# speechbrain/speechbrain

Measured on NVIDIA H100. Metric: audio-sec/sec (RTFx) Conformer-L ASR, batch=32x10s@16kHz, higher is better.
Workload: dtype fp16 operands, fp32 accumulate/residual/softmax

## Files before the change

### speechbrain_b200/csrc/common.cuh

```cuda
#pragma once
#include <cuda.h>
#include <cuda_fp16.h>
#include <cuda_runtime.h>
#include <stdint.h>

#define SBK_OK 0
#define SBK_ERR_CUDA -1
#define SBK_ERR_ARG -2
#define SBK_ERR_UNSUPPORTED -3
#define SBK_ERR_NOMEM -4

namespace sbk {

void set_error(const char* fmt, ...);

#define SBK_CUDA_CHECK(expr)                                                              \
    do {                                                                                  \
        cudaError_t _e = (expr);                                                          \
        if (_e != cudaSuccess) {                                                          \
            sbk::set_error("%s:%d: %s -> %s", __FILE__, __LINE__, #expr, cudaGetErrorString(_e)); \
            return SBK_ERR_CUDA;                                                          \
        }                                                                                 \
    } while (0)

void count_launch();
#define SBK_LAUNCH_CHECK()                   \
    do {                                     \
        sbk::count_launch();                 \
        SBK_CUDA_CHECK(cudaGetLastError());  \
    } while (0)

#define SBK_REQUIRE(cond, ...)            \
    do {                                  \
        if (!(cond)) {                    \
            sbk::set_error(__VA_ARGS__);  \
            return SBK_ERR_ARG;           \
        }                                 \
    } while (0)

__host__ __device__ inline int ceil_div(int a, int b) { return (a + b - 1) / b; }

constexpr int SBK_NUM_SMS = 132;

__device__ __forceinline__ float warp_sum(float v) {
#pragma unroll
    for (int o = 16; o > 0; o >>= 1) v += __shfl_xor_sync(0xffffffffu, v, o);
    return v;
}
__device__ __forceinline__ float warp_max(float v) {
#pragma unroll
    for (int o = 16; o > 0; o >>= 1) v = fmaxf(v, __shfl_xor_sync(0xffffffffu, v, o));
    return v;
}

__device__ __forceinline__ uint32_t smem_u32(const void* p) {
    return static_cast<uint32_t>(__cvta_generic_to_shared(p));
}

__device__ __forceinline__ void mbar_init(uint64_t* bar, uint32_t count) {
    asm volatile("mbarrier.init.shared::cta.b64 [%0], %1;" ::"r"(smem_u32(bar)), "r"(count));
}
__device__ __forceinline__ void mbar_fence_init() {
    asm volatile("fence.mbarrier_init.release.cluster;" ::: "memory");
}
__device__ __forceinline__ void mbar_arrive_expect_tx(uint64_t* bar, uint32_t bytes) {
    asm volatile("mbarrier.arrive.expect_tx.shared::cta.b64 _, [%0], %1;" ::"r"(smem_u32(bar)), "r"(bytes)
                 : "memory");
}
__device__ __forceinline__ void mbar_arrive(uint64_t* bar) {
    asm volatile("mbarrier.arrive.shared::cta.b64 _, [%0];" ::"r"(smem_u32(bar)) : "memory");
}
__device__ __forceinline__ bool mbar_try_wait(uint64_t* bar, uint32_t parity) {
    uint32_t ok;
    asm volatile(
        "{\n\t.reg .pred p;\n\t"
        "mbarrier.try_wait.parity.shared::cta.b64 p, [%1], %2;\n\t"
        "selp.u32 %0, 1, 0, p;\n\t}"
        : "=r"(ok)
        : "r"(smem_u32(bar)), "r"(parity)
        : "memory");
    return ok != 0;
}
__device__ __forceinline__ void mbar_wait(uint64_t* bar, uint32_t parity) {
    while (!mbar_try_wait(bar, parity)) {
    }
}

__device__ __forceinline__ void tma_prefetch_desc(const CUtensorMap* m) {
    asm volatile("prefetch.tensormap [%0];" ::"l"(reinterpret_cast<uint64_t>(m)) : "memory");
}
__device__ __forceinline__ void tma_load_2d(void* smem_dst, const CUtensorMap* m, uint64_t* bar, int c0, int c1) {
    asm volatile(
        "cp.async.bulk.tensor.2d.shared::cluster.global.mbarrier::complete_tx::bytes [%0], [%1, {%3, %4}], [%2];"
        ::"r"(smem_u32(smem_dst)), "l"(reinterpret_cast<uint64_t>(m)), "r"(smem_u32(bar)), "r"(c0), "r"(c1)
        : "memory");
}
__device__ __forceinline__ void tma_load_4d(void* smem_dst, const CUtensorMap* m, uint64_t* bar, int c0, int c1, int c2, int c3) {
    asm volatile(
        "cp.async.bulk.tensor.4d.shared::cluster.global.mbarrier::complete_tx::bytes [%0], [%1, {%3, %4, %5, %6}], [%2];"
        ::"r"(smem_u32(smem_dst)), "l"(reinterpret_cast<uint64_t>(m)), "r"(smem_u32(bar)), "r"(c0), "r"(c1), "r"(c2), "r"(c3)
        : "memory");
}
__device__ __forceinline__ void bulk_load_1d(void* smem_dst, const void* gsrc, uint32_t bytes, uint64_t* bar) {
    asm volatile(
        "cp.async.bulk.shared::cluster.global.mbarrier::complete_tx::bytes [%0], [%1], %2, [%3];"
        ::"r"(smem_u32(smem_dst)), "l"(reinterpret_cast<uint64_t>(gsrc)), "r"(bytes), "r"(smem_u32(bar))
        : "memory");
}

__device__ __forceinline__ void wgmma_fence() { asm volatile("wgmma.fence.sync.aligned;" ::: "memory"); }
__device__ __forceinline__ void wgmma_commit() { asm volatile("wgmma.commit_group.sync.aligned;" ::: "memory"); }
template <int N>
__device__ __forceinline__ void wgmma_wait() { asm volatile("wgmma.wait_group.sync.aligned %0;" ::"n"(N) : "memory"); }

__device__ __forceinline__ uint64_t make_kmajor_sw128_desc(uint32_t smem_addr) {
    uint64_t d = 0;
    d |= static_cast<uint64_t>((smem_addr & 0x3FFFFu) >> 4);
    d |= static_cast<uint64_t>(1) << 16;
    d |= static_cast<uint64_t>(1024 >> 4) << 32;
    d |= static_cast<uint64_t>(1) << 62;
    return d;
}

template <int N>
__device__ __forceinline__ void wgmma_f16(float (&d)[N / 2], uint64_t desc_a, uint64_t desc_b, uint32_t accumulate);
template <>
__device__ __forceinline__ void wgmma_f16<32>(float (&d)[16], uint64_t desc_a, uint64_t desc_b, uint32_t accumulate) {
    asm volatile(
        "{\n\t.reg .pred p;\n\tsetp.ne.b32 p, %18, 0;\n\t"
        "wgmma.mma_async.sync.aligned.m64n32k16.f32.f16.f16 "
        "{%0, %1, %2, %3, %4, %5, %6, %7, %8, %9, %10, %11, %12, %13, %14, %15}, "
        "%16, %17, p, 1, 1, 0, 0;\n\t}"
        : "+f"(d[0]), "+f"(d[1]), "+f"(d[2]), "+f"(d[3]), "+f"(d[4]), "+f"(d[5]), "+f"(d[6]), "+f"(d[7]),
          "+f"(d[8]), "+f"(d[9]), "+f"(d[10]), "+f"(d[11]), "+f"(d[12]), "+f"(d[13]), "+f"(d[14]), "+f"(d[15])
        : "l"(desc_a), "l"(desc_b), "r"(accumulate)
        : "memory");
}
template <>
__device__ __forceinline__ void wgmma_f16<64>(float (&d)[32], uint64_t desc_a, uint64_t desc_b, uint32_t accumulate) {
    asm volatile(
        "{\n\t.reg .pred p;\n\tsetp.ne.b32 p, %34, 0;\n\t"
        "wgmma.mma_async.sync.aligned.m64n64k16.f32.f16.f16 "
        "{%0, %1, %2, %3, %4, %5, %6, %7, %8, %9, %10, %11, %12, %13, %14, %15, "
        "%16, %17, %18, %19, %20, %21, %22, %23, %24, %25, %26, %27, %28, %29, %30, %31}, "
        "%32, %33, p, 1, 1, 0, 0;\n\t}"
        : "+f"(d[0]), "+f"(d[1]), "+f"(d[2]), "+f"(d[3]), "+f"(d[4]), "+f"(d[5]), "+f"(d[6]), "+f"(d[7]),
          "+f"(d[8]), "+f"(d[9]), "+f"(d[10]), "+f"(d[11]), "+f"(d[12]), "+f"(d[13]), "+f"(d[14]), "+f"(d[15]),
          "+f"(d[16]), "+f"(d[17]), "+f"(d[18]), "+f"(d[19]), "+f"(d[20]), "+f"(d[21]), "+f"(d[22]), "+f"(d[23]),
          "+f"(d[24]), "+f"(d[25]), "+f"(d[26]), "+f"(d[27]), "+f"(d[28]), "+f"(d[29]), "+f"(d[30]), "+f"(d[31])
        : "l"(desc_a), "l"(desc_b), "r"(accumulate)
        : "memory");
}
template <>
__device__ __forceinline__ void wgmma_f16<128>(float (&d)[64], uint64_t desc_a, uint64_t desc_b, uint32_t accumulate) {
    asm volatile(
        "{\n\t.reg .pred p;\n\tsetp.ne.b32 p, %66, 0;\n\t"
        "wgmma.mma_async.sync.aligned.m64n128k16.f32.f16.f16 "
        "{%0, %1, %2, %3, %4, %5, %6, %7, %8, %9, %10, %11, %12, %13, %14, %15, "
        "%16, %17, %18, %19, %20, %21, %22, %23, %24, %25, %26, %27, %28, %29, %30, %31, "
        "%32, %33, %34, %35, %36, %37, %38, %39, %40, %41, %42, %43, %44, %45, %46, %47, "
        "%48, %49, %50, %51, %52, %53, %54, %55, %56, %57, %58, %59, %60, %61, %62, %63}, "
        "%64, %65, p, 1, 1, 0, 0;\n\t}"
        : "+f"(d[0]), "+f"(d[1]), "+f"(d[2]), "+f"(d[3]), "+f"(d[4]), "+f"(d[5]), "+f"(d[6]), "+f"(d[7]),
          "+f"(d[8]), "+f"(d[9]), "+f"(d[10]), "+f"(d[11]), "+f"(d[12]), "+f"(d[13]), "+f"(d[14]), "+f"(d[15]),
          "+f"(d[16]), "+f"(d[17]), "+f"(d[18]), "+f"(d[19]), "+f"(d[20]), "+f"(d[21]), "+f"(d[22]), "+f"(d[23]),
          "+f"(d[24]), "+f"(d[25]), "+f"(d[26]), "+f"(d[27]), "+f"(d[28]), "+f"(d[29]), "+f"(d[30]), "+f"(d[31]),
          "+f"(d[32]), "+f"(d[33]), "+f"(d[34]), "+f"(d[35]), "+f"(d[36]), "+f"(d[37]), "+f"(d[38]), "+f"(d[39]),
          "+f"(d[40]), "+f"(d[41]), "+f"(d[42]), "+f"(d[43]), "+f"(d[44]), "+f"(d[45]), "+f"(d[46]), "+f"(d[47]),
          "+f"(d[48]), "+f"(d[49]), "+f"(d[50]), "+f"(d[51]), "+f"(d[52]), "+f"(d[53]), "+f"(d[54]), "+f"(d[55]),
          "+f"(d[56]), "+f"(d[57]), "+f"(d[58]), "+f"(d[59]), "+f"(d[60]), "+f"(d[61]), "+f"(d[62]), "+f"(d[63])
        : "l"(desc_a), "l"(desc_b), "r"(accumulate)
        : "memory");
}

template <>
__device__ __forceinline__ void wgmma_f16<256>(float (&d)[128], uint64_t desc_a, uint64_t desc_b, uint32_t accumulate) {
    asm volatile(
        "{\n\t.reg .pred p;\n\tsetp.ne.b32 p, %130, 0;\n\t"
        "wgmma.mma_async.sync.aligned.m64n256k16.f32.f16.f16 "
        "{"
        "%0, %1, %2, %3, %4, %5, %6, %7, %8, %9, %10, %11, %12, %13, %14, %15, "
        "%16, %17, %18, %19, %20, %21, %22, %23, %24, %25, %26, %27, %28, %29, %30, %31, "
        "%32, %33, %34, %35, %36, %37, %38, %39, %40, %41, %42, %43, %44, %45, %46, %47, "
        "%48, %49, %50, %51, %52, %53, %54, %55, %56, %57, %58, %59, %60, %61, %62, %63, "
        "%64, %65, %66, %67, %68, %69, %70, %71, %72, %73, %74, %75, %76, %77, %78, %79, "
        "%80, %81, %82, %83, %84, %85, %86, %87, %88, %89, %90, %91, %92, %93, %94, %95, "
        "%96, %97, %98, %99, %100, %101, %102, %103, %104, %105, %106, %107, %108, %109, %110, %111, "
        "%112, %113, %114, %115, %116, %117, %118, %119, %120, %121, %122, %123, %124, %125, %126, %127}, "
        "%128, %129, p, 1, 1, 0, 0;\n\t}"
        :
          "+f"(d[0]), "+f"(d[1]), "+f"(d[2]), "+f"(d[3]), "+f"(d[4]), "+f"(d[5]), "+f"(d[6]), "+f"(d[7]),
          "+f"(d[8]), "+f"(d[9]), "+f"(d[10]), "+f"(d[11]), "+f"(d[12]), "+f"(d[13]), "+f"(d[14]), "+f"(d[15]),
          "+f"(d[16]), "+f"(d[17]), "+f"(d[18]), "+f"(d[19]), "+f"(d[20]), "+f"(d[21]), "+f"(d[22]), "+f"(d[23]),
          "+f"(d[24]), "+f"(d[25]), "+f"(d[26]), "+f"(d[27]), "+f"(d[28]), "+f"(d[29]), "+f"(d[30]), "+f"(d[31]),
          "+f"(d[32]), "+f"(d[33]), "+f"(d[34]), "+f"(d[35]), "+f"(d[36]), "+f"(d[37]), "+f"(d[38]), "+f"(d[39]),
          "+f"(d[40]), "+f"(d[41]), "+f"(d[42]), "+f"(d[43]), "+f"(d[44]), "+f"(d[45]), "+f"(d[46]), "+f"(d[47]),
          "+f"(d[48]), "+f"(d[49]), "+f"(d[50]), "+f"(d[51]), "+f"(d[52]), "+f"(d[53]), "+f"(d[54]), "+f"(d[55]),
          "+f"(d[56]), "+f"(d[57]), "+f"(d[58]), "+f"(d[59]), "+f"(d[60]), "+f"(d[61]), "+f"(d[62]), "+f"(d[63]),
          "+f"(d[64]), "+f"(d[65]), "+f"(d[66]), "+f"(d[67]), "+f"(d[68]), "+f"(d[69]), "+f"(d[70]), "+f"(d[71]),
          "+f"(d[72]), "+f"(d[73]), "+f"(d[74]), "+f"(d[75]), "+f"(d[76]), "+f"(d[77]), "+f"(d[78]), "+f"(d[79]),
          "+f"(d[80]), "+f"(d[81]), "+f"(d[82]), "+f"(d[83]), "+f"(d[84]), "+f"(d[85]), "+f"(d[86]), "+f"(d[87]),
          "+f"(d[88]), "+f"(d[89]), "+f"(d[90]), "+f"(d[91]), "+f"(d[92]), "+f"(d[93]), "+f"(d[94]), "+f"(d[95]),
          "+f"(d[96]), "+f"(d[97]), "+f"(d[98]), "+f"(d[99]), "+f"(d[100]), "+f"(d[101]), "+f"(d[102]), "+f"(d[103]),
          "+f"(d[104]), "+f"(d[105]), "+f"(d[106]), "+f"(d[107]), "+f"(d[108]), "+f"(d[109]), "+f"(d[110]), "+f"(d[111]),
          "+f"(d[112]), "+f"(d[113]), "+f"(d[114]), "+f"(d[115]), "+f"(d[116]), "+f"(d[117]), "+f"(d[118]), "+f"(d[119]),
          "+f"(d[120]), "+f"(d[121]), "+f"(d[122]), "+f"(d[123]), "+f"(d[124]), "+f"(d[125]), "+f"(d[126]), "+f"(d[127])
        : "l"(desc_a), "l"(desc_b), "r"(accumulate)
        : "memory");
}

__device__ __forceinline__ __half2 floats2half2_sat(float lo, float hi) {
    uint32_t r;
    asm("cvt.rn.satfinite.f16x2.f32 %0, %1, %2;" : "=r"(r) : "f"(hi), "f"(lo));
    return *reinterpret_cast<__half2*>(&r);
}
__device__ __forceinline__ __half float2half_sat(float x) {
    const __half2 h = floats2half2_sat(x, 0.0f);
    return __low2half(h);
}

__device__ __forceinline__ float rcp_approx(float x) {
    float y;
    asm("rcp.approx.ftz.f32 %0, %1;" : "=f"(y) : "f"(x));
    return y;
}
__device__ __forceinline__ float exp_ftz(float x) {
    float y;
    asm("ex2.approx.ftz.f32 %0, %1;" : "=f"(y) : "f"(x * 1.4426950408889634f));
    return y;
}
__device__ __forceinline__ float sigmoid_f(float x) { return rcp_approx(1.0f + exp_ftz(-x)); }
__device__ __forceinline__ float tanh_approx(float x) {
    float y;
    asm("tanh.approx.f32 %0, %1;" : "=f"(y) : "f"(x));
    return y;
}
__device__ __forceinline__ float sigmoid_fast(float x) { return fmaf(0.5f, tanh_approx(0.5f * x), 0.5f); }
__device__ __forceinline__ float silu_fast(float x) {
    const float h = 0.5f * x;
    return fmaf(h, tanh_approx(h), h);
}
__device__ __forceinline__ void sts128(uint32_t addr, uint4 v) {
    asm volatile("st.shared.v4.b32 [%0], {%1, %2, %3, %4};" ::"r"(addr), "r"(v.x), "r"(v.y), "r"(v.z), "r"(v.w) : "memory");
}
__device__ __forceinline__ uint4 lds128(uint32_t addr) {
    uint4 v;
    asm volatile("ld.shared.v4.b32 {%0, %1, %2, %3}, [%4];" : "=r"(v.x), "=r"(v.y), "=r"(v.z), "=r"(v.w) : "r"(addr) : "memory");
    return v;
}
__device__ __forceinline__ uint4 f4_as_u4(float4 f) {
    return make_uint4(__float_as_uint(f.x), __float_as_uint(f.y), __float_as_uint(f.z), __float_as_uint(f.w));
}
__device__ __forceinline__ float4 u4_as_f4(uint4 u) {
    return make_float4(__uint_as_float(u.x), __uint_as_float(u.y), __uint_as_float(u.z), __uint_as_float(u.w));
}
__device__ __forceinline__ float silu_f(float x) { return x * sigmoid_f(x); }
__device__ __forceinline__ float gelu_erf_f(float x) { return 0.5f * x * (1.0f + erff(x * 0.70710678118654752f)); }

__device__ __forceinline__ int float_to_ordered(float f) {
    int i = __float_as_int(f);
    return i >= 0 ? i : i ^ 0x7FFFFFFF;
}
__device__ __forceinline__ float ordered_to_float(int i) { return __int_as_float(i >= 0 ? i : i ^ 0x7FFFFFFF); }

int make_tmap_2d_f16(CUtensorMap* out, const void* base, uint64_t rows, uint64_t cols, uint64_t row_stride_elems,
                     uint32_t box_rows, uint32_t box_cols);

}
```

### speechbrain_b200/csrc/decoder.cu

```cuda
#include <stdlib.h>

#include <algorithm>

#include "common.cuh"
#include "sbk_internal.h"

namespace sbk {

__device__ __forceinline__ void mma16816_d(float (&d)[4], const uint32_t (&a)[4], uint32_t b0, uint32_t b1) {
    asm volatile(
        "mma.sync.aligned.m16n8k16.row.col.f32.f16.f16.f32 {%0,%1,%2,%3}, {%4,%5,%6,%7}, {%8,%9}, {%0,%1,%2,%3};"
        : "+f"(d[0]), "+f"(d[1]), "+f"(d[2]), "+f"(d[3])
        : "r"(a[0]), "r"(a[1]), "r"(a[2]), "r"(a[3]), "r"(b0), "r"(b1));
}

__device__ __forceinline__ void pdl_trigger() { asm volatile("griddepcontrol.launch_dependents;" ::: "memory"); }
__device__ __forceinline__ void pdl_wait() { asm volatile("griddepcontrol.wait;" ::: "memory"); }

static bool g_use_pdl = true;
void set_pdl(bool on) { g_use_pdl = on; }

template <typename... KArgs, typename... Args>
static cudaError_t launch_k(void (*kern)(KArgs...), dim3 grid, dim3 block, size_t smem, cudaStream_t st, Args... args) {
    cudaLaunchConfig_t cfg = {};
    cfg.gridDim = grid;
    cfg.blockDim = block;
    cfg.dynamicSmemBytes = smem;
    cfg.stream = st;
    cudaLaunchAttribute attr[1];
    attr[0].id = cudaLaunchAttributeProgrammaticStreamSerialization;
    attr[0].val.programmaticStreamSerializationAllowed = 1;
    cfg.attrs = attr;
    cfg.numAttrs = g_use_pdl ? 1 : 0;
    return cudaLaunchKernelEx(&cfg, kern, args...);
}

constexpr int SK_WARPS = 8;

template <int UNR, int NT, int VPL, int MT = 2>
__global__ void __launch_bounds__(SK_WARPS * 32, ((VPL <= 4 && MT == 2) ? 2 : 1)) skinny_gemm_kernel(const SkinnyArgs a) {
    constexpr bool LN = VPL > 0;
    constexpr int SK_ROWS = 16 * MT;
    static_assert(!LN || MT == 2, "the LayerNorm-fused variant owns 32 rows per CTA");
    __shared__ float red[SK_WARPS][SK_ROWS][8 * NT + 1];
    extern __shared__ __align__(16) __half a_sm[];
    const int warp = threadIdx.x >> 5, lane = threadIdx.x & 31, g = lane >> 2, c = lane & 3;
    const int n0 = blockIdx.x * 8 * NT;
    const int row0 = blockIdx.y * SK_ROWS;
    const int rows = min(SK_ROWS, a.n_rows - row0);
    const int k_per_warp = ((a.K / 16 + SK_WARPS - 1) / SK_WARPS) * 16;
    const int k_begin = warp * k_per_warp, k_end = min(a.K, k_begin + k_per_warp);
    pdl_trigger();

    float acc[MT][NT][4];
#pragma unroll
    for (int i = 0; i < MT; ++i)
#pragma unroll
        for (int j = 0; j < NT; ++j) acc[i][j][0] = acc[i][j][1] = acc[i][j][2] = acc[i][j][3] = 0.0f;
    const __half* wrow[NT];
#pragma unroll
    for (int j = 0; j < NT; ++j)
        wrow[j] = a.W + static_cast<size_t>(min(n0 + 8 * j + g, a.N - 1)) * a.ldw + 2 * c;
    uint32_t bf[UNR][NT][2];
#pragma unroll
    for (int u = 0; u < UNR; ++u) {
        const int k = k_begin + 16 * u;
        const bool ok = k < k_end;
#pragma unroll
        for (int j = 0; j < NT; ++j) {
            bf[u][j][0] = ok ? __ldg(reinterpret_cast<const uint32_t*>(wrow[j] + k)) : 0u;
            bf[u][j][1] = ok ? __ldg(reinterpret_cast<const uint32_t*>(wrow[j] + k + 8)) : 0u;
        }
    }
    pdl_wait();

    const int astr = LN ? a.K + 8 : a.lda;
    const __half* abase = LN ? a_sm : a.A;
    if constexpr (LN) {
        float4 v[4][VPL];
#pragma unroll
        for (int r = 0; r < 4; ++r) {
            const float* xr = a.X + static_cast<size_t>(min(row0 + warp + 8 * r, a.n_rows - 1)) * a.K;
#pragma unroll
            for (int i = 0; i < VPL; ++i) v[r][i] = *reinterpret_cast<const float4*>(xr + 4 * (lane + 32 * i));
        }
        float4 gm[VPL], bt[VPL];
#pragma unroll
        for (int i = 0; i < VPL; ++i) {
            gm[i] = __ldg(reinterpret_cast<const float4*>(a.ln_g + 4 * (lane + 32 * i)));
            bt[i] = __ldg(reinterpret_cast<const float4*>(a.ln_b + 4 * (lane + 32 * i)));
        }
        float s[4], q[4];
#pragma unroll
        for (int r = 0; r < 4; ++r) {
            s[r] = 0.0f;
#pragma unroll
            for (int i = 0; i < VPL; ++i) s[r] += (v[r][i].x + v[r][i].y) + (v[r][i].z + v[r][i].w);
        }
#pragma unroll
        for (int o = 16; o > 0; o >>= 1)
#pragma unroll
            for (int r = 0; r < 4; ++r) s[r] += __shfl_xor_sync(0xffffffffu, s[r], o);
        const float inv_k = 1.0f / static_cast<float>(a.K);
#pragma unroll
        for (int r = 0; r < 4; ++r) {
            s[r] *= inv_k;
            q[r] = 0.0f;
#pragma unroll
            for (int i = 0; i < VPL; ++i) {
                v[r][i].x -= s[r]; v[r][i].y -= s[r]; v[r][i].z -= s[r]; v[r][i].w -= s[r];
                q[r] += (v[r][i].x * v[r][i].x + v[r][i].y * v[r][i].y) + (v[r][i].z * v[r][i].z + v[r][i].w * v[r][i].w);
            }
        }
#pragma unroll
        for (int o = 16; o > 0; o >>= 1)
#pragma unroll
            for (int r = 0; r < 4; ++r) q[r] += __shfl_xor_sync(0xffffffffu, q[r], o);
#pragma unroll
        for (int r = 0; r < 4; ++r) {
            const float rstd = rsqrtf(q[r] * inv_k + a.ln_eps);
            __half* dst = a_sm + (warp + 8 * r) * astr;
#pragma unroll
            for (int i = 0; i < VPL; ++i) {
                __half2 h0 = floats2half2_sat(v[r][i].x * rstd * gm[i].x + bt[i].x, v[r][i].y * rstd * gm[i].y + bt[i].y);
                __half2 h1 = floats2half2_sat(v[r][i].z * rstd * gm[i].z + bt[i].z, v[r][i].w * rstd * gm[i].w + bt[i].w);
                uint2 u;
                u.x = *reinterpret_cast<uint32_t*>(&h0);
                u.y = *reinterpret_cast<uint32_t*>(&h1);
                *reinterpret_cast<uint2*>(dst + 4 * (lane + 32 * i)) = u;
            }
        }
        __syncthreads();
    }
    const __half* arow[2 * MT];
#pragma unroll
    for (int i = 0; i < 2 * MT; ++i) {
        const int rr = LN ? (i * 8 + g) : min(row0 + i * 8 + g, a.n_rows - 1);
        arow[i] = abase + static_cast<size_t>(rr) * astr + 2 * c;
    }
    for (int k0 = k_begin; k0 < k_end; k0 += 16 * UNR) {
        uint32_t af[UNR][MT][4];
#pragma unroll
        for (int u = 0; u < UNR; ++u) {
            const int k = k0 + 16 * u;
            const bool ok = k < k_end;
            if (k0 != k_begin) {
#pragma unroll
                for (int j = 0; j < NT; ++j) {
                    bf[u][j][0] = ok ? __ldg(reinterpret_cast<const uint32_t*>(wrow[j] + k)) : 0u;
                    bf[u][j][1] = ok ? __ldg(reinterpret_cast<const uint32_t*>(wrow[j] + k + 8)) : 0u;
                }
            }
#pragma unroll
            for (int mt = 0; mt < MT; ++mt) {
                af[u][mt][0] = ok ? *reinterpret_cast<const uint32_t*>(arow[2 * mt] + k) : 0u;
                af[u][mt][1] = ok ? *reinterpret_cast<const uint32_t*>(arow[2 * mt + 1] + k) : 0u;
                af[u][mt][2] = ok ? *reinterpret_cast<const uint32_t*>(arow[2 * mt] + k + 8) : 0u;
                af[u][mt][3] = ok ? *reinterpret_cast<const uint32_t*>(arow[2 * mt + 1] + k + 8) : 0u;
            }
        }
#pragma unroll
        for (int u = 0; u < UNR; ++u)
#pragma unroll
            for (int j = 0; j < NT; ++j)
#pragma unroll
                for (int mt = 0; mt < MT; ++mt) mma16816_d(acc[mt][j], af[u][mt], bf[u][j][0], bf[u][j][1]);
    }
#pragma unroll
    for (int mt = 0; mt < MT; ++mt)
#pragma unroll
        for (int j = 0; j < NT; ++j) {
            red[warp][mt * 16 + g][8 * j + 2 * c] = acc[mt][j][0];
            red[warp][mt * 16 + g][8 * j + 2 * c + 1] = acc[mt][j][1];
            red[warp][mt * 16 + g + 8][8 * j + 2 * c] = acc[mt][j][2];
            red[warp][mt * 16 + g + 8][8 * j + 2 * c + 1] = acc[mt][j][3];
        }
    __syncthreads();
    const int step = a.step_ptr ? *a.step_ptr : 0;
#pragma unroll
    for (int it = 0; it < NT * MT / 2; ++it) {
        const int idx = threadIdx.x + it * SK_WARPS * 32;
        const int r = idx / (8 * NT), j = idx - r * (8 * NT);
        const int col = n0 + j;
        const int row = row0 + r;
        if (r < rows && col < a.N) {
            float v = 0.0f;
#pragma unroll
            for (int w = 0; w < SK_WARPS; ++w) v += red[w][r][j];
            if (a.bias) v += __ldg(a.bias + col);
            switch (a.epi) {
                case SK_F16: reinterpret_cast<__half*>(a.out)[static_cast<size_t>(row) * a.ldo + col] = float2half_sat(v); break;
                case SK_F16_RELU:
                    reinterpret_cast<__half*>(a.out)[static_cast<size_t>(row) * a.ldo + col] = float2half_sat(fmaxf(v, 0.0f));
                    break;
                case SK_F16_GELU:
                    reinterpret_cast<__half*>(a.out)[static_cast<size_t>(row) * a.ldo + col] = float2half_sat(gelu_erf_f(v));
                    break;
                case SK_F32: reinterpret_cast<float*>(a.out)[static_cast<size_t>(row) * a.ldo + col] = v; break;
                case SK_RESID: reinterpret_cast<float*>(a.out)[static_cast<size_t>(row) * a.ldo + col] += v; break;
                case SK_QKV_CACHE: {
                    if (col < a.d) {
                        reinterpret_cast<__half*>(a.out)[static_cast<size_t>(row) * a.ldo + col] = float2half_sat(v * a.q_scale);
                    } else if (col < 2 * a.d) {
                        a.kcache[(static_cast<size_t>(row) * a.S_max + step) * a.d + (col - a.d)] = float2half_sat(v);
                    } else {
                        a.vcache[(static_cast<size_t>(row) * a.S_max + step) * a.d + (col - 2 * a.d)] = float2half_sat(v);
                    }
                    break;
                }
            }
        }
    }
}

int skinny_gemm(const SkinnyArgs& a, cudaStream_t stream) {
    SBK_REQUIRE(a.K % 16 == 0 && a.lda % 2 == 0 && a.ldw % 2 == 0, "skinny_gemm: K %% 16 required (K=%d)", a.K);
    if (a.n_rows == 0) return SBK_OK;
    cudaError_t e;
    const int ry = ceil_div(a.n_rows, 32);
    if (a.X == nullptr && a.n_rows >= 96 && getenv("SBK_SKINNY_MT8") != nullptr) {
        const dim3 grid(ceil_div(a.N, 8), ceil_div(a.n_rows, 128));
        if (a.K <= 1024) e = launch_k(skinny_gemm_kernel<2, 1, 0, 8>, grid, dim3(SK_WARPS * 32), 0, stream, a);
        else e = launch_k(skinny_gemm_kernel<4, 1, 0, 8>, grid, dim3(SK_WARPS * 32), 0, stream, a);
        SBK_CUDA_CHECK(e);
        SBK_LAUNCH_CHECK();
        return SBK_OK;
    }
    if (a.X != nullptr) {
        const size_t smem = static_cast<size_t>(32) * (a.K + 8) * 2;
        dim3 grid(ceil_div(a.N, 16), ry);
        static bool attr_done = false;
        if (!attr_done) {
            cudaFuncSetAttribute(skinny_gemm_kernel<4, 2, 4>, cudaFuncAttributeMaxDynamicSharedMemorySize, 80 * 1024);
            cudaFuncSetAttribute(skinny_gemm_kernel<2, 2, 2>, cudaFuncAttributeMaxDynamicSharedMemorySize, 80 * 1024);
            cudaFuncSetAttribute(skinny_gemm_kernel<4, 2, 6>, cudaFuncAttributeMaxDynamicSharedMemorySize, 80 * 1024);
            cudaFuncSetAttribute(skinny_gemm_kernel<8, 2, 8>, cudaFuncAttributeMaxDynamicSharedMemorySize, 80 * 1024);
            attr_done = true;
        }
        if (a.K == 512) e = launch_k(skinny_gemm_kernel<4, 2, 4>, grid, dim3(SK_WARPS * 32), smem, stream, a);
        else if (a.K == 256) e = launch_k(skinny_gemm_kernel<2, 2, 2>, grid, dim3(SK_WARPS * 32), smem, stream, a);
        else if (a.K == 768) e = launch_k(skinny_gemm_kernel<4, 2, 6>, grid, dim3(SK_WARPS * 32), smem, stream, a);
        else if (a.K == 1024) e = launch_k(skinny_gemm_kernel<8, 2, 8>, grid, dim3(SK_WARPS * 32), smem, stream, a);
        else {
            set_error("skinny_gemm(LN): d_model=%d not built (256/512/768/1024)", a.K);
            return SBK_ERR_UNSUPPORTED;
        }
    } else if (a.K <= 1024 && a.N >= 1024) {
        e = launch_k(skinny_gemm_kernel<4, 2, 0>, dim3(ceil_div(a.N, 16), ry), dim3(SK_WARPS * 32), 0, stream, a);
    } else if (a.K <= 1024) {
        e = launch_k(skinny_gemm_kernel<4, 1, 0>, dim3(ceil_div(a.N, 8), ry), dim3(SK_WARPS * 32), 0, stream, a);
    } else {
        e = launch_k(skinny_gemm_kernel<8, 1, 0>, dim3(ceil_div(a.N, 8), ry), dim3(SK_WARPS * 32), 0, stream, a);
    }
    SBK_CUDA_CHECK(e);
    SBK_LAUNCH_CHECK();
    return SBK_OK;
}

constexpr int DA_WARPS = 4;
constexpr int DA_CHUNK = 32;
constexpr int DA_KPG = DA_CHUNK / 4;

__global__ void __launch_bounds__(DA_WARPS * 32, 4) dec_attention_kernel(const DecAttnArgs a) {
    __shared__ float part_o[DA_WARPS][64];
    __shared__ float part_m[DA_WARPS], part_l[DA_WARPS];
    const int warp = threadIdx.x >> 5, lane = threadIdx.x & 31;
    const int r = blockIdx.y, h = blockIdx.x;
    const int blk = r / a.rows_per_block;
    pdl_trigger();
    pdl_wait();
    int n_keys;
    if (a.n_keys_ptr) n_keys = *a.n_keys_ptr + 1;
    else n_keys = a.enc_len ? min(a.enc_len[blk], a.n_keys_fixed) : a.n_keys_fixed;
    const int per = (n_keys + DA_WARPS - 1) / DA_WARPS;
    const int kb = warp * per, ke = min(n_keys, kb + per);
    const int gq = lane >> 3, dl = (lane & 7) * 8;
    const int hs = a.head_stride > 0 ? a.head_stride : 64;
    const __half* kbase = a.kbase + static_cast<size_t>(blk) * a.row_stride + static_cast<size_t>(h) * hs + dl;
    const __half* vbase = a.vbase + static_cast<size_t>(blk) * a.row_stride + static_cast<size_t>(h) * hs + dl;
    const int* lin = nullptr;
    if (a.lineage) lin = a.lineage + static_cast<size_t>((n_keys - 1) & 1) * gridDim.y * a.lin_stride + static_cast<size_t>(r) * a.lin_stride;
    const int* tokc = a.tok_cache;
    float qf[8];
    {
        const uint4 qv = *reinterpret_cast<const uint4*>(a.q + static_cast<size_t>(r) * a.ldq + h * 64 + dl);
        const __half2* q2 = reinterpret_cast<const __half2*>(&qv);
#pragma unroll
        for (int u = 0; u < 4; ++u) {
            const float2 f = __half22float2(q2[u]);
            qf[2 * u] = f.x; qf[2 * u + 1] = f.y;
        }
    }
    float m_run = -INFINITY, l_run = 0.0f;
    float o[8];
#pragma unroll
    for (int e = 0; e < 8; ++e) o[e] = 0.0f;
    for (int c0 = kb; c0 < ke; c0 += DA_CHUNK) {
        uint4 kv[DA_KPG], vv[DA_KPG];
        bool live[DA_KPG];
#pragma unroll
        for (int i = 0; i < DA_KPG; ++i) {
            const int j = c0 + gq + 4 * i;
            live[i] = j < ke;
            if (live[i]) {
                ptrdiff_t off = static_cast<ptrdiff_t>(j) * a.key_stride;
                int src_row = r;
                if (lin) { src_row = lin[j]; off += (static_cast<ptrdiff_t>(src_row) - r) * static_cast<ptrdiff_t>(a.row_stride); }
                kv[i] = *reinterpret_cast<const uint4*>(kbase + off);
                vv[i] = *reinterpret_cast<const uint4*>(vbase + off);
                if (tokc) live[i] = tokc[static_cast<size_t>(src_row) * a.lin_stride + j] != a.pad_tok;
            } else {
                kv[i] = make_uint4(0u, 0u, 0u, 0u);
                vv[i] = make_uint4(0u, 0u, 0u, 0u);
            }
        }
        float sc[DA_KPG];
        float cm = -INFINITY;
#pragma unroll
        for (int i = 0; i < DA_KPG; ++i) {
            const __half2* k2 = reinterpret_cast<const __half2*>(&kv[i]);
            float dot = 0.0f;
#pragma unroll
            for (int u = 0; u < 4; ++u) {
                const float2 kf = __half22float2(k2[u]);
                dot = fmaf(kf.x, qf[2 * u], dot);
                dot = fmaf(kf.y, qf[2 * u + 1], dot);
            }
            dot += __shfl_xor_sync(0xffffffffu, dot, 1);
            dot += __shfl_xor_sync(0xffffffffu, dot, 2);
            dot += __shfl_xor_sync(0xffffffffu, dot, 4);
            sc[i] = live[i] ? dot : -INFINITY;
            cm = fmaxf(cm, sc[i]);
        }
        cm = fmaxf(cm, __shfl_xor_sync(0xffffffffu, cm, 8));
        cm = fmaxf(cm, __shfl_xor_sync(0xffffffffu, cm, 16));
        const float m_new = fmaxf(m_run, cm);
        const float alpha = (m_run == -INFINITY) ? 0.0f : __expf(m_run - m_new);
        float psum = 0.0f;
#pragma unroll
        for (int e = 0; e < 8; ++e) o[e] *= alpha;
#pragma unroll
        for (int i = 0; i < DA_KPG; ++i) {
            const float p = (sc[i] == -INFINITY) ? 0.0f : __expf(sc[i] - m_new);
            psum += p;
            const __half2* v2 = reinterpret_cast<const __half2*>(&vv[i]);
#pragma unroll
            for (int u = 0; u < 4; ++u) {
                const float2 vf = __half22float2(v2[u]);
                o[2 * u] = fmaf(p, vf.x, o[2 * u]);
                o[2 * u + 1] = fmaf(p, vf.y, o[2 * u + 1]);
            }
        }
        psum += __shfl_xor_sync(0xffffffffu, psum, 8);
        psum += __shfl_xor_sync(0xffffffffu, psum, 16);
        l_run = l_run * alpha + psum;
        m_run = m_new;
    }
#pragma unroll
    for (int e = 0; e < 8; ++e) {
        o[e] += __shfl_xor_sync(0xffffffffu, o[e], 8);
        o[e] += __shfl_xor_sync(0xffffffffu, o[e], 16);
    }
    if (lane < 8) {
#pragma unroll
        for (int e = 0; e < 8; ++e) part_o[warp][dl + e] = o[e];
    }
    if (lane == 0) { part_m[warp] = m_run; part_l[warp] = l_run; }
    __syncthreads();
    if (threadIdx.x < 64) {
        float M = part_m[0];
#pragma unroll
        for (int w = 1; w < DA_WARPS; ++w) M = fmaxf(M, part_m[w]);
        float num = 0.0f, den = 0.0f;
#pragma unroll
        for (int w = 0; w < DA_WARPS; ++w) {
            const float sc = part_m[w] == -INFINITY ? 0.0f : __expf(part_m[w] - M);
            num += part_o[w][threadIdx.x] * sc;
            den += part_l[w] * sc;
        }
        a.out[static_cast<size_t>(r) * a.ldo + h * 64 + threadIdx.x] = float2half_sat(num / den);
    }
}

__global__ void __launch_bounds__(DA_WARPS * 32)
dec_cross_attention_tma_kernel(const __grid_constant__ CUtensorMap tmap_kv, const DecAttnArgs a, int box_T) {
    extern __shared__ __align__(128) uint8_t xa_smem[];
    __shared__ uint64_t bar;
    __shared__ float part_o[DA_WARPS][64];
    __shared__ float part_m[DA_WARPS], part_l[DA_WARPS];
    const __half* Ks = reinterpret_cast<const __half*>(xa_smem);
    const __half* Vs = Ks + static_cast<size_t>(box_T) * 64;
    const int warp = threadIdx.x >> 5, lane = threadIdx.x & 31;
    const int r = blockIdx.y, h = blockIdx.x;
    const int blk = r / a.rows_per_block;
    if (threadIdx.x == 0) {
        mbar_init(&bar, 1);
        mbar_fence_init();
    }
    __syncthreads();
    if (threadIdx.x == 0) {
        mbar_arrive_expect_tx(&bar, static_cast<uint32_t>(box_T) * 256u);
        tma_load_4d(const_cast<__half*>(Ks), &tmap_kv, &bar, 0, h, 0, blk);
        tma_load_4d(const_cast<__half*>(Vs), &tmap_kv, &bar, 0, a.H + h, 0, blk);
    }
    const int n_keys = a.enc_len ? min(a.enc_len[blk], a.n_keys_fixed) : a.n_keys_fixed;
    const int per = (n_keys + DA_WARPS - 1) / DA_WARPS;
    const int kb = warp * per, ke = min(n_keys, kb + per);
    const int gq = lane >> 3, dl = (lane & 7) * 8;
    float qf[8];
    {
        const uint4 qv = *reinterpret_cast<const uint4*>(a.q + static_cast<size_t>(r) * a.ldq + h * 64 + dl);
        const __half2* q2 = reinterpret_cast<const __half2*>(&qv);
#pragma unroll
        for (int u = 0; u < 4; ++u) {
            const float2 f = __half22float2(q2[u]);
            qf[2 * u] = f.x; qf[2 * u + 1] = f.y;
        }
    }
    float m_run = -INFINITY, l_run = 0.0f;
    float o[8];
#pragma unroll
    for (int e = 0; e < 8; ++e) o[e] = 0.0f;
    mbar_wait(&bar, 0);
    for (int c0 = kb; c0 < ke; c0 += DA_CHUNK) {
        float sc[DA_KPG];
        float cm = -INFINITY;
#pragma unroll
        for (int i = 0; i < DA_KPG; ++i) {
            const int j = c0 + gq + 4 * i;
            float dot = 0.0f;
            if (j < ke) {
                const uint4 kv = *reinterpret_cast<const uint4*>(Ks + static_cast<size_t>(j) * 64 + dl);
                const __half2* k2 = reinterpret_cast<const __half2*>(&kv);
#pragma unroll
                for (int u = 0; u < 4; ++u) {
                    const float2 kf = __half22float2(k2[u]);
                    dot = fmaf(kf.x, qf[2 * u], dot);
                    dot = fmaf(kf.y, qf[2 * u + 1], dot);
                }
            }
            dot += __shfl_xor_sync(0xffffffffu, dot, 1);
            dot += __shfl_xor_sync(0xffffffffu, dot, 2);
            dot += __shfl_xor_sync(0xffffffffu, dot, 4);
            sc[i] = j < ke ? dot : -INFINITY;
            cm = fmaxf(cm, sc[i]);
        }
        cm = fmaxf(cm, __shfl_xor_sync(0xffffffffu, cm, 8));
        cm = fmaxf(cm, __shfl_xor_sync(0xffffffffu, cm, 16));
        const float m_new = fmaxf(m_run, cm);
        const float alpha = (m_run == -INFINITY) ? 0.0f : __expf(m_run - m_new);
        float psum = 0.0f;
#pragma unroll
        for (int e = 0; e < 8; ++e) o[e] *= alpha;
#pragma unroll
        for (int i = 0; i < DA_KPG; ++i) {
            const int j = c0 + gq + 4 * i;
            const float p = (sc[i] == -INFINITY) ? 0.0f : __expf(sc[i] - m_new);
            psum += p;
            if (j < ke) {
                const uint4 vv = *reinterpret_cast<const uint4*>(Vs + static_cast<size_t>(j) * 64 + dl);
                const __half2* v2 = reinterpret_cast<const __half2*>(&vv);
#pragma unroll
                for (int u = 0; u < 4; ++u) {
                    const float2 vf = __half22float2(v2[u]);
                    o[2 * u] = fmaf(p, vf.x, o[2 * u]);
                    o[2 * u + 1] = fmaf(p, vf.y, o[2 * u + 1]);
                }
            }
        }
        psum += __shfl_xor_sync(0xffffffffu, psum, 8);
        psum += __shfl_xor_sync(0xffffffffu, psum, 16);
        l_run = l_run * alpha + psum;
        m_run = m_new;
    }
#pragma unroll
    for (int e = 0; e < 8; ++e) {
        o[e] += __shfl_xor_sync(0xffffffffu, o[e], 8);
        o[e] += __shfl_xor_sync(0xffffffffu, o[e], 16);
    }
    if (lane < 8) {
#pragma unroll
        for (int e = 0; e < 8; ++e) part_o[warp][dl + e] = o[e];
    }
    if (lane == 0) { part_m[warp] = m_run; part_l[warp] = l_run; }
    __syncthreads();
    if (threadIdx.x < 64) {
        float M = part_m[0];
#pragma unroll
        for (int w = 1; w < DA_WARPS; ++w) M = fmaxf(M, part_m[w]);
        float num = 0.0f, den = 0.0f;
#pragma unroll
        for (int w = 0; w < DA_WARPS; ++w) {
            const float sc = part_m[w] == -INFINITY ? 0.0f : __expf(part_m[w] - M);
            num += part_o[w][threadIdx.x] * sc;
            den += part_l[w] * sc;
        }
        a.out[static_cast<size_t>(r) * a.ldo + h * 64 + threadIdx.x] = float2half_sat(num / den);
    }
}

constexpr int XP_WARPS = 8;
__global__ void __launch_bounds__(XP_WARPS * 32, 1)
dec_cross_attention_persist_kernel(const __grid_constant__ CUtensorMap tmap_kv, const DecAttnArgs a, int box_T, int n_items) {
    extern __shared__ __align__(128) uint8_t xp_smem[];
    __shared__ uint64_t full[2];
    __shared__ float part_o[XP_WARPS][64];
    __shared__ float part_m[XP_WARPS], part_l[XP_WARPS];
    const size_t stage_halfs = static_cast<size_t>(box_T) * 128;
    __half* stage0 = reinterpret_cast<__half*>(xp_smem);
    const int warp = threadIdx.x >> 5, lane = threadIdx.x & 31;
    const int gq = lane >> 3, dl = (lane & 7) * 8;
    const int H = a.H;
    if (threadIdx.x == 0) {
        mbar_init(&full[0], 1);
        mbar_init(&full[1], 1);
        mbar_fence_init();
    }
    __syncthreads();
    auto issue = [&](int item, int s) {
        const int r = item / H, h = item - r * H, blk = r / a.rows_per_block;
        __half* dst = stage0 + s * stage_halfs;
        mbar_arrive_expect_tx(&full[s], static_cast<uint32_t>(box_T) * 256u);
        tma_load_4d(dst, &tmap_kv, &full[s], 0, h, 0, blk);
        tma_load_4d(dst + static_cast<size_t>(box_T) * 64, &tmap_kv, &full[s], 0, H + h, 0, blk);
    };
    const int first = blockIdx.x, stride = gridDim.x;
    if (threadIdx.x == 0) {
        if (first < n_items) issue(first, 0);
        if (first + stride < n_items) issue(first + stride, 1);
    }
    auto load_q = [&](int item) {
        const int r = item / H, h = item - r * H;
        return *reinterpret_cast<const uint4*>(a.q + static_cast<size_t>(r) * a.ldq + h * 64 + dl);
    };
    uint4 qv = make_uint4(0u, 0u, 0u, 0u);
    if (first < n_items) qv = load_q(first);
    int it = 0;
    for (int item = first; item < n_items; item += stride, ++it) {
        const int s = it & 1;
        const int r = item / H, h = item - r * H, blk = r / a.rows_per_block;
        float qf[8];
        {
            const __half2* q2 = reinterpret_cast<const __half2*>(&qv);
#pragma unroll
            for (int u = 0; u < 4; ++u) {
                const float2 f = __half22float2(q2[u]);
                qf[2 * u] = f.x; qf[2 * u + 1] = f.y;
            }
        }
        if (item + stride < n_items) qv = load_q(item + stride);
        const int n_keys = a.enc_len ? min(a.enc_len[blk], a.n_keys_fixed) : a.n_keys_fixed;
        const __half* Ks = stage0 + s * stage_halfs;
        const __half* Vs = Ks + static_cast<size_t>(box_T) * 64;
        mbar_wait(&full[s], (it >> 1) & 1);
        const int c0 = warp * DA_CHUNK;
        float sc[DA_KPG];
        float cm = -INFINITY;
#pragma unroll
        for (int i = 0; i < DA_KPG; ++i) {
            const int j = c0 + gq + 4 * i;
            float dot = 0.0f;
            if (j < n_keys) {
                const uint4 kv = *reinterpret_cast<const uint4*>(Ks + static_cast<size_t>(j) * 64 + dl);
                const __half2* k2 = reinterpret_cast<const __half2*>(&kv);
#pragma unroll
                for (int u = 0; u < 4; ++u) {
                    const float2 kf = __half22float2(k2[u]);
                    dot = fmaf(kf.x, qf[2 * u], dot);
                    dot = fmaf(kf.y, qf[2 * u + 1], dot);
                }
            }
            dot += __shfl_xor_sync(0xffffffffu, dot, 1);
            dot += __shfl_xor_sync(0xffffffffu, dot, 2);
            dot += __shfl_xor_sync(0xffffffffu, dot, 4);
            sc[i] = j < n_keys ? dot : -INFINITY;
            cm = fmaxf(cm, sc[i]);
        }
        cm = fmaxf(cm, __shfl_xor_sync(0xffffffffu, cm, 8));
        cm = fmaxf(cm, __shfl_xor_sync(0xffffffffu, cm, 16));
        float o[8];
#pragma unroll
        for (int e = 0; e < 8; ++e) o[e] = 0.0f;
        float psum = 0.0f;
#pragma unroll
        for (int i = 0; i < DA_KPG; ++i) {
            const int j = c0 + gq + 4 * i;
            const float p = (sc[i] == -INFINITY) ? 0.0f : __expf(sc[i] - cm);
            psum += p;
            if (j < n_keys) {
                const uint4 vv = *reinterpret_cast<const uint4*>(Vs + static_cast<size_t>(j) * 64 + dl);
                const __half2* v2 = reinterpret_cast<const __half2*>(&vv);
#pragma unroll
                for (int u = 0; u < 4; ++u) {
                    const float2 vf = __half22float2(v2[u]);
                    o[2 * u] = fmaf(p, vf.x, o[2 * u]);
                    o[2 * u + 1] = fmaf(p, vf.y, o[2 * u + 1]);
                }
            }
        }
        psum += __shfl_xor_sync(0xffffffffu, psum, 8);
        psum += __shfl_xor_sync(0xffffffffu, psum, 16);
#pragma unroll
        for (int e = 0; e < 8; ++e) {
            o[e] += __shfl_xor_sync(0xffffffffu, o[e], 8);
            o[e] += __shfl_xor_sync(0xffffffffu, o[e], 16);
        }
        if (lane < 8) {
#pragma unroll
            for (int e = 0; e < 8; ++e) part_o[warp][dl + e] = o[e];
        }
        if (lane == 0) { part_m[warp] = cm; part_l[warp] = psum; }
        __syncthreads();
        if (threadIdx.x == 0 && item + 2 * stride < n_items) issue(item + 2 * stride, s);
        if (threadIdx.x < 64) {
            float M = part_m[0];
#pragma unroll
            for (int w = 1; w < XP_WARPS; ++w) M = fmaxf(M, part_m[w]);
            float num = 0.0f, den = 0.0f;
// ... 936 lines not shown
```

### speechbrain_b200/csrc/encoder_ops.cu

```cuda
#include <algorithm>

#include "common.cuh"
#include "sbk_internal.h"

namespace sbk {

constexpr int LN_MAX_PER_LANE = 32;

template <bool OUT_HALF>
__global__ void __launch_bounds__(256)
layernorm_rows_kernel(const float* __restrict__ x, void* __restrict__ out, const float* __restrict__ gamma,
                      const float* __restrict__ beta, int M, int D, float eps, int act_silu) {
    const int row = blockIdx.x * (blockDim.x >> 5) + (threadIdx.x >> 5);
    if (row >= M) return;
    const int lane = threadIdx.x & 31;
    const float* xr = x + static_cast<size_t>(row) * D;
    float v[LN_MAX_PER_LANE];
    float s = 0.0f;
    const int nv = D >> 2;
#pragma unroll
    for (int i = 0; i < LN_MAX_PER_LANE / 4; ++i) {
        const int vi = lane + i * 32;
        if (vi < nv) {
            const float4 t = *reinterpret_cast<const float4*>(xr + vi * 4);
            v[4 * i] = t.x; v[4 * i + 1] = t.y; v[4 * i + 2] = t.z; v[4 * i + 3] = t.w;
            s += (t.x + t.y) + (t.z + t.w);
        } else {
            v[4 * i] = v[4 * i + 1] = v[4 * i + 2] = v[4 * i + 3] = 0.0f;
        }
    }
    const float mean = warp_sum(s) / D;
    float q = 0.0f;
#pragma unroll
    for (int i = 0; i < LN_MAX_PER_LANE / 4; ++i) {
        const int vi = lane + i * 32;
        if (vi < nv) {
#pragma unroll
            for (int j = 0; j < 4; ++j) {
                const float d = v[4 * i + j] - mean;
                q += d * d;
            }
        }
    }
    const float rstd = rsqrtf(warp_sum(q) / D + eps);
#pragma unroll
    for (int i = 0; i < LN_MAX_PER_LANE / 4; ++i) {
        const int vi = lane + i * 32;
        if (vi < nv) {
            const float4 g = __ldg(reinterpret_cast<const float4*>(gamma + vi * 4));
            const float4 b = __ldg(reinterpret_cast<const float4*>(beta + vi * 4));
            float y0 = (v[4 * i] - mean) * rstd * g.x + b.x;
            float y1 = (v[4 * i + 1] - mean) * rstd * g.y + b.y;
            float y2 = (v[4 * i + 2] - mean) * rstd * g.z + b.z;
            float y3 = (v[4 * i + 3] - mean) * rstd * g.w + b.w;
            if (act_silu) { y0 = silu_f(y0); y1 = silu_f(y1); y2 = silu_f(y2); y3 = silu_f(y3); }
            if constexpr (OUT_HALF) {
                __half2 h0 = floats2half2_sat(y0, y1), h1 = floats2half2_sat(y2, y3);
                uint2 u;
                u.x = *reinterpret_cast<uint32_t*>(&h0);
                u.y = *reinterpret_cast<uint32_t*>(&h1);
                *reinterpret_cast<uint2*>(reinterpret_cast<__half*>(out) + static_cast<size_t>(row) * D + vi * 4) = u;
            } else {
                *reinterpret_cast<float4*>(reinterpret_cast<float*>(out) + static_cast<size_t>(row) * D + vi * 4) =
                    make_float4(y0, y1, y2, y3);
            }
        }
    }
}

int layernorm_rows(const float* x, void* out, bool out_half, const float* gamma, const float* beta, int M, int D,
                   float eps, bool act_silu, cudaStream_t stream) {
    SBK_REQUIRE(D % 4 == 0 && D <= 32 * LN_MAX_PER_LANE, "layernorm_rows: D=%d unsupported", D);
    if (M == 0) return SBK_OK;
    const int rows_per_cta = 8;
    if (out_half)
        layernorm_rows_kernel<true><<<ceil_div(M, rows_per_cta), rows_per_cta * 32, 0, stream>>>(x, out, gamma, beta, M, D,
                                                                                              eps, act_silu);
    else
        layernorm_rows_kernel<false><<<ceil_div(M, rows_per_cta), rows_per_cta * 32, 0, stream>>>(x, out, gamma, beta, M,
                                                                                               D, eps, act_silu);
    SBK_LAUNCH_CHECK();
    return SBK_OK;
}


template <bool OUT_HALF>
__global__ void __launch_bounds__(256)
layernorm2_rows_kernel(const float* __restrict__ x, float* __restrict__ y_out, void* __restrict__ z_out,
                       const float* __restrict__ ga, const float* __restrict__ ba, float eps_a,
                       const float* __restrict__ gb, const float* __restrict__ bb, float eps_b, int M, int D) {
    const int row = blockIdx.x * (blockDim.x >> 5) + (threadIdx.x >> 5);
    if (row >= M) return;
    const int lane = threadIdx.x & 31;
    const float* xr = x + static_cast<size_t>(row) * D;
    float v[LN_MAX_PER_LANE];
    const int nv = D >> 2;
    float s = 0.0f;
#pragma unroll
    for (int i = 0; i < LN_MAX_PER_LANE / 4; ++i) {
        const int vi = lane + i * 32;
        float4 t = make_float4(0.f, 0.f, 0.f, 0.f);
        if (vi < nv) t = *reinterpret_cast<const float4*>(xr + vi * 4);
        v[4 * i] = t.x; v[4 * i + 1] = t.y; v[4 * i + 2] = t.z; v[4 * i + 3] = t.w;
        s += (t.x + t.y) + (t.z + t.w);
    }
    float mean = warp_sum(s) / D;
    float q = 0.0f;
#pragma unroll
    for (int i = 0; i < LN_MAX_PER_LANE / 4; ++i)
        if (lane + i * 32 < nv) {
#pragma unroll
            for (int j = 0; j < 4; ++j) { const float d = v[4 * i + j] - mean; q += d * d; }
        }
    float rstd = rsqrtf(warp_sum(q) / D + eps_a);
    s = 0.0f;
#pragma unroll
    for (int i = 0; i < LN_MAX_PER_LANE / 4; ++i) {
        const int vi = lane + i * 32;
        if (vi < nv) {
            const float4 g = __ldg(reinterpret_cast<const float4*>(ga + vi * 4));
            const float4 b = __ldg(reinterpret_cast<const float4*>(ba + vi * 4));
            v[4 * i] = (v[4 * i] - mean) * rstd * g.x + b.x;
            v[4 * i + 1] = (v[4 * i + 1] - mean) * rstd * g.y + b.y;
            v[4 * i + 2] = (v[4 * i + 2] - mean) * rstd * g.z + b.z;
            v[4 * i + 3] = (v[4 * i + 3] - mean) * rstd * g.w + b.w;
            if (y_out != nullptr)
                *reinterpret_cast<float4*>(y_out + static_cast<size_t>(row) * D + vi * 4) =
                    make_float4(v[4 * i], v[4 * i + 1], v[4 * i + 2], v[4 * i + 3]);
            s += (v[4 * i] + v[4 * i + 1]) + (v[4 * i + 2] + v[4 * i + 3]);
        }
    }
    mean = warp_sum(s) / D;
    q = 0.0f;
#pragma unroll
    for (int i = 0; i < LN_MAX_PER_LANE / 4; ++i)
        if (lane + i * 32 < nv) {
#pragma unroll
            for (int j = 0; j < 4; ++j) { const float d = v[4 * i + j] - mean; q += d * d; }
        }
    rstd = rsqrtf(warp_sum(q) / D + eps_b);
#pragma unroll
    for (int i = 0; i < LN_MAX_PER_LANE / 4; ++i) {
        const int vi = lane + i * 32;
        if (vi < nv) {
            const float4 g = __ldg(reinterpret_cast<const float4*>(gb + vi * 4));
            const float4 b = __ldg(reinterpret_cast<const float4*>(bb + vi * 4));
            const float z0 = (v[4 * i] - mean) * rstd * g.x + b.x, z1 = (v[4 * i + 1] - mean) * rstd * g.y + b.y;
            const float z2 = (v[4 * i + 2] - mean) * rstd * g.z + b.z, z3 = (v[4 * i + 3] - mean) * rstd * g.w + b.w;
            if constexpr (OUT_HALF) {
                __half2 h0 = floats2half2_sat(z0, z1), h1 = floats2half2_sat(z2, z3);
                uint2 u;
                u.x = *reinterpret_cast<uint32_t*>(&h0);
                u.y = *reinterpret_cast<uint32_t*>(&h1);
                *reinterpret_cast<uint2*>(reinterpret_cast<__half*>(z_out) + static_cast<size_t>(row) * D + vi * 4) = u;
            } else {
                *reinterpret_cast<float4*>(reinterpret_cast<float*>(z_out) + static_cast<size_t>(row) * D + vi * 4) =
                    make_float4(z0, z1, z2, z3);
            }
        }
    }
}

int layernorm2_rows(const float* x, float* y_out, void* z_out, bool z_half, const float* ga, const float* ba, float eps_a,
                    const float* gb, const float* bb, float eps_b, int M, int D, cudaStream_t stream) {
    SBK_REQUIRE(D % 4 == 0 && D <= 32 * LN_MAX_PER_LANE, "layernorm2_rows: D=%d unsupported", D);
    if (M == 0) return SBK_OK;
    const int rows_per_cta = 8;
    if (z_half)
        layernorm2_rows_kernel<true><<<ceil_div(M, rows_per_cta), rows_per_cta * 32, 0, stream>>>(x, y_out, z_out, ga, ba, eps_a,
                                                                                                 gb, bb, eps_b, M, D);
    else
        layernorm2_rows_kernel<false><<<ceil_div(M, rows_per_cta), rows_per_cta * 32, 0, stream>>>(x, y_out, z_out, ga, ba, eps_a,
                                                                                                  gb, bb, eps_b, M, D);
    SBK_LAUNCH_CHECK();
    return SBK_OK;
}

__global__ void cast_f32_f16_kernel(const float* __restrict__ in, __half* __restrict__ out, size_t n) {
    for (size_t i = blockIdx.x * static_cast<size_t>(blockDim.x) + threadIdx.x; i < n;
         i += static_cast<size_t>(gridDim.x) * blockDim.x)
        out[i] = float2half_sat(in[i]);
}
int cast_f32_f16(const float* in, __half* out, size_t n, cudaStream_t stream) {
    if (n == 0) return SBK_OK;
    const int blocks = static_cast<int>(std::min<size_t>((n + 255) / 256, SBK_NUM_SMS * 16));
    cast_f32_f16_kernel<<<blocks, 256, 0, stream>>>(in, out, n);
    SBK_LAUNCH_CHECK();
    return SBK_OK;
}

constexpr int DW_TT = 16;

template <int KT, int MAXC, bool CHUNKED = false>
__global__ void __launch_bounds__(256, 2)
dwconv_ln_swish_kernel(const float* __restrict__ glu, int T, int D, int K, const float* __restrict__ wdw ,
                       const float* __restrict__ bdw, const float* __restrict__ gamma, const float* __restrict__ beta,
                       float eps, __half* __restrict__ out, int chunk) {
    extern __shared__ __align__(128) float dw_smem[];
    __shared__ uint64_t bar;
    const int halo = (K - 1) / 2;
    const int rows_in = DW_TT + K - 1;
    float* slab = dw_smem;
    const int b = blockIdx.y, t0 = blockIdx.x * DW_TT;
    const float* src = glu + static_cast<size_t>(b) * T * D;
    const int r_lo = max(0, halo - t0), r_hi = min(rows_in, T + halo - t0);
    if (threadIdx.x == 0) {
        mbar_init(&bar, 1);
        mbar_fence_init();
    }
    __syncthreads();
    if (threadIdx.x == 0) {
        const uint32_t row_bytes = static_cast<uint32_t>(D) * 4;
        mbar_arrive_expect_tx(&bar, row_bytes * static_cast<uint32_t>(r_hi - r_lo));
        for (int r = r_lo; r < r_hi; r += 8) {
            const int nr = min(8, r_hi - r);
            bulk_load_1d(slab + r * D, src + static_cast<size_t>(t0 - halo + r) * D, row_bytes * nr, &bar);
        }
    }
    for (int i = threadIdx.x; i < (r_lo + rows_in - r_hi) * D; i += blockDim.x) {
        int r = i / D;
        const int ch = i - r * D;
        if (r >= r_lo) r += r_hi - r_lo;
        slab[r * D + ch] = 0.0f;
    }
    float wreg[KT > 0 ? MAXC : 1][KT > 0 ? KT : 1];
    float breg[MAXC];
#pragma unroll
    for (int cc = 0; cc < MAXC; ++cc) {
        const int ch = threadIdx.x + cc * 256;
        breg[cc] = 0.0f;
        if (ch < D) {
            breg[cc] = __ldg(bdw + ch);
            if constexpr (KT > 0) {
#pragma unroll
                for (int k = 0; k < KT; ++k) wreg[cc][k] = __ldg(wdw + static_cast<size_t>(k) * D + ch);
            }
        }
    }
    mbar_wait(&bar, 0);
    __syncthreads();
    float acc[MAXC][DW_TT];
#pragma unroll
    for (int cc = 0; cc < MAXC; ++cc) {
        const int ch = threadIdx.x + cc * 256;
        if (ch < D) {
            const float bz = breg[cc];
#pragma unroll
            for (int i = 0; i < DW_TT; ++i) acc[cc][i] = bz;
            const float* w = wdw + ch;
            if constexpr (KT > 0) {
                int lim[CHUNKED ? DW_TT : 1];
                if constexpr (CHUNKED) {
#pragma unroll
                    for (int i = 0; i < DW_TT; ++i) lim[i] = ((t0 + i) / chunk + 1) * chunk - t0 + halo;
                }
#pragma unroll
                for (int r = 0; r < DW_TT + KT - 1; ++r) {
                    const float xv = slab[r * D + ch];
#pragma unroll
                    for (int i = 0; i < DW_TT; ++i)
                        if (r - i >= 0 && r - i < KT) {
                            if constexpr (CHUNKED) acc[cc][i] = fmaf(r < lim[i] ? xv : 0.0f, wreg[cc][r - i], acc[cc][i]);
                            else acc[cc][i] = fmaf(xv, wreg[cc][r - i], acc[cc][i]);
                        }
                }
            } else {
                for (int r = 0; r < rows_in; ++r) {
                    const float xv = slab[r * D + ch];
#pragma unroll
                    for (int i = 0; i < DW_TT; ++i) {
                        const int k = r - i;
                        if (k >= 0 && k < K && (!CHUNKED || r < ((t0 + i) / chunk + 1) * chunk - t0 + halo))
                            acc[cc][i] = fmaf(xv, __ldg(w + static_cast<size_t>(k) * D), acc[cc][i]);
                    }
                }
            }
        }
    }
    __syncthreads();
#pragma unroll
    for (int cc = 0; cc < MAXC; ++cc) {
        const int ch = threadIdx.x + cc * 256;
        if (ch < D) {
#pragma unroll
            for (int i = 0; i < DW_TT; ++i) slab[i * D + ch] = acc[cc][i];
        }
    }
    __syncthreads();
    const int warp = threadIdx.x >> 5, lane = threadIdx.x & 31;
    constexpr int MAXP = MAXC * 4;
    float2 g2[MAXP], b2[MAXP];
#pragma unroll
    for (int p = 0; p < MAXP; ++p) {
        const int j = 2 * lane + 64 * p;
        if (j < D) {
            g2[p] = __ldg(reinterpret_cast<const float2*>(gamma + j));
            b2[p] = __ldg(reinterpret_cast<const float2*>(beta + j));
        }
    }
    for (int i = warp; i < DW_TT; i += (blockDim.x >> 5)) {
        const int t = t0 + i;
        if (t >= T) continue;
        const float* c = slab + i * D;
        float s = 0.0f;
        for (int j = lane; j < D; j += 32) s += c[j];
        const float mean = warp_sum(s) / D;
        float q = 0.0f;
        for (int j = lane; j < D; j += 32) {
            const float d = c[j] - mean;
            q += d * d;
        }
        const float rstd = rsqrtf(warp_sum(q) / D + eps);
        __half* o = out + (static_cast<size_t>(b) * T + t) * D;
#pragma unroll
        for (int p = 0; p < MAXP; ++p) {
            const int j = 2 * lane + 64 * p;
            if (j < D) {
                const float2 cv = *reinterpret_cast<const float2*>(c + j);
                const float y0 = silu_f((cv.x - mean) * rstd * g2[p].x + b2[p].x);
                const float y1 = silu_f((cv.y - mean) * rstd * g2[p].y + b2[p].y);
                *reinterpret_cast<__half2*>(o + j) = floats2half2_sat(y0, y1);
            }
        }
    }
}

int dwconv_ln_swish(const float* glu, int B, int T, int D, int K, const float* wdw, const float* bdw,
                    const float* gamma, const float* beta, float eps, __half* out, cudaStream_t stream, int chunk) {
    SBK_REQUIRE(D % 4 == 0 && D <= 1024 && (K & 1) == 1, "dwconv_ln_swish: D %% 4, D <= 1024 and odd K required (D=%d K=%d)", D, K);
    SBK_REQUIRE((reinterpret_cast<uintptr_t>(glu) & 15) == 0, "dwconv_ln_swish: input must be 16-byte aligned");
    const size_t smem = static_cast<size_t>(DW_TT + K - 1) * D * sizeof(float);
    SBK_REQUIRE(smem <= 200 * 1024, "dwconv_ln_swish: tile too large for shared memory (D=%d K=%d)", D, K);
    auto kern = dwconv_ln_swish_kernel<0, 4>;
    if (chunk > 0) {
        kern = dwconv_ln_swish_kernel<0, 4, true>;
        if (K == 31) kern = D <= 256 ? dwconv_ln_swish_kernel<31, 1, true> : D <= 512 ? dwconv_ln_swish_kernel<31, 2, true>
                                                                                        : dwconv_ln_swish_kernel<31, 4, true>;
    } else if (K == 31) {
        kern = D <= 256 ? dwconv_ln_swish_kernel<31, 1> : D <= 512 ? dwconv_ln_swish_kernel<31, 2> : dwconv_ln_swish_kernel<31, 4>;
    }
    SBK_CUDA_CHECK(cudaFuncSetAttribute(kern, cudaFuncAttributeMaxDynamicSharedMemorySize, (int)smem));
    kern<<<dim3(ceil_div(T, DW_TT), B), 256, smem, stream>>>(glu, T, D, K, wdw, bdw, gamma, beta, eps, out, chunk);
    SBK_LAUNCH_CHECK();
    return SBK_OK;
}

constexpr int ATT_BQ = 64;
constexpr int ATT_BK = 64;

__device__ __forceinline__ void ldmatrix_x2_trans(uint32_t& r0, uint32_t& r1, const void* p) {
    asm volatile("ldmatrix.sync.aligned.m8n8.x2.trans.shared.b16 {%0,%1}, [%2];" : "=r"(r0), "=r"(r1) : "r"(smem_u32(p)));
}
__device__ __forceinline__ void ldmatrix_x4(uint32_t& r0, uint32_t& r1, uint32_t& r2, uint32_t& r3, const void* p) {
    asm volatile("ldmatrix.sync.aligned.m8n8.x4.shared.b16 {%0,%1,%2,%3}, [%4];"
                 : "=r"(r0), "=r"(r1), "=r"(r2), "=r"(r3) : "r"(smem_u32(p)));
}
__device__ __forceinline__ void ldmatrix_x2(uint32_t& r0, uint32_t& r1, const void* p) {
    asm volatile("ldmatrix.sync.aligned.m8n8.x2.shared.b16 {%0,%1}, [%2];" : "=r"(r0), "=r"(r1) : "r"(smem_u32(p)));
}
__device__ __forceinline__ void ldmatrix_x4_trans(uint32_t& r0, uint32_t& r1, uint32_t& r2, uint32_t& r3, const void* p) {
    asm volatile("ldmatrix.sync.aligned.m8n8.x4.trans.shared.b16 {%0,%1,%2,%3}, [%4];"
                 : "=r"(r0), "=r"(r1), "=r"(r2), "=r"(r3) : "r"(smem_u32(p)));
}
__device__ __forceinline__ float ex2_ftz(float x) {
    float y;
    asm("ex2.approx.ftz.f32 %0, %1;" : "=f"(y) : "f"(x));
    return y;
}
__device__ __forceinline__ void mma16816(float (&d)[4], const uint32_t (&a)[4], uint32_t b0, uint32_t b1) {
    asm volatile(
        "mma.sync.aligned.m16n8k16.row.col.f32.f16.f16.f32 {%0,%1,%2,%3}, {%4,%5,%6,%7}, {%8,%9}, {%0,%1,%2,%3};"
        : "+f"(d[0]), "+f"(d[1]), "+f"(d[2]), "+f"(d[3])
        : "r"(a[0]), "r"(a[1]), "r"(a[2]), "r"(a[3]), "r"(b0), "r"(b1));
}
__device__ __forceinline__ uint32_t pack_half2(float a, float b) {
    __half2 h = floats2half2_sat(a, b);
    return *reinterpret_cast<uint32_t*>(&h);
}

template <int DH, int DHP, bool RELPOS>
__global__ void __launch_bounds__(128)
encoder_attention_kernel(const __half* __restrict__ qkv, int ld, int T, const int* __restrict__ lens,
                         const float* __restrict__ pos_u, const float* __restrict__ pos_v,
// ... 319 lines not shown
```

### speechbrain_b200/csrc/engine.cu

```cuda
#include <math.h>
#include <stdio.h>
#include <stdlib.h>
#include <string.h>

#include <algorithm>
#include <map>
#include <string>
#include <vector>

#include "common.cuh"
#include "sbk_internal.h"
#include "../../include/sbk.h"

namespace sbk {

struct EncLayerW {
    const float *ffn1_ln_g, *ffn1_ln_b, *ffn1_b1, *ffn1_b2;
    const __half *ffn1_w1, *ffn1_w2;
    const float *norm1_g, *norm1_b;
    const __half *wqkv, *wo;
    const float* bo;
    const __half* wpos;
    const float *pos_u, *pos_v;
    const float *conv_ln_g, *conv_ln_b;
// ... 387 lines not shown
            std::vector<float> ws(wi, wi + (size_t)3 * dl * dl), bs(bi, bi + 3 * dl);
            for (size_t i = 0; i < (size_t)dl * dl; ++i) ws[i] *= qs;
            for (int i = 0; i < dl; ++i) bs[i] *= qs;
            e.w_in = p.f16_raw(ws.data(), ws.size());
            e.b_in = p.f32_raw(bs.data(), bs.size());
            e.w_out = p.f16(q + "self_att.att.out_proj.weight", (int64_t)dl * dl); e.b_out = p.f32(q + "self_att.att.out_proj.bias", dl);
            e.w1 = p.f16(q + "pos_ffn.ffn.0.weight", (int64_t)Fl * dl); e.b1 = p.f32(q + "pos_ffn.ffn.0.bias", Fl);
            e.w2 = p.f16(q + "pos_ffn.ffn.3.weight", (int64_t)dl * Fl); e.b2 = p.f32(q + "pos_ffn.ffn.3.bias", dl);
            e.n1g = p.f32(q + "norm1.norm.weight", dl); e.n1b = p.f32(q + "norm1.norm.bias", dl);
            e.n2g = p.f32(q + "norm2.norm.weight", dl); e.n2b = p.f32(q + "norm2.norm.bias", dl);
        }
        m->lm_norm_g = p.f32("lm.encoder.norm.norm.weight", dl); m->lm_norm_b = p.f32("lm.encoder.norm.norm.bias", dl);
        m->lm_wp0 = p.f16("lm.output_proj.layers.0.w.weight", (int64_t)dl * dl); m->lm_bp0 = p.f32("lm.output_proj.layers.0.w.bias", dl);
        m->lm_lnp_g = p.f32("lm.output_proj.layers.1.norm.weight", dl); m->lm_lnp_b = p.f32("lm.output_proj.layers.1.norm.bias", dl);
        m->lm_wp2 = p.f16("lm.output_proj.layers.2.w.weight", (int64_t)c.vocab * dl); m->lm_bp2 = p.f32("lm.output_proj.layers.2.w.bias", c.vocab);
        if (!p.ok) { rc = SBK_ERR_ARG; goto fail; }
    }
    if (w.count("ctc_lin.w.weight")) {
        m->w_ctc = p.f16("ctc_lin.w.weight", (int64_t)c.vocab * d);
        m->b_ctc = p.f32("ctc_lin.w.bias", c.vocab);
    }
    if (!p.ok) { rc = SBK_ERR_ARG; goto fail; }
    if (cudaMallocHost(&m->host_flag, 64) != cudaSuccess) { set_error("cudaMallocHost failed"); rc = SBK_ERR_NOMEM; goto fail; }
    m->weight_refs = new int(1);
    if (cudaDeviceSynchronize() != cudaSuccess) { set_error("asr_create: device error after upload"); rc = SBK_ERR_CUDA; goto fail; }
    *out = m;
    return SBK_OK;
fail:
    if (m->fbank) fbank_destroy(m->fbank);
    cudaFree(m->warena.base);
    delete m;
    return rc;
}

int asr_clone(AsrModel* src, AsrModel** out) {
    SBK_REQUIRE(src && out, "asr_clone: null argument");
    AsrModel* m = new AsrModel(*src);
    m->ws = Arena();
    m->wsB = m->wsL = m->ws_rows = m->ws_steps = 0;
    m->b = AsrModel::Buf();
    m->ctc = AsrModel::CtcBuf();
    m->cov = AsrModel::CovBuf();
    m->step_graph = nullptr;
    m->pipe_graph = nullptr;
    m->group_graph = nullptr;
    m->hgroup_graph = nullptr;
    m->beam_graph = nullptr;
    m->gwav = m->grel = nullptr; m->gwav_cap = 0;
    m->copy_stream = nullptr; m->ev_fork = nullptr;
    for (auto& e : m->ev_ready) e = nullptr;
    m->graph_rows = m->graph_T = m->graph_B = -1;
    m->cap_stream = nullptr;
    m->host_flag = nullptr;
    if (cudaMallocHost(&m->host_flag, 64) != cudaSuccess) {
        delete m;
        set_error("asr_clone: cudaMallocHost failed");
        return SBK_ERR_NOMEM;
    }
    ++*m->weight_refs;
    *out = m;
    return SBK_OK;
}

void asr_destroy(AsrModel* m) {
    if (!m) return;
    if (m->step_graph) cudaGraphExecDestroy(m->step_graph);
    if (m->pipe_graph) cudaGraphExecDestroy(m->pipe_graph);
    if (m->group_graph) cudaGraphExecDestroy(m->group_graph);
    if (m->hgroup_graph) cudaGraphExecDestroy(m->hgroup_graph);
    if (m->beam_graph) cudaGraphExecDestroy(m->beam_graph);
    cudaFree(m->gwav);
    if (m->copy_stream) cudaStreamDestroy(m->copy_stream);
    if (m->ev_fork) cudaEventDestroy(m->ev_fork);
    for (auto e : m->ev_ready) if (e) cudaEventDestroy(e);
    if (m->weight_refs && --*m->weight_refs == 0) {
        if (m->fbank) fbank_destroy(m->fbank);
        cudaFree(m->warena.base);
        delete m->weight_refs;
    }
    cudaFree(m->ws.base);
    cudaFree(m->ctc.base);
    cudaFree(m->cov.base);
    if (m->host_flag) cudaFreeHost(m->host_flag);
    if (m->cap_stream) cudaStreamDestroy(m->cap_stream);
    if (m->side_stream) cudaStreamDestroy(m->side_stream);
    if (m->dec_stream) cudaStreamDestroy(m->dec_stream);
    if (m->ev_dfork) cudaEventDestroy(m->ev_dfork);
    if (m->ev_djoin) cudaEventDestroy(m->ev_djoin);
    if (m->ev_bfork) cudaEventDestroy(m->ev_bfork);
    if (m->ev_bjoin) cudaEventDestroy(m->ev_bjoin);
    delete m;
}

static void drop_graphs(AsrModel* m) {
    if (m->step_graph) { cudaGraphExecDestroy(m->step_graph); m->step_graph = nullptr; m->graph_rows = -1; }
    if (m->pipe_graph) { cudaGraphExecDestroy(m->pipe_graph); m->pipe_graph = nullptr; }
    if (m->group_graph) { cudaGraphExecDestroy(m->group_graph); m->group_graph = nullptr; }
    if (m->hgroup_graph) { cudaGraphExecDestroy(m->hgroup_graph); m->hgroup_graph = nullptr; }
    if (m->beam_graph) { cudaGraphExecDestroy(m->beam_graph); m->beam_graph = nullptr; }
}

static void frames(const sbk_asr_config& c, int L, int* T0, int* T1, int* T2) {
    *T0 = 1 + L / c.hop;
    *T1 = (*T0 - 1) / 2 + 1;
    *T2 = (*T1 - 1) / 2 + 1;
}

static int ensure_workspace(AsrModel* m, int B, int L, int rows, int steps) {
    if (m->ws.base && B <= m->wsB && L <= m->wsL && rows <= m->ws_rows && steps <= m->ws_steps) return SBK_OK;
    B = std::max(B, m->wsB); L = std::max(L, m->wsL); rows = std::max(rows, m->ws_rows); steps = std::max(steps, m->ws_steps);
    const sbk_asr_config& c = m->cfg;
    int T0, T1, T2;
    frames(c, L, &T0, &T1, &T2);
    const int F1 = (c.n_mels - 1) / 2 + 1;
    const size_t M = (size_t)B * T2, d = c.d_model, F = c.d_ffn, Ld = c.num_decoder_layers, S = steps + 1;
    const size_t Md = (size_t)std::max(B, rows) * T2;
    size_t need = 0;
    auto sz = [&](size_t bytes) { need += (bytes + 255) & ~size_t(255); };
    sz((size_t)B * L * 4); sz((size_t)B * T0 * c.n_mels * 4); sz(M * d * 4); sz(M * d * 4); sz(Md * d * 4);
    sz((size_t)B * T1 * F1 * c.cnn_c1 * 4); sz(M * c.input_size * 4); sz((size_t)rows * d * 4);
    sz((size_t)rows * c.vocab * 4); sz((size_t)rows * S * 4);
    sz(B * 4); sz((size_t)std::max(B, rows) * 4); sz((size_t)rows * (S + 1) * 4); sz(rows * 4 + 64); sz(rows * 4); sz(64); sz((size_t)rows * S * 4); sz(B * 4);
    sz((size_t)B * T1 * F1 * c.cnn_c1 * 2); sz(M * c.input_size * 2); sz(M * d * 2); sz(M * F * 2); sz(M * 3 * d * 2);
    sz(M * d * 2); sz((size_t)T2 * d * 2); sz(Md * d * 2); sz(Md * Ld * 2 * d * 2);
    sz((size_t)Ld * rows * S * d * 2); sz((size_t)Ld * rows * S * d * 2);
    sz((size_t)rows * d * 2); sz((size_t)rows * d * 2); sz((size_t)rows * d * 2); sz((size_t)rows * F * 2);
    sz((size_t)2 * rows * S * 4); sz(B * 4 + 64); sz((size_t)2 * rows * 4); sz((size_t)rows * d * 4); sz((size_t)rows * 33 * 4);
    sz((size_t)rows * S * 4); sz((size_t)rows * S * 4); sz((size_t)rows * S * 4); sz((size_t)rows * S * 4);
    const size_t dl = m->has_lm ? c.lm_d_model : 0, Fl = m->has_lm ? c.lm_d_ffn : 0, Ll = m->has_lm ? c.lm_layers : 0;
    if (m->has_lm) {
        sz(rows * dl * 4); sz(rows * dl * 4); sz((size_t)rows * c.vocab * 4); sz((size_t)rows * c.vocab * 4);
        sz(rows * dl * 2); sz(rows * dl * 2); sz(rows * dl * 2); sz(rows * Fl * 2); sz(rows * dl * 2);
        sz(Ll * rows * S * dl * 2); sz(Ll * rows * S * dl * 2); sz((size_t)rows * S * 4);
    }
    need += 1 << 20;
    if (need > m->ws.cap) {
        if (m->ws.base) { cudaDeviceSynchronize(); cudaFree(m->ws.base); m->ws.base = nullptr; }
        if (cudaMalloc(&m->ws.base, need) != cudaSuccess) {
            m->ws.cap = 0;
            set_error("workspace cudaMalloc(%zu) failed", need);
            return SBK_ERR_NOMEM;
        }
        m->ws.cap = need;
    }
    drop_graphs(m);
    m->ws.used = 0;
    AsrModel::Buf& b = m->b;
#define TAKE(field, type, bytes) b.field = reinterpret_cast<type*>(m->ws.take(bytes))
    TAKE(wav, float, (size_t)B * L * 4); TAKE(feats, float, (size_t)B * T0 * c.n_mels * 4); TAKE(x, float, M * d * 4);
    TAKE(glu, float, M * d * 4); TAKE(enc_out, float, Md * d * 4); TAKE(act1_f, float, (size_t)B * T1 * F1 * c.cnn_c1 * 4);
    TAKE(cnn_f, float, M * c.input_size * 4); TAKE(dx, float, (size_t)rows * d * 4); TAKE(logits, float, (size_t)rows * c.vocab * 4);
    TAKE(score, float, (size_t)rows * S * 4);
    TAKE(utt_max, int, B * 4); TAKE(enc_len, int, (size_t)std::max(B, rows) * 4); TAKE(tokens, int, (size_t)rows * (S + 1) * 4); TAKE(step, int, rows * 4 + 64);
    TAKE(has_ended, int, rows * 4); TAKE(ended_count, int, 64); TAKE(pred, int, (size_t)rows * S * 4); TAKE(rel_len, float, B * 4);
    TAKE(act1, __half, (size_t)B * T1 * F1 * c.cnn_c1 * 2); TAKE(a_in, __half, M * c.input_size * 2); TAKE(h16, __half, M * d * 2);
    TAKE(f16, __half, M * F * 2); TAKE(qkv16, __half, M * 3 * d * 2); TAKE(att16, __half, M * d * 2);
    TAKE(P16, __half, (size_t)T2 * d * 2); TAKE(enc16, __half, Md * d * 2); TAKE(ckv16, __half, Md * Ld * 2 * d * 2);
    TAKE(kcache, __half, (size_t)Ld * rows * S * d * 2); TAKE(vcache, __half, (size_t)Ld * rows * S * d * 2);
    TAKE(dh16, __half, (size_t)rows * d * 2); TAKE(dq16, __half, (size_t)rows * d * 2); TAKE(datt16, __half, (size_t)rows * d * 2);
    TAKE(df16, __half, (size_t)rows * F * 2);
    TAKE(lineage, int, (size_t)2 * rows * S * 4); TAKE(finished, int, B * 4 + 64); TAKE(seq_scores, float, (size_t)2 * rows * 4);
    TAKE(lnout, float, (size_t)rows * d * 4); TAKE(beam_scr, float, (size_t)rows * 33 * 4);
    TAKE(hist_tok, int, (size_t)rows * S * 4); TAKE(hist_pred, int, (size_t)rows * S * 4);
    TAKE(hist_score, float, (size_t)rows * S * 4); TAKE(hist_lp, float, (size_t)rows * S * 4);
    if (m->has_lm) {
        TAKE(lx, float, rows * dl * 4); TAKE(lh32, float, rows * dl * 4); TAKE(lm_logits, float, (size_t)rows * c.vocab * 4);
        TAKE(lm_extra, float, (size_t)rows * c.vocab * 4);
        TAKE(lx16, __half, rows * dl * 2); TAKE(lq16, __half, rows * dl * 2); TAKE(latt16, __half, rows * dl * 2);
        TAKE(lf16, __half, rows * Fl * 2); TAKE(lh16, __half, rows * dl * 2);
        TAKE(lkc, __half, Ll * rows * S * dl * 2); TAKE(lvc, __half, Ll * rows * S * dl * 2); TAKE(tok_cache, int, (size_t)rows * S * 4);
        if (!b.tok_cache) { set_error("workspace carve failed (LM)"); return SBK_ERR_NOMEM; }
    }
    if (!b.df16 || !b.seq_scores || !b.lnout || !b.hist_lp) { set_error("workspace carve failed"); return SBK_ERR_NOMEM; }
#undef TAKE
    m->wsB = B; m->wsL = L; m->ws_rows = rows; m->ws_steps = steps;
    return SBK_OK;
}

#define RC(expr) do { int _rc = (expr); if (_rc) return _rc; } while (0)

static int run_encoder(AsrModel* m, const float* feats, int B, int T0, const int* enc_len, float* cnn_out_f,
                       float* enc_out, cudaStream_t st) {
    const sbk_asr_config& c = m->cfg;
    AsrModel::Buf& b = m->b;
    const int T1 = (T0 - 1) / 2 + 1, T = feats ? (T1 - 1) / 2 + 1 : T0;
    const int M = B * T, d = c.d_model, F = c.d_ffn, H = c.nhead, dh = d / H;
    SBK_REQUIRE(m->has_enc, "encode: this handle was created without encoder weights");
    SBK_REQUIRE(feats == nullptr || m->has_cnn, "encode: this handle was created without CNN weights");
    SBK_REQUIRE(T <= m->pos_len, "encode: %d frames exceed max_len=%d", T, m->pos_len);
    if (feats != nullptr)
        RC(cnn_frontend_forward(feats, B, T0, c.n_mels, m->c1_w, m->c1_b, m->c1_g, m->c1_be, c.cnn_c1, m->c2_w, m->c2_b,
                                m->c2_g, m->c2_be, c.cnn_c2, b.act1, nullptr, b.a_in, cnn_out_f, st));
    GemmEpilogue e;
    e.mode = EPI_F32; e.bias = m->b_in; e.out = b.x; e.ldo = d;
    RC(gemm_f16(b.a_in, c.input_size, m->w_in, c.input_size, e, M, d, c.input_size, st));
    const float att_scale = 1.0f / sqrtf((float)d);
    for (int l = 0; l < c.num_encoder_layers; ++l) {
        const EncLayerW& w = m->enc[l];
        if (l == 0) RC(layernorm_rows(b.x, b.h16, true, w.ffn1_ln_g, w.ffn1_ln_b, M, d, 1e-5f, false, st));
        e = GemmEpilogue(); e.mode = EPI_F16; e.act = ACT_SILU; e.bias = w.ffn1_b1; e.out = b.f16; e.ldo = F;
        RC(gemm_f16(b.h16, d, w.ffn1_w1, d, e, M, F, d, st));
        e = GemmEpilogue(); e.mode = EPI_RESID; e.bias = w.ffn1_b2; e.out = b.x; e.resid = b.x; e.ldo = d; e.alpha = 0.5f;
        RC(gemm_f16(b.f16, F, w.ffn1_w2, F, e, M, d, F, st));
        RC(layernorm_rows(b.x, b.h16, true, w.norm1_g, w.norm1_b, M, d, 1e-5f, false, st));
        e = GemmEpilogue(); e.out = b.qkv16; e.ldo = 3 * d;
        if (c.attention_type == SBK_ATT_ROPE) {
            e.mode = EPI_ROPE; e.alpha = att_scale; e.T = T; e.rope_cos = m->rope_cos; e.rope_sin = m->rope_sin; e.head_dim = dh;
        } else {
            e.mode = EPI_F16;
        }
        RC(gemm_f16(b.h16, d, w.wqkv, d, e, M, 3 * d, d, st));
        if (c.attention_type == SBK_ATT_RELPOS) {
            e = GemmEpilogue(); e.mode = EPI_F16; e.out = b.P16; e.ldo = d;
            RC(gemm_f16(m->relpos_pe, d, w.wpos, d, e, T, d, d, st));
        }
        RC(encoder_attention(b.qkv16, 3 * d, B, T, H, dh, enc_len, c.attention_type == SBK_ATT_RELPOS, w.pos_u, w.pos_v,
                             b.P16, d, att_scale, b.att16, d, st, m->dyn_chunk, m->dyn_left));
        e = GemmEpilogue(); e.mode = EPI_RESID; e.bias = w.bo; e.out = b.x; e.resid = b.x; e.ldo = d; e.alpha = 1.0f;
        RC(gemm_f16(b.att16, d, w.wo, d, e, M, d, d, st));
        RC(layernorm_rows(b.x, b.h16, true, w.conv_ln_g, w.conv_ln_b, M, d, 1e-5f, false, st));
        e = GemmEpilogue(); e.mode = EPI_GLU; e.bias = w.bpw1; e.out = b.glu; e.ldo = d;
        RC(gemm_f16(b.h16, d, w.wpw1, d, e, M, 2 * d, d, st));
        RC(dwconv_ln_swish(b.glu, B, T, d, c.kernel_size, w.wdw, w.bdw, w.aconv_ln_g, w.aconv_ln_b, 1e-5f, b.h16, st, m->dyn_chunk));
        e = GemmEpilogue(); e.mode = EPI_RESID; e.bias = w.bpw2; e.out = b.x; e.resid = b.x; e.ldo = d; e.alpha = 1.0f;
        e.row_lens = enc_len; e.T = T;
        RC(gemm_f16(b.h16, d, w.wpw2, d, e, M, d, d, st));
        RC(layernorm_rows(b.x, b.h16, true, w.ffn2_ln_g, w.ffn2_ln_b, M, d, 1e-5f, false, st));
        e = GemmEpilogue(); e.mode = EPI_F16; e.act = ACT_SILU; e.bias = w.ffn2_b1; e.out = b.f16; e.ldo = F;
        RC(gemm_f16(b.h16, d, w.ffn2_w1, d, e, M, F, d, st));
        e = GemmEpilogue(); e.mode = EPI_RESID; e.bias = w.ffn2_b2; e.out = b.x; e.resid = b.x; e.ldo = d; e.alpha = 0.5f;
        RC(gemm_f16(b.f16, F, w.ffn2_w2, F, e, M, d, F, st));
        if (l + 1 < c.num_encoder_layers) {
            const EncLayerW& nx = m->enc[l + 1];
            RC(layernorm2_rows(b.x, b.x, b.h16, true, w.norm2_g, w.norm2_b, 1e-5f, nx.ffn1_ln_g, nx.ffn1_ln_b, 1e-5f, M, d, st));
        } else {
            RC(layernorm2_rows(b.x, nullptr, enc_out, false, w.norm2_g, w.norm2_b, 1e-5f, m->enc_norm_g, m->enc_norm_b, 1e-6f, M,
                               d, st));
        }
    }
    if (c.num_encoder_layers == 0)
        RC(layernorm_rows(b.x, enc_out, false, m->enc_norm_g, m->enc_norm_b, M, d, 1e-6f, false, st));
    return SBK_OK;
}

__global__ void abs_len_kernel(const float* rel, int B, int T, int* out) {
    const int i = blockIdx.x * blockDim.x + threadIdx.x;
    if (i < B) out[i] = min(T, max(0, __float2int_rn(rel[i] * static_cast<float>(T))));
}

static int dec_ln(AsrModel* m, SkinnyArgs& a, const float* g, const float* bta, int rows, cudaStream_t st) {
    AsrModel::Buf& b = m->b;
    const int d = m->cfg.d_model;
    if (m->fuse_dec_ln && (d == 256 || d == 512 || d == 768 || d == 1024)) {
        a.X = b.dx; a.ln_g = g; a.ln_b = bta; a.ln_eps = 1e-6f;
        return SBK_OK;
    }
    a.A = b.dh16; a.lda = d;
    return layernorm_rows(b.dx, b.dh16, true, g, bta, rows, d, 1e-6f, false, st);
}

static bool xatt_headmajor(const AsrModel* m) {
    static const bool legacy = getenv("SBK_XATT_ROWMAJOR") != nullptr || getenv("SBK_GEMM_V1") != nullptr;
    return !legacy && m->cfg.d_model / m->cfg.nhead == 64 && m->cfg.d_model % 256 == 0;
}
static int project_cross_kv(AsrModel* m, int M, int T, cudaStream_t st) {
    const sbk_asr_config& c = m->cfg;
    AsrModel::Buf& b = m->b;
    const int d = c.d_model, Ld = c.num_decoder_layers;
    RC(cast_f32_f16(b.enc_out, b.enc16, (size_t)M * d, st));
    if (xatt_headmajor(m)) {
        GemmEpilogue e;
        e.mode = EPI_F16; e.bias = m->b_ckv; e.out = b.ckv16; e.ldo = Ld * 2 * d;
        e.kv_heads = c.nhead; e.kv_part_stride = (size_t)M * d; e.kv_layer_stride = (size_t)M * 2 * d; e.T = T;
        return gemm_f16(b.enc16, d, m->w_ckv, d, e, M, Ld * 2 * d, d, st);
    }
    for (int l = 0; l < Ld; ++l) {
        GemmEpilogue e;
        e.mode = EPI_F16; e.bias = m->b_ckv + (size_t)l * 2 * d; e.out = b.ckv16 + (size_t)l * M * 2 * d; e.ldo = 2 * d;
        RC(gemm_f16(b.enc16, d, m->w_ckv + (size_t)l * 2 * d * d, d, e, M, 2 * d, d, st));
    }
    return SBK_OK;
}
static void cross_kv_args(const AsrModel* m, DecAttnArgs& t, int l, int n_utt, int T) {
    const int d = m->cfg.d_model;
    const size_t M = (size_t)n_utt * T;
    t.kbase = m->b.ckv16 + (size_t)l * M * 2 * d;
    if (xatt_headmajor(m)) {
        t.vbase = t.kbase + M * d; t.row_stride = (size_t)T * d; t.head_stride = T * 64; t.key_stride = 64;
    } else {
        t.vbase = t.kbase + d; t.row_stride = (size_t)T * 2 * d; t.head_stride = 0; t.key_stride = 2 * d;
    }
}

static int enqueue_decode_layers_tc(AsrModel* m, int rows, int rows_per_utt, int T, int S_max, const int* lineage,
                                    cudaStream_t st, bool with_head) {
    const sbk_asr_config& c = m->cfg;
    AsrModel::Buf& b = m->b;
    const int d = c.d_model, F = c.d_ffn, H = c.nhead, dh = d / H, Ld = c.num_decoder_layers;
    const int n_utt = rows / rows_per_utt;
    for (int l = 0; l < Ld; ++l) {
        const DecLayerW& w = m->dec[l];
        __half* kc = b.kcache + (size_t)l * rows * S_max * d;
        __half* vc = b.vcache + (size_t)l * rows * S_max * d;
        RC(layernorm_rows(b.dx, b.dh16, true, w.n1g, w.n1b, rows, d, 1e-6f, false, st));
        GemmEpilogue e;
        e.mode = EPI_QKV_CACHE; e.bias = w.b_self_in; e.out = b.dq16; e.ldo = d; e.kcache = kc; e.vcache = vc;
        e.step_ptr = b.step; e.S_max = S_max; e.qkv_d = d;
        RC(gemm_f16_small(b.dh16, d, w.w_self_in, d, e, rows, 3 * d, d, st));
        DecAttnArgs t{};
        t.q = b.dq16; t.ldq = d; t.kbase = kc; t.vbase = vc; t.row_stride = (size_t)S_max * d; t.key_stride = d;
        t.rows_per_block = 1; t.n_keys_ptr = b.step; t.enc_len = nullptr; t.H = H; t.dh = dh; t.out = b.datt16; t.ldo = d;
        t.lineage = lineage; t.lin_stride = S_max;
        RC(dec_attention(t, rows, S_max, st));
        e = GemmEpilogue(); e.mode = EPI_RESID; e.bias = w.b_self_out; e.out = b.dx; e.resid = b.dx; e.ldo = d;
        RC(gemm_f16_small(b.datt16, d, w.w_self_out, d, e, rows, d, d, st));
        RC(layernorm_rows(b.dx, b.dh16, true, w.n2g, w.n2b, rows, d, 1e-6f, false, st));
        e = GemmEpilogue(); e.mode = EPI_F16; e.bias = w.b_cross_q; e.out = b.dq16; e.ldo = d;
        RC(gemm_f16_small(b.dh16, d, w.w_cross_q, d, e, rows, d, d, st));
        t = DecAttnArgs{};
        t.q = b.dq16; t.ldq = d; cross_kv_args(m, t, l, n_utt, T); t.rows_per_block = rows_per_utt;
        t.n_keys_ptr = nullptr; t.enc_len = b.enc_len; t.H = H; t.dh = dh; t.out = b.datt16; t.ldo = d;
        RC(dec_attention(t, rows, T, st));
        e = GemmEpilogue(); e.mode = EPI_RESID; e.bias = w.b_cross_out; e.out = b.dx; e.resid = b.dx; e.ldo = d;
        RC(gemm_f16_small(b.datt16, d, w.w_cross_out, d, e, rows, d, d, st));
        RC(layernorm_rows(b.dx, b.dh16, true, w.n3g, w.n3b, rows, d, 1e-6f, false, st));
        e = GemmEpilogue(); e.mode = EPI_F16; e.act = c.decoder_activation == SBK_ACT_GELU ? ACT_GELU : ACT_RELU;
        e.bias = w.b_ffn1; e.out = b.df16; e.ldo = F;
        RC(gemm_f16_small(b.dh16, d, w.w_ffn1, d, e, rows, F, d, st));
        e = GemmEpilogue(); e.mode = EPI_RESID; e.bias = w.b_ffn2; e.out = b.dx; e.resid = b.dx; e.ldo = d;
        RC(gemm_f16_small(b.df16, F, w.w_ffn2, F, e, rows, d, F, st));
    }
    if (!with_head) return SBK_OK;
    SBK_REQUIRE(m->w_lin != nullptr, "decode step: this handle was created without the output head (seq_lin.w.*)");
    RC(layernorm_rows(b.dx, b.dh16, true, m->dec_norm_g, m->dec_norm_b, rows, d, 1e-6f, false, st));
    GemmEpilogue e;
    e.mode = EPI_F32; e.bias = m->b_lin; e.out = b.logits; e.ldo = c.vocab;
    RC(gemm_f16_small(b.dh16, d, m->w_lin, d, e, rows, c.vocab, d, st));
    return SBK_OK;
}

static int enqueue_decode_layers(AsrModel* m, int rows, int rows_per_utt, int T, int S_max, const int* lineage,
                                 cudaStream_t st, bool with_head = true) {
    if (rows >= m->dec_tc_rows && m->cfg.d_model % 32 == 0)
        return enqueue_decode_layers_tc(m, rows, rows_per_utt, T, S_max, lineage, st, with_head);
    const sbk_asr_config& c = m->cfg;
    AsrModel::Buf& b = m->b;
    const int d = c.d_model, F = c.d_ffn, H = c.nhead, dh = d / H, Ld = c.num_decoder_layers;
    const int ffn_epi = c.decoder_activation == SBK_ACT_GELU ? SK_F16_GELU : SK_F16_RELU;
    const int n_utt = rows / rows_per_utt;
    for (int l = 0; l < Ld; ++l) {
        const DecLayerW& w = m->dec[l];
        __half* kc = b.kcache + (size_t)l * rows * S_max * d;
        __half* vc = b.vcache + (size_t)l * rows * S_max * d;
        SkinnyArgs a{};
        RC(dec_ln(m, a, w.n1g, w.n1b, rows, st));
        a.W = w.w_self_in; a.ldw = d; a.bias = w.b_self_in; a.n_rows = rows; a.N = 3 * d; a.K = d;
        a.epi = SK_QKV_CACHE; a.out = b.dq16; a.ldo = d; a.kcache = kc; a.vcache = vc; a.step_ptr = b.step; a.S_max = S_max;
        a.d = d; a.q_scale = 1.0f;
        RC(skinny_gemm(a, st));
        DecAttnArgs t{};
        t.q = b.dq16; t.ldq = d; t.kbase = kc; t.vbase = vc; t.row_stride = (size_t)S_max * d; t.key_stride = d;
        t.rows_per_block = 1; t.n_keys_ptr = b.step; t.enc_len = nullptr; t.H = H; t.dh = dh; t.out = b.datt16; t.ldo = d;
        t.lineage = lineage; t.lin_stride = S_max;
        RC(dec_attention(t, rows, S_max, st));
        a = SkinnyArgs{}; a.A = b.datt16; a.lda = d; a.W = w.w_self_out; a.ldw = d; a.bias = w.b_self_out; a.n_rows = rows;
        a.N = d; a.K = d; a.epi = SK_RESID; a.out = b.dx; a.ldo = d;
        RC(skinny_gemm(a, st));
        a = SkinnyArgs{};
        RC(dec_ln(m, a, w.n2g, w.n2b, rows, st));
        a.W = w.w_cross_q; a.ldw = d; a.bias = w.b_cross_q; a.n_rows = rows;
        a.N = d; a.K = d; a.epi = SK_F16; a.out = b.dq16; a.ldo = d;
        RC(skinny_gemm(a, st));
        t = DecAttnArgs{};
        t.q = b.dq16; t.ldq = d; cross_kv_args(m, t, l, n_utt, T); t.rows_per_block = rows_per_utt;
        t.n_keys_ptr = nullptr; t.enc_len = b.enc_len; t.H = H; t.dh = dh; t.out = b.datt16; t.ldo = d;
        RC(dec_attention(t, rows, T, st));
        a = SkinnyArgs{}; a.A = b.datt16; a.lda = d; a.W = w.w_cross_out; a.ldw = d; a.bias = w.b_cross_out; a.n_rows = rows;
        a.N = d; a.K = d; a.epi = SK_RESID; a.out = b.dx; a.ldo = d;
        RC(skinny_gemm(a, st));
        a = SkinnyArgs{};
        RC(dec_ln(m, a, w.n3g, w.n3b, rows, st));
        a.W = w.w_ffn1; a.ldw = d; a.bias = w.b_ffn1; a.n_rows = rows;
        a.N = F; a.K = d; a.epi = ffn_epi; a.out = b.df16; a.ldo = F;
        RC(skinny_gemm(a, st));
        a = SkinnyArgs{}; a.A = b.df16; a.lda = F; a.W = w.w_ffn2; a.ldw = F; a.bias = w.b_ffn2; a.n_rows = rows;
        a.N = d; a.K = F; a.epi = SK_RESID; a.out = b.dx; a.ldo = d;
        RC(skinny_gemm(a, st));
    }
    if (!with_head) return SBK_OK;
    SBK_REQUIRE(m->w_lin != nullptr, "decode step: this handle was created without the output head (seq_lin.w.*)");
    SkinnyArgs a{};
    RC(dec_ln(m, a, m->dec_norm_g, m->dec_norm_b, rows, st));
    a.W = m->w_lin; a.ldw = d; a.bias = m->b_lin; a.n_rows = rows; a.N = c.vocab; a.K = d;
    a.epi = SK_F32; a.out = b.logits; a.ldo = c.vocab;
    RC(skinny_gemm(a, st));
    return SBK_OK;
}

static int enqueue_decode_step(AsrModel* m, int rows, int rows_per_utt, int T, int S_max, int eos, float* log_probs,
                               int L_lp, cudaStream_t st) {
    AsrModel::Buf& b = m->b;
    RC(enqueue_decode_layers(m, rows, rows_per_utt, T, S_max, nullptr, st));
    RC(greedy_select(b.logits, rows, m->cfg.vocab, b.step, eos, b.tokens, S_max + 1, b.has_ended, b.ended_count, b.pred,
                     b.score, S_max, log_probs, L_lp, m->emb, m->dec_pe, m->cfg.d_model, b.dx, st));
    return SBK_OK;
}

static int enqueue_lm_step_tc(AsrModel* m, int rows, int S_max, float temperature, float weight, cudaStream_t st) {
    const sbk_asr_config& c = m->cfg;
    AsrModel::Buf& b = m->b;
    const int dl = c.lm_d_model, Fl = c.lm_d_ffn, H = c.lm_nhead;
    for (int l = 0; l < c.lm_layers; ++l) {
        const LmLayerW& w = m->lm[l];
        __half* kc = b.lkc + (size_t)l * rows * S_max * dl;
        __half* vc = b.lvc + (size_t)l * rows * S_max * dl;
        GemmEpilogue e;
        e.mode = EPI_QKV_CACHE; e.bias = w.b_in; e.out = b.lq16; e.ldo = dl; e.kcache = kc; e.vcache = vc;
        e.step_ptr = b.step; e.S_max = S_max; e.qkv_d = dl;
        RC(gemm_f16_small(b.lx16, dl, w.w_in, dl, e, rows, 3 * dl, dl, st));
        DecAttnArgs t{};
        t.q = b.lq16; t.ldq = dl; t.kbase = kc; t.vbase = vc; t.row_stride = (size_t)S_max * dl; t.key_stride = dl;
        t.rows_per_block = 1; t.n_keys_ptr = b.step; t.H = H; t.dh = 64; t.out = b.latt16; t.ldo = dl;
        t.lineage = b.lineage; t.lin_stride = S_max; t.tok_cache = b.tok_cache; t.pad_tok = 0;
        RC(dec_attention(t, rows, S_max, st));
        e = GemmEpilogue(); e.mode = EPI_RESID; e.bias = w.b_out; e.out = b.lx; e.resid = b.lx; e.ldo = dl;
        RC(gemm_f16_small(b.latt16, dl, w.w_out, dl, e, rows, dl, dl, st));
        RC(layernorm_dual(b.lx, b.lx16, w.n1g, w.n1b, rows, dl, 1e-6f, true, st));
        e = GemmEpilogue(); e.mode = EPI_F16; e.act = c.lm_activation == SBK_ACT_GELU ? ACT_GELU : ACT_RELU;
        e.bias = w.b1; e.out = b.lf16; e.ldo = Fl;
        RC(gemm_f16_small(b.lx16, dl, w.w1, dl, e, rows, Fl, dl, st));
        e = GemmEpilogue(); e.mode = EPI_RESID; e.bias = w.b2; e.out = b.lx; e.resid = b.lx; e.ldo = dl;
        RC(gemm_f16_small(b.lf16, Fl, w.w2, Fl, e, rows, dl, Fl, st));
        RC(layernorm_dual(b.lx, b.lx16, w.n2g, w.n2b, rows, dl, 1e-6f, true, st));
    }
    RC(layernorm_dual(b.lx, b.lx16, m->lm_norm_g, m->lm_norm_b, rows, dl, 1e-6f, false, st));
    GemmEpilogue e;
    e.mode = EPI_F32; e.bias = m->lm_bp0; e.out = b.lh32; e.ldo = dl;
    RC(gemm_f16_small(b.lx16, dl, m->lm_wp0, dl, e, rows, dl, dl, st));
    RC(layernorm_dual(b.lh32, b.lh16, m->lm_lnp_g, m->lm_lnp_b, rows, dl, 1e-6f, false, st));
    e = GemmEpilogue(); e.mode = EPI_F32; e.bias = m->lm_bp2; e.out = b.lm_logits; e.ldo = c.vocab;
    RC(gemm_f16_small(b.lh16, dl, m->lm_wp2, dl, e, rows, c.vocab, dl, st));
    RC(weighted_log_softmax(b.lm_logits, b.lm_extra, rows, c.vocab, temperature, weight, st));
    return SBK_OK;
}

static int enqueue_lm_step(AsrModel* m, int rows, int S_max, float temperature, float weight, cudaStream_t st) {
    if (rows >= m->dec_tc_rows) return enqueue_lm_step_tc(m, rows, S_max, temperature, weight, st);
    const sbk_asr_config& c = m->cfg;
    AsrModel::Buf& b = m->b;
    const int dl = c.lm_d_model, Fl = c.lm_d_ffn, H = c.lm_nhead;
    for (int l = 0; l < c.lm_layers; ++l) {
        const LmLayerW& w = m->lm[l];
        __half* kc = b.lkc + (size_t)l * rows * S_max * dl;
        __half* vc = b.lvc + (size_t)l * rows * S_max * dl;
        SkinnyArgs a{};
        a.A = b.lx16; a.lda = dl; a.W = w.w_in; a.ldw = dl; a.bias = w.b_in; a.n_rows = rows; a.N = 3 * dl; a.K = dl;
        a.epi = SK_QKV_CACHE; a.out = b.lq16; a.ldo = dl; a.kcache = kc; a.vcache = vc; a.step_ptr = b.step; a.S_max = S_max;
        a.d = dl; a.q_scale = 1.0f;
        RC(skinny_gemm(a, st));
        DecAttnArgs t{};
        t.q = b.lq16; t.ldq = dl; t.kbase = kc; t.vbase = vc; t.row_stride = (size_t)S_max * dl; t.key_stride = dl;
        t.rows_per_block = 1; t.n_keys_ptr = b.step; t.H = H; t.dh = 64; t.out = b.latt16; t.ldo = dl;
        t.lineage = b.lineage; t.lin_stride = S_max; t.tok_cache = b.tok_cache; t.pad_tok = 0;
        RC(dec_attention(t, rows, S_max, st));
        a = SkinnyArgs{}; a.A = b.latt16; a.lda = dl; a.W = w.w_out; a.ldw = dl; a.bias = w.b_out; a.n_rows = rows;
        a.N = dl; a.K = dl; a.epi = SK_RESID; a.out = b.lx; a.ldo = dl;
        RC(skinny_gemm(a, st));
        RC(layernorm_dual(b.lx, b.lx16, w.n1g, w.n1b, rows, dl, 1e-6f, true, st));
        a = SkinnyArgs{}; a.A = b.lx16; a.lda = dl; a.W = w.w1; a.ldw = dl; a.bias = w.b1; a.n_rows = rows;
        a.N = Fl; a.K = dl; a.epi = c.lm_activation == SBK_ACT_GELU ? SK_F16_GELU : SK_F16_RELU; a.out = b.lf16; a.ldo = Fl;
        RC(skinny_gemm(a, st));
        a = SkinnyArgs{}; a.A = b.lf16; a.lda = Fl; a.W = w.w2; a.ldw = Fl; a.bias = w.b2; a.n_rows = rows;
        a.N = dl; a.K = Fl; a.epi = SK_RESID; a.out = b.lx; a.ldo = dl;
        RC(skinny_gemm(a, st));
        RC(layernorm_dual(b.lx, b.lx16, w.n2g, w.n2b, rows, dl, 1e-6f, true, st));
    }
    RC(layernorm_dual(b.lx, b.lx16, m->lm_norm_g, m->lm_norm_b, rows, dl, 1e-6f, false, st));
    SkinnyArgs a{};
    a.A = b.lx16; a.lda = dl; a.W = m->lm_wp0; a.ldw = dl; a.bias = m->lm_bp0; a.n_rows = rows; a.N = dl; a.K = dl;
    a.epi = SK_F32; a.out = b.lh32; a.ldo = dl;
    RC(skinny_gemm(a, st));
    RC(layernorm_dual(b.lh32, b.lh16, m->lm_lnp_g, m->lm_lnp_b, rows, dl, 1e-6f, false, st));
    a = SkinnyArgs{}; a.A = b.lh16; a.lda = dl; a.W = m->lm_wp2; a.ldw = dl; a.bias = m->lm_bp2; a.n_rows = rows;
    a.N = c.vocab; a.K = dl; a.epi = SK_F32; a.out = b.lm_logits; a.ldo = c.vocab;
    RC(skinny_gemm(a, st));
    RC(weighted_log_softmax(b.lm_logits, b.lm_extra, rows, c.vocab, temperature, weight, st));
    return SBK_OK;
}

static int run_beam(AsrModel* m, int B, int T, const sbk_beam_params& p, int* hist_tok_out, int* hist_pred_out,
                    float* hist_score_out, float* hist_lp_out, int* steps_done, cudaStream_t st) {
    const sbk_asr_config& c = m->cfg;
    AsrModel::Buf& b = m->b;
    const int d = c.d_model, Ld = c.num_decoder_layers, M = B * T, beam = p.beam_size, rows = B * beam, S_max = m->ws_steps + 1;
    SBK_REQUIRE(m->has_dec, "beam: this handle was created without decoder weights");
    SBK_REQUIRE(p.max_steps <= m->ws_steps && p.max_steps + 1 <= c.max_len, "beam: max_steps=%d too large", p.max_steps);
    *steps_done = 0;
    if (p.max_steps <= 0) return SBK_OK;
    RC(project_cross_kv(m, M, T, st));
    set_pdl(getenv("SBK_PDL") != nullptr);
    const bool use_lm = p.lm_weight != 0.0f;
    SBK_REQUIRE(!use_lm || m->has_lm, "beam: lm_weight != 0 but this handle has no TransformerLM weights");
    const bool use_ctc = p.ctc_weight != 0.0f;
    int* hist_tok = b.hist_tok; int* hist_pred = b.hist_pred; float* hist_score = b.hist_score; float* hist_lp = b.hist_lp;
    CtcStep cs{};
    if (use_ctc) {
        SBK_REQUIRE(m->w_ctc, "beam: ctc_weight != 0 but this handle has no ctc_lin weights");
        SBK_REQUIRE(p.blank_index >= 0 && p.blank_index < c.vocab && p.blank_index != p.bos && p.blank_index != p.eos &&
                    p.bos != p.eos, "Set blank, eos and bos to different indexes for joint ATT/CTC or CTC decoding");
        const size_t V = c.vocab;
        auto al = [](size_t n) { return (n * 4 + 255) & ~size_t(255); };
        const size_t need = 2 * al((size_t)M * V) + al(M) + 2 * al((size_t)2 * rows * T) + al(2 * rows) + (use_lm ? 0 : al(rows * V)) +
                            al((size_t)2 * rows * (T + 4)) + al(2 * rows);
        AsrModel::CtcBuf& cb = m->ctc;
        if (need > cb.cap) {
            if (cb.base) { SBK_CUDA_CHECK(cudaStreamSynchronize(st)); cudaFree(cb.base); cb.base = nullptr; cb.cap = 0; }
            if (m->beam_graph) { cudaGraphExecDestroy(m->beam_graph); m->beam_graph = nullptr; }
            if (cudaMalloc(&cb.base, need) != cudaSuccess) { set_error("beam: CTC scorer cudaMalloc(%zu) failed", need); return SBK_ERR_NOMEM; }
            cb.cap = need;
        }
        char* q = reinterpret_cast<char*>(cb.base);
        cb.x = reinterpret_cast<float*>(q); q += al((size_t)M * V);
        cb.xlin = reinterpret_cast<float*>(q); q += al((size_t)M * V);
        cb.xb = reinterpret_cast<float*>(q); q += al(M);
        cb.rsum = reinterpret_cast<float*>(q); q += al((size_t)2 * rows * T);
        cb.rb = reinterpret_cast<float*>(q); q += al((size_t)2 * rows * T);
        cb.psi = reinterpret_cast<float*>(q); q += al(2 * rows);
        cb.tab = reinterpret_cast<float*>(q); q += al((size_t)2 * rows * (T + 4));
        cb.tabM = reinterpret_cast<float*>(q); q += al(2 * rows);
        cb.add = use_lm ? b.lm_extra : reinterpret_cast<float*>(q);
        GemmEpilogue e;
        e.mode = EPI_F32; e.bias = m->b_ctc; e.out = cb.x; e.ldo = c.vocab;
        RC(gemm_f16(b.enc16, d, m->w_ctc, d, e, M, c.vocab, d, st));
        RC(ctc_prefix_reset(cb.x, cb.xlin, cb.xb, b.enc_len, B, T, c.vocab, p.blank_index, beam, cb.rsum, cb.rb, cb.psi, cb.tab, cb.tabM, st));
        cs.x = cb.x; cs.xlin = cb.xlin; cs.xb = cb.xb; cs.enc_len = b.enc_len; cs.hist_tok = hist_tok; cs.hist_pred = hist_pred; cs.n_bh = rows;
        cs.rsum_base = cb.rsum; cs.rb_base = cb.rb; cs.psi_base = cb.psi; cs.step_ptr = b.step; cs.tab = cb.tab; cs.tabM = cb.tabM;
        cs.bos = p.bos; cs.T = T; cs.V = c.vocab; cs.beam = beam; cs.blank = p.blank_index; cs.eos = p.eos;
        cs.weight = p.ctc_weight; cs.out = cb.add; cs.accumulate = use_lm ? 1 : 0;
    }
    const bool use_cov = p.coverage_weight != 0.0f;
    CoverageStep cv{};
    if (use_cov) {
        SBK_REQUIRE(d / c.nhead == 64, "beam: the coverage scorer is built for head_dim 64");
        const size_t need = ((size_t)2 * rows * T + rows) * 4 + 256;
        if (need > m->cov.cap) {
            if (m->cov.base) { SBK_CUDA_CHECK(cudaStreamSynchronize(st)); cudaFree(m->cov.base); m->cov.base = nullptr; m->cov.cap = 0; }
            if (m->beam_graph) { cudaGraphExecDestroy(m->beam_graph); m->beam_graph = nullptr; }
            if (cudaMalloc(&m->cov.base, need) != cudaSuccess) { set_error("beam: coverage scorer cudaMalloc(%zu) failed", need); return SBK_ERR_NOMEM; }
            m->cov.cap = need;
        }
        cv.q = b.dq16; cv.ldq = d; cv.kbase = b.ckv16 + (size_t)(Ld - 1) * M * 2 * d;
        if (xatt_headmajor(m)) { cv.utt_stride = (size_t)T * d; cv.key_stride = 64; cv.head_stride = T * 64; }
        else { cv.utt_stride = (size_t)T * 2 * d; cv.key_stride = 2 * d; cv.head_stride = 64; }
        cv.enc_len = b.enc_len; cv.rows_per_utt = beam; cv.T = T; cv.H = c.nhead;
        cv.cov_base = m->cov.base; cv.hist_pred = hist_pred; cv.step_ptr = b.step; cv.n_bh = rows;
        cv.threshold = p.coverage_threshold; cv.weight = p.coverage_weight; cv.out = m->cov.base + (size_t)2 * rows * T;
    }
    BeamLm lm;
    if (use_lm) { lm.emb = m->lm_emb; lm.pe = m->lm_pe; lm.d = c.lm_d_model; lm.x = b.lx; lm.x16 = b.lx16; lm.tok_cache = b.tok_cache; }
    RC(beam_reset(rows, beam, S_max, p.bos, b.step, b.seq_scores, b.lineage, b.finished, b.ended_count, m->emb, m->dec_pe, d,
                  b.dx, use_lm ? &lm : nullptr, st));
    BeamStepArgs a{};
    a.add_scores = use_lm ? b.lm_extra : (use_ctc ? m->ctc.add : nullptr);
    a.lm = lm;
    if (use_ctc) { a.attn_weight = 1.0f - p.ctc_weight; a.blank = p.blank_index; }
    a.add_const = p.length_weight;
    a.add_row = use_cov ? cv.out : nullptr;
    a.logits = b.logits; a.V = c.vocab; a.beam = beam; a.S_max = S_max; a.seq_scores = b.seq_scores; a.lineage = b.lineage;
    a.step_arr = b.step; a.finished = b.finished; a.n_full = b.ended_count;
    a.hist_tok = hist_tok; a.hist_pred = hist_pred; a.hist_score = hist_score; a.hist_lp = hist_lp;
    a.temperature = p.temperature; a.eos_threshold = p.eos_threshold; a.minus_inf = p.minus_inf; a.min_steps = p.min_steps;
    a.eos = p.eos; a.use_eos_threshold = p.using_eos_threshold; a.length_norm = p.length_normalization;
    a.emb = m->emb; a.pe = m->dec_pe; a.d = d; a.x_next = b.dx; a.scratch = b.beam_scr;
    const bool fork = (use_lm || use_ctc) && getenv("SBK_BEAM_SERIAL") == nullptr;
    if (fork && !m->side_stream) {
        SBK_CUDA_CHECK(cudaStreamCreateWithFlags(&m->side_stream, cudaStreamNonBlocking));
        SBK_CUDA_CHECK(cudaEventCreateWithFlags(&m->ev_bfork, cudaEventDisableTiming));
        SBK_CUDA_CHECK(cudaEventCreateWithFlags(&m->ev_bjoin, cudaEventDisableTiming));
    }
    auto enqueue_step = [&](cudaStream_t s_) -> int {
        cudaStream_t s2 = s_;
        if (fork) {
            s2 = m->side_stream;
            SBK_CUDA_CHECK(cudaEventRecord(m->ev_bfork, s_));
            SBK_CUDA_CHECK(cudaStreamWaitEvent(s2, m->ev_bfork, 0));
        }
        if (use_ctc) RC(ctc_prefix_update(cs, s2));
        if (use_lm) RC(enqueue_lm_step(m, rows, S_max, p.lm_temperature, p.lm_weight, s2));
        RC(enqueue_decode_layers(m, rows, beam, T, S_max, b.lineage, s_));
        if (use_cov) RC(coverage_score(cv, s_));
        if (fork) {
            SBK_CUDA_CHECK(cudaEventRecord(m->ev_bjoin, s2));
            SBK_CUDA_CHECK(cudaStreamWaitEvent(s_, m->ev_bjoin, 0));
        }
        if (use_ctc) RC(ctc_prefix_score(cs, s_));
        RC(beam_step(a, B, s_));
        return SBK_OK;
    };
    const bool use_graph = getenv("SBK_NO_GRAPH") == nullptr;
    if (use_graph) {
        AsrModel::BeamKey key;
        memset(&key, 0, sizeof(key));
        key.p = p; key.B = B; key.T = T; key.rows = rows; key.S_max = S_max; key.fuse_ln = m->fuse_dec_ln; key.tc_rows = m->dec_tc_rows; key.fork = fork ? 1 : 0;
        if (m->beam_graph == nullptr || memcmp(&key, &m->beam_key, sizeof(key)) != 0) {
            if (m->beam_graph) { cudaGraphExecDestroy(m->beam_graph); m->beam_graph = nullptr; }
            if (!m->cap_stream) SBK_CUDA_CHECK(cudaStreamCreateWithFlags(&m->cap_stream, cudaStreamNonBlocking));
            cudaGraph_t g;
            SBK_CUDA_CHECK(cudaStreamBeginCapture(m->cap_stream, cudaStreamCaptureModeThreadLocal));
            launch_count_begin_capture();
            int rc = enqueue_step(m->cap_stream);
            m->beam_nodes = launch_count_end_capture();
            cudaError_t ce = cudaStreamEndCapture(m->cap_stream, &g);
            if (rc) return rc;
            SBK_CUDA_CHECK(ce);
            SBK_CUDA_CHECK(cudaGraphInstantiate(&m->beam_graph, g, 0));
            cudaGraphDestroy(g);
            m->beam_key = key;
        }
    }
    const int check_every = m->poll_every > 0 ? m->poll_every : p.max_steps;
    int s = 0;
    while (s < p.max_steps) {
        const int chunk = std::min(check_every, p.max_steps - s);
        for (int i = 0; i < chunk; ++i) {
            if (use_graph) { SBK_CUDA_CHECK(cudaGraphLaunch(m->beam_graph, st)); launch_count_add(m->beam_nodes); }
            else RC(enqueue_step(st));
        }
        s += chunk;
        if (s < p.max_steps && m->poll_every > 0) {
            SBK_CUDA_CHECK(cudaMemcpyAsync(m->host_flag, b.ended_count, 4, cudaMemcpyDeviceToHost, st));
            SBK_CUDA_CHECK(cudaStreamSynchronize(st));
            if (*m->host_flag >= B) break;
        }
    }
    const size_t hb = (size_t)s * rows * 4;
    if (hist_tok_out) SBK_CUDA_CHECK(cudaMemcpyAsync(hist_tok_out, hist_tok, hb, cudaMemcpyDeviceToDevice, st));
    if (hist_pred_out) SBK_CUDA_CHECK(cudaMemcpyAsync(hist_pred_out, hist_pred, hb, cudaMemcpyDeviceToDevice, st));
    if (hist_score_out) SBK_CUDA_CHECK(cudaMemcpyAsync(hist_score_out, hist_score, hb, cudaMemcpyDeviceToDevice, st));
    if (hist_lp_out) SBK_CUDA_CHECK(cudaMemcpyAsync(hist_lp_out, hist_lp, hb, cudaMemcpyDeviceToDevice, st));
    *steps_done = s;
    return SBK_OK;
}

static int run_greedy(AsrModel* m, int B, int T, int max_steps, int bos, int eos, float* log_probs, int* steps_done,
                      cudaStream_t st, bool in_capture = false) {
    const sbk_asr_config& c = m->cfg;
    AsrModel::Buf& b = m->b;
    const int d = c.d_model, M = B * T, rows = B, S_max = m->ws_steps + 1;
    SBK_REQUIRE(m->has_dec, "greedy: this handle was created without decoder weights");
    SBK_REQUIRE(max_steps <= m->ws_steps && max_steps + 1 <= c.max_len, "greedy: max_steps=%d too large", max_steps);
    *steps_done = 0;
    if (max_steps <= 0) return SBK_OK;
    RC(project_cross_kv(m, M, T, st));
    RC(greedy_reset(b.tokens, S_max + 1, rows, bos, b.step, b.has_ended, b.ended_count, m->emb, m->dec_pe, d, b.dx, st));
    set_pdl(getenv("SBK_PDL") != nullptr);
    const bool use_graph = !in_capture && getenv("SBK_NO_GRAPH") == nullptr && log_probs == nullptr;
    if (in_capture) {
        for (int i = 0; i < max_steps; ++i) RC(enqueue_decode_step(m, rows, 1, T, S_max, eos, log_probs, max_steps, st));
        *steps_done = max_steps;
        return SBK_OK;
    }
    if (use_graph && (m->step_graph == nullptr || m->graph_rows != rows || m->graph_T != T || m->graph_B != B ||
                      m->graph_eos != eos || m->graph_S != S_max)) {
        if (m->step_graph) { cudaGraphExecDestroy(m->step_graph); m->step_graph = nullptr; }
        cudaGraph_t g;
        if (!m->cap_stream) SBK_CUDA_CHECK(cudaStreamCreateWithFlags(&m->cap_stream, cudaStreamNonBlocking));
        SBK_CUDA_CHECK(cudaStreamBeginCapture(m->cap_stream, cudaStreamCaptureModeThreadLocal));
        launch_count_begin_capture();
        int rc = enqueue_decode_step(m, rows, 1, T, S_max, eos, nullptr, 0, m->cap_stream);
        m->graph_nodes = launch_count_end_capture();
        cudaError_t ce = cudaStreamEndCapture(m->cap_stream, &g);
        if (rc) return rc;
        SBK_CUDA_CHECK(ce);
        SBK_CUDA_CHECK(cudaGraphInstantiate(&m->step_graph, g, 0));
        cudaGraphDestroy(g);
        m->graph_rows = rows; m->graph_T = T; m->graph_B = B; m->graph_eos = eos; m->graph_S = S_max;
    }
    const int check_every = m->poll_every > 0 ? m->poll_every : max_steps;
    int s = 0;
    while (s < max_steps) {
        const int chunk = std::min(check_every, max_steps - s);
        for (int i = 0; i < chunk; ++i) {
            if (use_graph) { SBK_CUDA_CHECK(cudaGraphLaunch(m->step_graph, st)); launch_count_add(m->graph_nodes); }
            else RC(enqueue_decode_step(m, rows, 1, T, S_max, eos, log_probs, max_steps, st));
        }
        s += chunk;
        if (s < max_steps && m->poll_every > 0) {
            SBK_CUDA_CHECK(cudaMemcpyAsync(m->host_flag, b.ended_count, 4, cudaMemcpyDeviceToHost, st));
            SBK_CUDA_CHECK(cudaStreamSynchronize(st));
            if (*m->host_flag >= rows) break;
        }
    }
    *steps_done = s;
    return SBK_OK;
}

__global__ void lm_teacher_reset_kernel(const int* __restrict__ tokens, int n, int L, int S_max, int pad, int* __restrict__ lineage,
                                        int* __restrict__ tok_cache, float* __restrict__ scores) {
    const int r = blockIdx.x;
    for (int p = threadIdx.x; p < S_max; p += blockDim.x) {
        lineage[static_cast<size_t>(r) * S_max + p] = r;
        lineage[static_cast<size_t>(n) * S_max + static_cast<size_t>(r) * S_max + p] = r;
        tok_cache[static_cast<size_t>(r) * S_max + p] = p < L ? tokens[static_cast<size_t>(r) * L + p] : pad;
    }
    if (threadIdx.x == 0) scores[r] = 0.0f;
}
__global__ void lm_teacher_embed_kernel(const int* __restrict__ tokens, int L, int s, const float* __restrict__ emb,
                                        const float* __restrict__ pe, int d, float sqrt_d, float* __restrict__ x,
                                        __half* __restrict__ x16, int* __restrict__ step_arr) {
    const int r = blockIdx.x;
    const int tok = tokens[static_cast<size_t>(r) * L + s];
    for (int i = threadIdx.x; i < d; i += blockDim.x) {
        const float v = emb[static_cast<size_t>(tok) * d + i] * sqrt_d + pe[static_cast<size_t>(s) * d + i];
        x[static_cast<size_t>(r) * d + i] = v;
        x16[static_cast<size_t>(r) * d + i] = float2half_sat(v);
    }
    if (threadIdx.x == 0) step_arr[r] = s;
}
__global__ void lm_teacher_score_kernel(const float* __restrict__ log_probs, int V, const int* __restrict__ tokens, int L, int s,
                                        const int* __restrict__ lens, int pad, float* __restrict__ scores, int n) {
    const int r = blockIdx.x * blockDim.x + threadIdx.x;
    if (r >= n || s + 1 >= lens[r]) return;
    const float* lp = log_probs + static_cast<size_t>(r) * V;
    const int tgt = tokens[static_cast<size_t>(r) * L + s + 1];
    const float v = (tgt == pad ? -INFINITY : lp[tgt]) - log1pf(-expf(lp[pad]));
    if (v == v) scores[r] += v;
}

__global__ void dec_teacher_embed_kernel(const int* __restrict__ tokens, int S, int s, const float* __restrict__ emb,
                                         const float* __restrict__ pe, int d, float sqrt_d, float* __restrict__ x,
                                         int* __restrict__ step_arr) {
    const int r = blockIdx.x;
    const int tok = tokens[static_cast<size_t>(r) * S + s];
    for (int i = threadIdx.x; i < d; i += blockDim.x)
        x[static_cast<size_t>(r) * d + i] = emb[static_cast<size_t>(tok) * d + i] * sqrt_d + pe[static_cast<size_t>(s) * d + i];
    if (threadIdx.x == 0) step_arr[r] = s;
}

static int run_decode_teacher(AsrModel* m, const int* tokens, int n, int S, int T, float* out, cudaStream_t st) {
    const sbk_asr_config& c = m->cfg;
    AsrModel::Buf& b = m->b;
    const int d = c.d_model, M = n * T, S_max = m->ws_steps + 1;
    SBK_REQUIRE(m->has_dec, "decode: this handle was created without decoder weights");
    SBK_REQUIRE(S <= m->ws_steps && S <= c.max_len, "decode: %d target positions exceed the workspace / max_len", S);
    RC(project_cross_kv(m, M, T, st));
    for (int s = 0; s < S; ++s) {
        dec_teacher_embed_kernel<<<n, 128, 0, st>>>(tokens, S, s, m->emb, m->dec_pe, d, sqrtf((float)d), b.dx, b.step);
        SBK_LAUNCH_CHECK();
        RC(enqueue_decode_layers(m, n, 1, T, S_max, nullptr, st, false));
        RC(layernorm_rows(b.dx, b.lnout, false, m->dec_norm_g, m->dec_norm_b, n, d, 1e-6f, false, st));
        SBK_CUDA_CHECK(cudaMemcpy2DAsync(out + (size_t)s * d, (size_t)S * d * 4, b.lnout, (size_t)d * 4, (size_t)d * 4, n,
                                         cudaMemcpyDeviceToDevice, st));
    }
    return SBK_OK;
}

static int run_lm_rescore(AsrModel* m, const int* tokens, const int* lens, int n, int L, float temperature, int pad,
                          float* scores, cudaStream_t st) {
    const sbk_asr_config& c = m->cfg;
    AsrModel::Buf& b = m->b;
    const int S_max = m->ws_steps + 1, dl = c.lm_d_model;
    lm_teacher_reset_kernel<<<n, 128, 0, st>>>(tokens, n, L, S_max, pad, b.lineage, b.tok_cache, scores);
    SBK_LAUNCH_CHECK();
    for (int s = 0; s + 1 < L; ++s) {
        lm_teacher_embed_kernel<<<n, 128, 0, st>>>(tokens, L, s, m->lm_emb, m->lm_pe, dl, sqrtf((float)dl), b.lx, b.lx16, b.step);
        SBK_LAUNCH_CHECK();
        RC(enqueue_lm_step(m, n, S_max, temperature, 1.0f, st));
        lm_teacher_score_kernel<<<ceil_div(n, 128), 128, 0, st>>>(b.lm_extra, c.vocab, tokens, L, s, lens, pad, scores, n);
        SBK_LAUNCH_CHECK();
    }
    return SBK_OK;
}

}

using namespace sbk;

extern "C" {

const char* sbk_last_error(void) { return sbk::last_error(); }

int sbk_version(void) { return 100; }

long long sbk_launch_count(void) { return sbk::launch_count(); }

void sbk_gemm_profile_enable(int on) {
    GemmProfile* p = gemm_profile();
    for (cudaEvent_t e : p->ev) cudaEventDestroy(e);
    p->ev.clear();
    p->flops.clear();
    p->shape.clear();
    p->enabled = on != 0;
}
int sbk_gemm_profile_read(int* n_launches, double* total_ms, double* total_flops) {
    GemmProfile* p = gemm_profile();
    double ms = 0.0, fl = 0.0;
    for (size_t i = 0; i < p->flops.size(); ++i) {
        float t = 0.0f;
        if (cudaEventElapsedTime(&t, p->ev[2 * i], p->ev[2 * i + 1]) != cudaSuccess) {
            set_error("sbk_gemm_profile_read: events not complete (synchronize first)");
            return SBK_ERR_CUDA;
        }
        ms += t;
        fl += p->flops[i];
        if (getenv("SBK_GEMM_TRACE"))
            fprintf(stderr, "gemm M=%d N=%d K=%d epi=%d : %.1f us  %.0f TFLOP/s\n", p->shape[4 * i], p->shape[4 * i + 1],
                    p->shape[4 * i + 2], p->shape[4 * i + 3], t * 1e3, p->flops[i] / (t * 1e-3) / 1e12);
    }
    if (n_launches) *n_launches = (int)p->flops.size();
    if (total_ms) *total_ms = ms;
    if (total_flops) *total_flops = fl;
    return SBK_OK;
}

int sbk_fbank_create(int n_fft, int hop, int n_mels, const float* window_host, const float* mel_matrix_host, float amin,
                     float top_db, sbk_fbank** out) {
    return fbank_create(reinterpret_cast<Fbank**>(out), n_fft, hop, n_mels, window_host, mel_matrix_host, amin, top_db);
}
void sbk_fbank_destroy(sbk_fbank* fb) { fbank_destroy(reinterpret_cast<Fbank*>(fb)); }
int sbk_fbank_num_frames(const sbk_fbank* fb, int n_samples) { return fbank_num_frames(reinterpret_cast<const Fbank*>(fb), n_samples); }
int sbk_fbank_forward(const sbk_fbank* fb, const float* wav_dev, int B, int L, float* out_dev, int* utt_max_scratch_dev,
                      void* stream) {
    return fbank_forward(reinterpret_cast<const Fbank*>(fb), wav_dev, B, L, out_dev, utt_max_scratch_dev, nullptr, nullptr,
                         0.0f, static_cast<cudaStream_t>(stream));
}
int sbk_input_norm_global(const float* x_dev, float* out_dev, int B, int T, int F, const float* mean_dev,
                          const float* std_dev, float eps, void* stream) {
    return global_norm_forward(x_dev, out_dev, B, T, F, mean_dev, std_dev, eps, static_cast<cudaStream_t>(stream));
}
int sbk_input_norm_sentence(const float* x_dev, float* out_dev, const float* rel_len_dev, int B, int T, int F,
                            int std_norm, int avoid_padding_norm, float eps, void* stream) {
    return sentence_norm_forward(x_dev, out_dev, rel_len_dev, B, T, F, std_norm, avoid_padding_norm, eps,
                                 static_cast<cudaStream_t>(stream));
}

int sbk_gemm_f16_test(const void* A_dev, const void* W_dev, const float* bias_dev, void* out_dev, int out_is_f32, int act,
                      int M, int N, int K, void* stream) {
    GemmEpilogue e;
    e.mode = out_is_f32 ? EPI_F32 : EPI_F16;
    e.act = act;
    e.bias = bias_dev;
    e.out = out_dev;
    e.ldo = N;
    return gemm_f16(A_dev, K, W_dev, K, e, M, N, K, static_cast<cudaStream_t>(stream));
}

int sbk_gemm_f16_resid_test(const void* A_dev, const void* W_dev, const float* bias_dev, float* x_dev, float alpha, int M,
                            int N, int K, void* stream) {
    GemmEpilogue e;
    e.mode = EPI_RESID;
    e.bias = bias_dev;
    e.out = x_dev;
    e.resid = x_dev;
    e.alpha = alpha;
    e.ldo = N;
    return gemm_f16(A_dev, K, W_dev, K, e, M, N, K, static_cast<cudaStream_t>(stream));
}

int sbk_gemm_epilogue_test(const void* A_dev, const void* W_dev, const float* bias_dev, void* out_dev, int ldo, int mode,
                           int act, float alpha, const float* resid_dev, const int* row_lens_dev, int T,
                           const float* rope_cos_dev, const float* rope_sin_dev, int head_dim, int kv_heads,
                           long long kv_part_stride, long long kv_layer_stride, int M, int N, int K, void* stream) {
    GemmEpilogue e;
    e.mode = mode; e.act = act; e.bias = bias_dev; e.out = out_dev; e.ldo = ldo; e.alpha = alpha;
    e.resid = resid_dev; e.row_lens = row_lens_dev; e.T = T;
    e.rope_cos = rope_cos_dev; e.rope_sin = rope_sin_dev; e.head_dim = head_dim;
    e.kv_heads = kv_heads; e.kv_part_stride = (size_t)kv_part_stride; e.kv_layer_stride = (size_t)kv_layer_stride;
    if (mode < EPI_F16 || mode > EPI_ROPE) { set_error("sbk_gemm_epilogue_test: mode %d", mode); return SBK_ERR_ARG; }
    return gemm_f16(A_dev, K, W_dev, K, e, M, N, K, static_cast<cudaStream_t>(stream));
}

int sbk_asr_create(const sbk_asr_config* cfg, const sbk_tensor* weights, int n_weights, sbk_asr** out) {
    return asr_create(cfg, weights, n_weights, reinterpret_cast<AsrModel**>(out));
}
void sbk_asr_destroy(sbk_asr* m) { asr_destroy(reinterpret_cast<AsrModel*>(m)); }
int sbk_asr_clone(sbk_asr* src, sbk_asr** out) {
    return asr_clone(reinterpret_cast<AsrModel*>(src), reinterpret_cast<AsrModel**>(out));
}
int sbk_asr_set_decoder_ln_fusion(sbk_asr* m, int on) {
    AsrModel* mm = reinterpret_cast<AsrModel*>(m);
    if (mm->fuse_dec_ln != (on != 0)) drop_graphs(mm);
    mm->fuse_dec_ln = on != 0;
    return SBK_OK;
}
int sbk_asr_set_decoder_tc_min_rows(sbk_asr* m, int rows) {
    AsrModel* mm = reinterpret_cast<AsrModel*>(m);
    if (mm->dec_tc_rows != rows) drop_graphs(mm);
    mm->dec_tc_rows = rows;
    return SBK_OK;
}
int sbk_asr_set_dynchunk(sbk_asr* m, int chunk_size, int left_context_chunks) {
    AsrModel* mm = reinterpret_cast<AsrModel*>(m);
    SBK_REQUIRE(chunk_size >= 0, "set_dynchunk: chunk_size must be >= 0 (0 = full-context attention)");
    const int left = left_context_chunks < 0 ? -1 : left_context_chunks;
    if (mm->dyn_chunk != chunk_size || mm->dyn_left != left) drop_graphs(mm);
    mm->dyn_chunk = chunk_size;
    mm->dyn_left = left;
    return SBK_OK;
}
int sbk_asr_set_poll_interval(sbk_asr* m, int every_n_steps) {
    reinterpret_cast<AsrModel*>(m)->poll_every = every_n_steps;
    return SBK_OK;
}

int sbk_asr_num_frames(const sbk_asr* mm, int n_samples, int* T_feat, int* T_enc) {
    const AsrModel* m = reinterpret_cast<const AsrModel*>(mm);
    int T0, T1, T2;
    frames(m->cfg, n_samples, &T0, &T1, &T2);
    if (T_feat) *T_feat = T0;
    if (T_enc) *T_enc = T2;
    return SBK_OK;
}

int sbk_asr_cnn_forward(sbk_asr* mm, const float* feats_dev, int B, int T0, float* out_dev, void* stream) {
    AsrModel* m = reinterpret_cast<AsrModel*>(mm);
    const sbk_asr_config& c = m->cfg;
    SBK_REQUIRE(m->has_cnn, "cnn_forward: this handle was created without CNN weights");
    const int L = (T0 - 1) * c.hop;
    RC(ensure_workspace(m, B, L, std::max(B, m->ws_rows), std::max(1, m->ws_steps)));
    return cnn_frontend_forward(feats_dev, B, T0, c.n_mels, m->c1_w, m->c1_b, m->c1_g, m->c1_be, c.cnn_c1, m->c2_w, m->c2_b,
                                m->c2_g, m->c2_be, c.cnn_c2, m->b.act1, nullptr, m->b.a_in, out_dev,
                                static_cast<cudaStream_t>(stream));
}

int sbk_asr_encode_feats(sbk_asr* mm, const float* feats_dev, const float* rel_len_dev, int B, int T0,
                         float* cnn_out_dev, float* enc_out_dev, void* stream) {
    AsrModel* m = reinterpret_cast<AsrModel*>(mm);
    cudaStream_t st = static_cast<cudaStream_t>(stream);
    const sbk_asr_config& c = m->cfg;
    const int L = (T0 - 1) * c.hop;
    RC(ensure_workspace(m, B, L, std::max(B, m->ws_rows), std::max(1, m->ws_steps)));
    const int T1 = (T0 - 1) / 2 + 1, T = (T1 - 1) / 2 + 1;
    const int* enc_len = nullptr;
    if (rel_len_dev) {
        abs_len_kernel<<<ceil_div(B, 128), 128, 0, st>>>(rel_len_dev, B, T, m->b.enc_len);
        SBK_LAUNCH_CHECK();
        enc_len = m->b.enc_len;
    }
    return run_encoder(m, feats_dev, B, T0, enc_len, cnn_out_dev, enc_out_dev ? enc_out_dev : m->b.enc_out, st);
}

int sbk_asr_encode_from_cnn(sbk_asr* mm, const float* src_dev, const float* rel_len_dev, int B, int T,
                            float* enc_out_dev, void* stream) {
    AsrModel* m = reinterpret_cast<AsrModel*>(mm);
    cudaStream_t st = static_cast<cudaStream_t>(stream);
    const sbk_asr_config& c = m->cfg;
    const int L = ((T - 1) * 4) * c.hop;
    RC(ensure_workspace(m, B, L, std::max(B, m->ws_rows), std::max(1, m->ws_steps)));
    RC(cast_f32_f16(src_dev, m->b.a_in, (size_t)B * T * c.input_size, st));
    const int* enc_len = nullptr;
    if (rel_len_dev) {
        abs_len_kernel<<<ceil_div(B, 128), 128, 0, st>>>(rel_len_dev, B, T, m->b.enc_len);
        SBK_LAUNCH_CHECK();
        enc_len = m->b.enc_len;
    }
    return run_encoder(m, nullptr, B, T, enc_len, nullptr, enc_out_dev ? enc_out_dev : m->b.enc_out, st);
}

// ... 408 lines not shown
```

### speechbrain_b200/csrc/gemm_epilogue.cuh

```cuda
#pragma once
#include "common.cuh"
#include "sbk_internal.h"

namespace sbk {

struct EpiPrefetch {
    float4 bias[8];
    float4 res[8];
    bool on = false;
};
__device__ __forceinline__ void epilogue_prefetch(const GemmEpilogue& e, EpiPrefetch& p, int row, int col0, int M, int N) {
    p.on = row < M && col0 + 32 <= N;
    if (!p.on) return;
#pragma unroll
    for (int j = 0; j < 8; ++j)
        p.bias[j] = e.bias != nullptr ? __ldg(reinterpret_cast<const float4*>(e.bias + col0) + j) : make_float4(0.f, 0.f, 0.f, 0.f);
    if (e.mode == EPI_RESID) {
        const float4* r = reinterpret_cast<const float4*>(e.resid + static_cast<size_t>(row) * e.ldo + col0);
#pragma unroll
        for (int j = 0; j < 8; ++j) p.res[j] = __ldcg(r + j);
    }
}

__device__ __forceinline__ void epilogue_chunk(const GemmEpilogue& e, const uint32_t (&acc)[32], int row, int col0,
                                               int M, int N, const EpiPrefetch& pre) {
    if (row >= M || col0 >= N) return;
    const bool full = (col0 + 32 <= N);
    float v[32];
#pragma unroll
    for (int j = 0; j < 32; ++j) v[j] = __uint_as_float(acc[j]);
    if (pre.on) {
#pragma unroll
        for (int j = 0; j < 32; j += 4) {
            const float4 b = pre.bias[j >> 2];
            v[j] += b.x; v[j + 1] += b.y; v[j + 2] += b.z; v[j + 3] += b.w;
        }
    } else if (e.bias != nullptr) {
        if (full) {
#pragma unroll
            for (int j = 0; j < 32; j += 4) {
                const float4 b = __ldg(reinterpret_cast<const float4*>(e.bias + col0 + j));
                v[j] += b.x; v[j + 1] += b.y; v[j + 2] += b.z; v[j + 3] += b.w;
            }
        } else {
#pragma unroll
            for (int j = 0; j < 32; ++j)
                if (col0 + j < N) v[j] += __ldg(e.bias + col0 + j);
        }
    }
    switch (e.mode) {
        case EPI_F16: {
            if (e.act == ACT_SILU) {
#pragma unroll
                for (int j = 0; j < 32; ++j) v[j] = silu_f(v[j]);
            } else if (e.act == ACT_GELU) {
#pragma unroll
                for (int j = 0; j < 32; ++j) v[j] = gelu_erf_f(v[j]);
            } else if (e.act == ACT_RELU) {
#pragma unroll
                for (int j = 0; j < 32; ++j) v[j] = fmaxf(v[j], 0.0f);
            }
            __half* o = reinterpret_cast<__half*>(e.out) + static_cast<size_t>(row) * e.ldo + col0;
            if (full) {
#pragma unroll
                for (int j = 0; j < 32; j += 8) {
                    __half2 h0 = floats2half2_sat(v[j], v[j + 1]), h1 = floats2half2_sat(v[j + 2], v[j + 3]);
                    __half2 h2 = floats2half2_sat(v[j + 4], v[j + 5]), h3 = floats2half2_sat(v[j + 6], v[j + 7]);
                    uint4 u;
                    u.x = *reinterpret_cast<uint32_t*>(&h0); u.y = *reinterpret_cast<uint32_t*>(&h1);
                    u.z = *reinterpret_cast<uint32_t*>(&h2); u.w = *reinterpret_cast<uint32_t*>(&h3);
                    *reinterpret_cast<uint4*>(o + j) = u;
                }
            } else {
#pragma unroll
                for (int j = 0; j < 32; ++j)
                    if (col0 + j < N) o[j] = float2half_sat(v[j]);
            }
            break;
        }
        case EPI_F32: {
            float* o = reinterpret_cast<float*>(e.out) + static_cast<size_t>(row) * e.ldo + col0;
            if (full) {
#pragma unroll
                for (int j = 0; j < 32; j += 4)
                    *reinterpret_cast<float4*>(o + j) = make_float4(v[j], v[j + 1], v[j + 2], v[j + 3]);
            } else {
#pragma unroll
                for (int j = 0; j < 32; ++j)
                    if (col0 + j < N) o[j] = v[j];
            }
            break;
        }
        case EPI_RESID: {
            float alpha = e.alpha;
            if (e.row_lens != nullptr) {
                const int b = row / e.T, t = row - b * e.T;
                if (t >= e.row_lens[b]) alpha = 0.0f;
            }
            const float* r = e.resid + static_cast<size_t>(row) * e.ldo + col0;
            float* o = reinterpret_cast<float*>(e.out) + static_cast<size_t>(row) * e.ldo + col0;
            if (full) {
#pragma unroll
                for (int j = 0; j < 32; j += 4) {
                    const float4 x = pre.on ? pre.res[j >> 2] : *reinterpret_cast<const float4*>(r + j);
                    *reinterpret_cast<float4*>(o + j) = make_float4(fmaf(alpha, v[j], x.x), fmaf(alpha, v[j + 1], x.y),
                                                                    fmaf(alpha, v[j + 2], x.z), fmaf(alpha, v[j + 3], x.w));
                }
            } else {
#pragma unroll
                for (int j = 0; j < 32; ++j)
                    if (col0 + j < N) o[j] = fmaf(alpha, v[j], r[j]);
            }
            break;
        }
        case EPI_QKV_CACHE: {
            const int sect = col0 / e.qkv_d, c = col0 - sect * e.qkv_d;
            __half* o;
            if (sect == 0) o = reinterpret_cast<__half*>(e.out) + static_cast<size_t>(row) * e.ldo + c;
            else o = (sect == 1 ? e.kcache : e.vcache) +
                     (static_cast<size_t>(row) * e.S_max + __ldg(e.step_ptr + row)) * e.qkv_d + c;
#pragma unroll
            for (int j = 0; j < 32; j += 8) {
                __half2 h0 = floats2half2_sat(v[j], v[j + 1]), h1 = floats2half2_sat(v[j + 2], v[j + 3]);
                __half2 h2 = floats2half2_sat(v[j + 4], v[j + 5]), h3 = floats2half2_sat(v[j + 6], v[j + 7]);
                uint4 u;
                u.x = *reinterpret_cast<uint32_t*>(&h0); u.y = *reinterpret_cast<uint32_t*>(&h1);
                u.z = *reinterpret_cast<uint32_t*>(&h2); u.w = *reinterpret_cast<uint32_t*>(&h3);
                *reinterpret_cast<uint4*>(o + j) = u;
            }
            break;
        }
        case EPI_GLU: {
            float* o = reinterpret_cast<float*>(e.out) + static_cast<size_t>(row) * e.ldo + (col0 >> 1);
#pragma unroll
            for (int j = 0; j < 16; j += 4)
                *reinterpret_cast<float4*>(o + j) =
                    make_float4(v[j] * sigmoid_f(v[j + 16]), v[j + 1] * sigmoid_f(v[j + 17]),
                                v[j + 2] * sigmoid_f(v[j + 18]), v[j + 3] * sigmoid_f(v[j + 19]));
            break;
        }
        case EPI_ROPE: {
            const int dh = e.head_dim;
            const int within = col0 % (3 * dh);
            const int sect = within / dh;
            if (sect < 2) {
                const int t = row % e.T;
                const int p0 = (within - sect * dh) >> 1;
                const float* cs = e.rope_cos + static_cast<size_t>(t) * (dh >> 1) + p0;
                const float* sn = e.rope_sin + static_cast<size_t>(t) * (dh >> 1) + p0;
                const float sc = sect == 0 ? e.alpha : 1.0f;
#pragma unroll
                for (int j = 0; j < 32; j += 2) {
                    const float c = __ldg(cs + (j >> 1)), s = __ldg(sn + (j >> 1));
                    const float x0 = v[j], x1 = v[j + 1];
                    v[j] = (x0 * c - x1 * s) * sc;
                    v[j + 1] = (x1 * c + x0 * s) * sc;
                }
            }
            __half* o = reinterpret_cast<__half*>(e.out) + static_cast<size_t>(row) * e.ldo + col0;
#pragma unroll
            for (int j = 0; j < 32; j += 8) {
                __half2 h0 = floats2half2_sat(v[j], v[j + 1]), h1 = floats2half2_sat(v[j + 2], v[j + 3]);
                __half2 h2 = floats2half2_sat(v[j + 4], v[j + 5]), h3 = floats2half2_sat(v[j + 6], v[j + 7]);
                uint4 u;
                u.x = *reinterpret_cast<uint32_t*>(&h0); u.y = *reinterpret_cast<uint32_t*>(&h1);
                u.z = *reinterpret_cast<uint32_t*>(&h2); u.w = *reinterpret_cast<uint32_t*>(&h3);
                *reinterpret_cast<uint4*>(o + j) = u;
            }
            break;
        }
    }
}

}
```

### speechbrain_b200/csrc/gemm_mainloop.cuh

```cuda
#pragma once
#include "common.cuh"

namespace sbk {

constexpr int WG_BM = 128;
constexpr int WG_BK = 64;
constexpr int WG_CONSUMERS = 256;
constexpr int WG_THREADS = WG_CONSUMERS + 32;

template <int BN>
struct WgAcc {
    static constexpr int WN = BN < 128 ? BN : 128;
    static constexpr int NI = BN / WN;
    float r[NI][WN / 2];
};

template <int BN, int STAGES>
struct WgRing {
    static constexpr int A_BYTES = WG_BM * WG_BK * 2;
    static constexpr int B_BYTES = BN * WG_BK * 2;
    static constexpr int STAGE_BYTES = A_BYTES + B_BYTES;
    static constexpr int BAR_OFFSET = STAGES * STAGE_BYTES;
    static constexpr int END = BAR_OFFSET + 2 * STAGES * 8;
    static constexpr int STG_PITCH = BN * 4 + 16;
    static_assert(STAGE_BYTES % 1024 == 0, "128B-swizzled stages must stay 1 KB aligned");
    static_assert(WG_BM * STG_PITCH <= BAR_OFFSET, "the accumulator staging tile reuses the operand ring");
};

__device__ __forceinline__ void wg_consumers_sync() { asm volatile("bar.sync 1, %0;" ::"n"(WG_CONSUMERS) : "memory"); }

template <int BN, int STAGES>
__device__ __forceinline__ void wg_init(uint8_t* smem, const CUtensorMap* ta, const CUtensorMap* tb) {
    using R = WgRing<BN, STAGES>;
    uint64_t* full_bar = reinterpret_cast<uint64_t*>(smem + R::BAR_OFFSET);
    uint64_t* empty_bar = full_bar + STAGES;
    if (threadIdx.x == WG_CONSUMERS) {
        tma_prefetch_desc(ta);
        tma_prefetch_desc(tb);
        for (int s = 0; s < STAGES; ++s) {
            mbar_init(&full_bar[s], 1);
            mbar_init(&empty_bar[s], 2);
        }
        mbar_fence_init();
    }
    __syncthreads();
}

template <int BN, int STAGES>
__device__ __forceinline__ void wg_produce(uint8_t* smem, const CUtensorMap* ta, const CUtensorMap* tb, int m0, int n0,
                                           int kb0, int num_kb) {
    using R = WgRing<BN, STAGES>;
    if (threadIdx.x != WG_CONSUMERS) return;
    uint64_t* full_bar = reinterpret_cast<uint64_t*>(smem + R::BAR_OFFSET);
    uint64_t* empty_bar = full_bar + STAGES;
    for (int kb = 0; kb < num_kb; ++kb) {
        const int s = kb % STAGES;
        const uint32_t ph = (kb / STAGES) & 1;
        mbar_wait(&empty_bar[s], ph ^ 1);
        mbar_arrive_expect_tx(&full_bar[s], R::STAGE_BYTES);
        uint8_t* a_dst = smem + s * R::STAGE_BYTES;
        tma_load_2d(a_dst, ta, &full_bar[s], (kb0 + kb) * WG_BK, m0);
        tma_load_2d(a_dst + R::A_BYTES, tb, &full_bar[s], (kb0 + kb) * WG_BK, n0);
    }
}

template <int BN, int STAGES>
__device__ __forceinline__ void wg_consume_and_stage(uint8_t* smem, int num_kb) {
    using R = WgRing<BN, STAGES>;
    using Acc = WgAcc<BN>;
    uint64_t* full_bar = reinterpret_cast<uint64_t*>(smem + R::BAR_OFFSET);
    uint64_t* empty_bar = full_bar + STAGES;
    const int wg = threadIdx.x >> 7;
    Acc acc;
#pragma unroll
    for (int i = 0; i < Acc::NI; ++i)
#pragma unroll
        for (int j = 0; j < Acc::WN / 2; ++j) acc.r[i][j] = 0.0f;
    for (int kb = 0; kb < num_kb; ++kb) {
        const int s = kb % STAGES;
        const uint32_t ph = (kb / STAGES) & 1;
        mbar_wait(&full_bar[s], ph);
        const uint32_t a_addr = smem_u32(smem + s * R::STAGE_BYTES) + wg * 64 * 128;
        const uint32_t b_addr = smem_u32(smem + s * R::STAGE_BYTES) + R::A_BYTES;
        const uint64_t da = make_kmajor_sw128_desc(a_addr);
        wgmma_fence();
#pragma unroll
        for (int k = 0; k < WG_BK / 16; ++k)
#pragma unroll
            for (int i = 0; i < Acc::NI; ++i)
                wgmma_f16<Acc::WN>(acc.r[i], da + 2 * k, make_kmajor_sw128_desc(b_addr + i * Acc::WN * 128) + 2 * k, 1u);
        wgmma_commit();
        wgmma_wait<1>();
        if (kb > 0 && (threadIdx.x & 127) == 0) mbar_arrive(&empty_bar[(kb - 1) % STAGES]);
    }
    wgmma_wait<0>();
    wg_consumers_sync();
    const int w = (threadIdx.x >> 5) & 3, l = threadIdx.x & 31;
    uint8_t* base = smem + (wg * 64 + w * 16 + (l >> 2)) * R::STG_PITCH + (l & 3) * 8;
#pragma unroll
    for (int i = 0; i < Acc::NI; ++i)
#pragma unroll
        for (int j = 0; j < Acc::WN / 8; ++j) {
            const int col = i * Acc::WN + j * 8;
            *reinterpret_cast<float2*>(base + col * 4) = make_float2(acc.r[i][4 * j], acc.r[i][4 * j + 1]);
            *reinterpret_cast<float2*>(base + 8 * R::STG_PITCH + col * 4) = make_float2(acc.r[i][4 * j + 2], acc.r[i][4 * j + 3]);
        }
    wg_consumers_sync();
}

__device__ __forceinline__ void wg_load_row32(uint32_t addr, uint32_t (&a)[32]) {
#pragma unroll
    for (int j = 0; j < 8; ++j) {
        const uint4 v = lds128(addr + 16 * j);
        a[4 * j] = v.x; a[4 * j + 1] = v.y; a[4 * j + 2] = v.z; a[4 * j + 3] = v.w;
    }
}

}
```

### speechbrain_b200/csrc/gemm_tc.cu

```cuda
#include <stdlib.h>

#include "common.cuh"
#include "gemm_epilogue.cuh"
#include "gemm_mainloop.cuh"
#include "sbk_internal.h"

namespace sbk {

template <int BN, int STAGES, int SPLIT = 1>
struct GemmSmem {
    static constexpr int TOTAL = WgRing<BN, STAGES>::END + 1024;
};

__device__ __forceinline__ uint32_t gemm_cluster_rank() {
    uint32_t r;
    asm volatile("mov.u32 %0, %%cluster_ctarank;" : "=r"(r));
    return r;
}
__device__ __forceinline__ void gemm_cluster_sync() {
    asm volatile("barrier.cluster.arrive.release.aligned;" ::: "memory");
    asm volatile("barrier.cluster.wait.acquire.aligned;" ::: "memory");
}
__device__ __forceinline__ uint4 ld_cluster_u4(uint32_t local_addr, uint32_t cta) {
    uint32_t raddr;
    asm volatile("mapa.shared::cluster.u32 %0, %1, %2;" : "=r"(raddr) : "r"(local_addr), "r"(cta));
    uint4 v;
    asm volatile("ld.shared::cluster.v4.u32 {%0, %1, %2, %3}, [%4];" : "=r"(v.x), "=r"(v.y), "=r"(v.z), "=r"(v.w) : "r"(raddr)
                 : "memory");
    return v;
}

template <int BN, int STAGES, int SPLIT = 1>
__global__ void __launch_bounds__(WG_THREADS, (BN <= 128 ? 2 : 1))
gemm_tc_kernel(const __grid_constant__ CUtensorMap tmap_a, const __grid_constant__ CUtensorMap tmap_b,
               const GemmEpilogue epi, int M, int N, int K) {
    using R = WgRing<BN, STAGES>;
    extern __shared__ uint8_t smem_raw[];
    uint8_t* smem = reinterpret_cast<uint8_t*>((reinterpret_cast<uintptr_t>(smem_raw) + 1023) & ~uintptr_t(1023));
    const int n0 = blockIdx.x * BN, m0 = blockIdx.y * WG_BM;
    const uint32_t rank = SPLIT > 1 ? gemm_cluster_rank() : 0u;
    const int num_kb = (K + WG_BK - 1) / WG_BK / SPLIT;
    const int kb0 = static_cast<int>(rank) * num_kb;

    wg_init<BN, STAGES>(smem, &tmap_a, &tmap_b);
    EpiPrefetch pre;
    if (threadIdx.x >= WG_CONSUMERS) {
        wg_produce<BN, STAGES>(smem, &tmap_a, &tmap_b, m0, n0, kb0, num_kb);
    } else {
        if constexpr (BN == 32 && SPLIT == 1)
            if (threadIdx.x < WG_BM) epilogue_prefetch(epi, pre, m0 + threadIdx.x, n0, M, N);
        wg_consume_and_stage<BN, STAGES>(smem, num_kb);
    }
    if constexpr (SPLIT > 1) gemm_cluster_sync();
    if (threadIdx.x < WG_CONSUMERS && rank == 0) {
        const int r = threadIdx.x & (WG_BM - 1);
#pragma unroll 1
        for (int c = threadIdx.x / WG_BM; c < BN / 32; c += WG_CONSUMERS / WG_BM) {
            const uint32_t src = smem_u32(smem) + r * R::STG_PITCH + c * 128;
            uint32_t acc[32];
            wg_load_row32(src, acc);
#pragma unroll 1
            for (int p = 1; p < SPLIT; ++p) {
#pragma unroll
                for (int j = 0; j < 8; ++j) {
                    const uint4 v = ld_cluster_u4(src + 16 * j, static_cast<uint32_t>(p));
                    acc[4 * j] = __float_as_uint(__uint_as_float(acc[4 * j]) + __uint_as_float(v.x));
                    acc[4 * j + 1] = __float_as_uint(__uint_as_float(acc[4 * j + 1]) + __uint_as_float(v.y));
                    acc[4 * j + 2] = __float_as_uint(__uint_as_float(acc[4 * j + 2]) + __uint_as_float(v.z));
                    acc[4 * j + 3] = __float_as_uint(__uint_as_float(acc[4 * j + 3]) + __uint_as_float(v.w));
                }
            }
            epilogue_chunk(epi, acc, m0 + r, n0 + c * 32, M, N, pre);
        }
    }
    if constexpr (SPLIT > 1) gemm_cluster_sync();
}

template <int BN, int STAGES, int SPLIT = 1>
static int launch_gemm(const void* A, int lda, const void* W, int ldw, const GemmEpilogue& epi, int M, int N, int K,
                       cudaStream_t stream) {
    using S = GemmSmem<BN, STAGES, SPLIT>;
    CUtensorMap ta, tb;
    int rc = make_tmap_2d_f16(&ta, A, M, K, lda, WG_BM, WG_BK);
    if (rc) return rc;
    rc = make_tmap_2d_f16(&tb, W, N, K, ldw, BN, WG_BK);
    if (rc) return rc;
    auto kern = gemm_tc_kernel<BN, STAGES, SPLIT>;
    SBK_CUDA_CHECK(cudaFuncSetAttribute(kern, cudaFuncAttributeMaxDynamicSharedMemorySize, S::TOTAL));
    dim3 grid(ceil_div(N, BN), ceil_div(M, WG_BM), SPLIT);
    GemmProfile* prof = gemm_profile();
    cudaEvent_t e0 = nullptr, e1 = nullptr;
    if (prof->enabled) {
        cudaEventCreate(&e0);
        cudaEventCreate(&e1);
        cudaEventRecord(e0, stream);
    }
    if constexpr (SPLIT == 1) {
        kern<<<grid, WG_THREADS, S::TOTAL, stream>>>(ta, tb, epi, M, N, K);
    } else {
        cudaLaunchConfig_t cfg = {};
        cfg.gridDim = grid;
        cfg.blockDim = dim3(WG_THREADS);
        cfg.dynamicSmemBytes = S::TOTAL;
        cfg.stream = stream;
        cudaLaunchAttribute attr[1];
        attr[0].id = cudaLaunchAttributeClusterDimension;
        attr[0].val.clusterDim.x = 1;
        attr[0].val.clusterDim.y = 1;
        attr[0].val.clusterDim.z = SPLIT;
        cfg.attrs = attr;
        cfg.numAttrs = 1;
        SBK_CUDA_CHECK(cudaLaunchKernelEx(&cfg, kern, ta, tb, epi, M, N, K));
    }
    if (prof->enabled) {
        cudaEventRecord(e1, stream);
        prof->ev.push_back(e0);
        prof->ev.push_back(e1);
        prof->flops.push_back(2.0 * M * N * K);
        prof->shape.insert(prof->shape.end(), {M, N, K, epi.mode});
    }
    SBK_LAUNCH_CHECK();
    return SBK_OK;
}

int gemm_f16_small(const void* A, int lda, const void* W, int ldw, const GemmEpilogue& epi, int M, int N, int K,
                   cudaStream_t stream) {
    SBK_REQUIRE(M > 0 && N > 0 && K > 0, "gemm_f16_small: empty problem M=%d N=%d K=%d", M, N, K);
    SBK_REQUIRE((K % 8) == 0 && (lda % 8) == 0 && (ldw % 8) == 0, "gemm_f16_small: K/lda/ldw must be multiples of 8");
    SBK_REQUIRE((reinterpret_cast<uintptr_t>(A) & 15) == 0 && (reinterpret_cast<uintptr_t>(W) & 15) == 0,
                "gemm_f16_small: operands must be 16-byte aligned");
    SBK_REQUIRE(epi.mode == EPI_F16 || epi.mode == EPI_F32 || epi.mode == EPI_RESID || epi.mode == EPI_QKV_CACHE,
                "gemm_f16_small: epilogue mode %d not supported", epi.mode);
    if (epi.mode == EPI_QKV_CACHE)
        SBK_REQUIRE(epi.qkv_d % 32 == 0 && N == 3 * epi.qkv_d && epi.kcache && epi.vcache && epi.step_ptr,
                    "gemm_f16_small: bad EPI_QKV_CACHE arguments");
    if (N > 2048) return launch_gemm<64, 6>(A, lda, W, ldw, epi, M, N, K, stream);
    static const bool split = getenv("SBK_DEC_SPLITK") != nullptr;
    if (K >= 2048 && K % (4 * WG_BK) == 0 && split)
        return launch_gemm<32, 8, 4>(A, lda, W, ldw, epi, M, N, K, stream);
    return launch_gemm<32, 8>(A, lda, W, ldw, epi, M, N, K, stream);
}

int gemm_f16(const void* A, int lda, const void* W, int ldw, const GemmEpilogue& epi, int M, int N, int K,
             cudaStream_t stream) {
    SBK_REQUIRE(M > 0 && N > 0 && K > 0, "gemm_f16: empty problem M=%d N=%d K=%d", M, N, K);
    SBK_REQUIRE((K % 8) == 0 && (lda % 8) == 0 && (ldw % 8) == 0, "gemm_f16: K/lda/ldw must be multiples of 8");
    SBK_REQUIRE((reinterpret_cast<uintptr_t>(A) & 15) == 0 && (reinterpret_cast<uintptr_t>(W) & 15) == 0,
                "gemm_f16: operands must be 16-byte aligned");
    if (epi.mode == EPI_GLU || epi.mode == EPI_ROPE)
        SBK_REQUIRE(N % 32 == 0, "gemm_f16: GLU/RoPE epilogues need N %% 32 == 0");
    if (epi.mode == EPI_ROPE) SBK_REQUIRE(epi.head_dim % 32 == 0, "gemm_f16: RoPE epilogue needs head_dim %% 32 == 0");
    if (N % 256 == 0 && getenv("SBK_GEMM_V1") == nullptr) return gemm_f16_wide(A, lda, W, ldw, epi, M, N, K, stream);
    return launch_gemm<128, 3>(A, lda, W, ldw, epi, M, N, K, stream);
}

}
```

### speechbrain_b200/csrc/sbk_internal.h

```cpp
#pragma once
#include <cuda_fp16.h>
#include <cuda_runtime.h>
#include <stdint.h>

#include <vector>

namespace sbk {

enum GemmEpiMode { EPI_F16 = 0, EPI_F32 = 1, EPI_RESID = 2, EPI_GLU = 3, EPI_ROPE = 4, EPI_QKV_CACHE = 5 };
enum GemmAct { ACT_NONE = 0, ACT_SILU = 1, ACT_GELU = 2, ACT_RELU = 3, ACT_SILU_FAST = 4  };

struct GemmEpilogue {
    int mode = EPI_F16;
    int act = ACT_NONE;
    const float* bias = nullptr;
    void* out = nullptr;
    int ldo = 0;
    const float* resid = nullptr;
    float alpha = 1.0f;
    const int* row_lens = nullptr;
    int T = 1;
    const float* rope_cos = nullptr;
    const float* rope_sin = nullptr;
    int head_dim = 64;
    __half* kcache = nullptr; __half* vcache = nullptr; const int* step_ptr = nullptr; int S_max = 0; int qkv_d = 0;
    int kv_heads = 0; size_t kv_part_stride = 0; size_t kv_layer_stride = 0;
};

int gemm_f16(const void* A, int lda, const void* W, int ldw, const GemmEpilogue& epi, int M, int N, int K,
             cudaStream_t stream);
int gemm_f16_small(const void* A, int lda, const void* W, int ldw, const GemmEpilogue& epi, int M, int N, int K,
                   cudaStream_t stream);
int gemm_f16_wide(const void* A, int lda, const void* W, int ldw, const GemmEpilogue& epi, int M, int N, int K,
                  cudaStream_t stream);


const char* last_error();
void launch_count_begin_capture();
long long launch_count_end_capture();
void launch_count_add(long long n);
long long launch_count();

struct GemmProfile {
    bool enabled = false;
    std::vector<cudaEvent_t> ev;
    std::vector<double> flops;
    std::vector<int> shape;
};
GemmProfile* gemm_profile();

struct Fbank;
int fbank_create(Fbank** out, int n_fft, int hop, int n_mels, const float* window_host, const float* mel_matrix_host,
                 float amin, float top_db);
void fbank_destroy(Fbank* fb);
int fbank_num_frames(const Fbank* fb, int L);
int fbank_forward(const Fbank* fb, const float* wav, int B, int L, float* out, int* utt_max, const float* mean,
                  const float* stdv, float eps, cudaStream_t stream);
int global_norm_forward(const float* x, float* out, int B, int T, int F, const float* mean, const float* stdv,
                        float eps, cudaStream_t stream);
int sentence_norm_forward(const float* x, float* out, const float* rel_len, int B, int T, int F, int std_norm,
                          int avoid_padding_norm, float eps, cudaStream_t stream);

int cnn_frontend_forward(const float* feats, int B, int T0, int F0, const float* w1, const float* b1, const float* g1,
                         const float* be1, int C1, const __half* w2p, const float* b2, const float* g2,
                         const float* be2, int C2, __half* act1_h, float* act1_f, __half* out_h, float* out_f,
                         cudaStream_t stream);

int layernorm_rows(const float* x, void* out, bool out_half, const float* gamma, const float* beta, int M, int D,
                   float eps, bool act_silu, cudaStream_t stream);
int layernorm2_rows(const float* x, float* y_out, void* z_out, bool z_half, const float* ga, const float* ba, float eps_a,
                    const float* gb, const float* bb, float eps_b, int M, int D, cudaStream_t stream);
int cast_f32_f16(const float* in, __half* out, size_t n, cudaStream_t stream);
int dwconv_ln_swish(const float* glu, int B, int T, int D, int K, const float* wdw, const float* bdw,
                    const float* gamma, const float* beta, float eps, __half* out, cudaStream_t stream, int chunk = 0);
int encoder_attention(const __half* qkv, int ld, int B, int T, int H, int head_dim, const int* lens, bool relpos,
                      const float* pos_u, const float* pos_v, const __half* P, int ldp, float scale, __half* out,
                      int ldo, cudaStream_t stream, int chunk = 0, int left_chunks = -1);

enum SkinnyEpi { SK_F16 = 0, SK_F16_GELU = 1, SK_F32 = 2, SK_RESID = 3, SK_QKV_CACHE = 4, SK_F16_RELU = 5 };
struct SkinnyArgs {
    const __half* A; int lda;
    const __half* W; int ldw;
    const float* bias;
    int n_rows, N, K, epi;
    void* out; int ldo;
    __half* kcache; __half* vcache;
    const int* step_ptr; int S_max; int d; float q_scale;
    const float* X; const float* ln_g; const float* ln_b; float ln_eps;
};
void set_pdl(bool on);
int skinny_gemm(const SkinnyArgs& a, cudaStream_t stream);
struct DecAttnArgs {
    const __half* q; int ldq;
    const __half* kbase; const __half* vbase;
    size_t row_stride;
    int key_stride;
    int head_stride = 0;
    int rows_per_block;
    const int* n_keys_ptr;
    const int* enc_len;
    int n_keys_fixed;
    int H, dh;
    __half* out; int ldo;
    const int* lineage; int lin_stride;
    const int* tok_cache; int pad_tok;
};
int dec_attention(const DecAttnArgs& a, int n_rows, int max_keys, cudaStream_t stream);
int make_tmap_kv_f16(CUtensorMap* out, const void* base, int n_utt, int T, int H, uint64_t key_stride_elems,
                     uint64_t utt_stride_elems, int box_T);
struct BeamLm {
    const float* emb = nullptr; const float* pe = nullptr; int d = 0;
    float* x = nullptr; __half* x16 = nullptr; int* tok_cache = nullptr;
};
struct BeamStepArgs {
    const float* logits; int V; int beam; int S_max;
    float* seq_scores; int* lineage; int* step_arr; int* finished; int* n_full;
    int* hist_tok; int* hist_pred; float* hist_score; float* hist_lp;
    float temperature, eos_threshold, minus_inf;
    int min_steps, eos, use_eos_threshold, length_norm;
    const float* emb; const float* pe; int d; float* x_next;
    const float* add_scores;
    BeamLm lm;
    float attn_weight = 1.0f;
    int blank = -1;
    float add_const = 0.0f;
    const float* add_row = nullptr;
    float* scratch = nullptr;
};
struct CoverageStep {
    const __half* q; int ldq; const __half* kbase; size_t utt_stride; int key_stride; const int* enc_len;
    int head_stride = 0;
    int rows_per_utt, T, H; float* cov_base; const int* hist_pred; const int* step_ptr; int n_bh;
    float threshold, weight; float* out;
};
int coverage_score(const CoverageStep& p, cudaStream_t stream);
struct CtcStep {
    const float* x; const float* xlin; const float* xb; const int* enc_len;
    float* rsum_base; float* rb_base; float* psi_base;
    float* tab; float* tabM;
    const int* hist_tok; const int* hist_pred;
    const int* step_ptr;
    int n_bh, bos, T, V, beam, blank, eos;
    float weight; float* out; int accumulate;
};
int ctc_prefix_reset(float* x, float* xlin, float* xb, const int* enc_len, int B, int T, int V, int blank, int beam, float* rsum,
                     float* rb, float* psi_prev, float* tab, float* tabM, cudaStream_t stream);
int ctc_prefix_score(const CtcStep& p, cudaStream_t stream);
int rows_logsoftmax_argmax(float* x, int rows, int V, bool do_logsoftmax, int* idx, cudaStream_t stream);
int ctc_prefix_update(const CtcStep& p, cudaStream_t stream);
int beam_reset(int n_bh, int beam, int S_max, int bos, int* step_arr, float* seq_scores, int* lineage, int* finished,
               int* n_full, const float* emb, const float* pe, int d, float* x, const BeamLm* lm, cudaStream_t stream);
int layernorm_dual(float* x, __half* x16, const float* gamma, const float* beta, int M, int D, float eps, bool write_f32,
                   cudaStream_t stream);
int weighted_log_softmax(const float* logits, float* out, int rows, int V, float temperature, float weight,
                         cudaStream_t stream);
int beam_step(const BeamStepArgs& p, int B, cudaStream_t stream);
int greedy_reset(int* tokens, int tok_stride, int n_rows, int bos, int* step_arr, int* has_ended, int* ended_count,
                 const float* emb, const float* pe, int d, float* x, cudaStream_t stream);
int greedy_select(const float* logits, int n_rows, int V, int* step_arr, int eos, int* tokens, int tok_stride,
                  int* has_ended, int* ended_count, int* pred, float* score, int out_stride, float* log_probs, int L,
                  const float* emb, const float* pe, int d, float* x_next, cudaStream_t stream);

}
```

Before: 42870.

## Enable PDL across tensor-core decode step with prologue prefetch before grid wait

Result: faster. 44260, median of 6 (+3.3%).

```diff
diff --git a/speechbrain_b200/csrc/common.cuh b/speechbrain_b200/csrc/common.cuh
--- a/speechbrain_b200/csrc/common.cuh
+++ b/speechbrain_b200/csrc/common.cuh
@@ -41,6 +41,25 @@
 __host__ __device__ inline int ceil_div(int a, int b) { return (a + b - 1) / b; }
 
 constexpr int SBK_NUM_SMS = 132;
+
+__device__ __forceinline__ void pdl_trigger() { asm volatile("griddepcontrol.launch_dependents;" ::: "memory"); }
+__device__ __forceinline__ void pdl_wait() { asm volatile("griddepcontrol.wait;" ::: "memory"); }
+
+template <typename... KArgs, typename... Args>
+inline cudaError_t launch_pdl(void (*kern)(KArgs...), dim3 grid, dim3 block, size_t smem, cudaStream_t st, bool pdl,
+                              Args... args) {
+    cudaLaunchConfig_t cfg = {};
+    cfg.gridDim = grid;
+    cfg.blockDim = block;
+    cfg.dynamicSmemBytes = smem;
+    cfg.stream = st;
+    cudaLaunchAttribute attr[1];
+    attr[0].id = cudaLaunchAttributeProgrammaticStreamSerialization;
+    attr[0].val.programmaticStreamSerializationAllowed = 1;
+    cfg.attrs = attr;
+    cfg.numAttrs = pdl ? 1 : 0;
+    return cudaLaunchKernelEx(&cfg, kern, args...);
+}
 
 __device__ __forceinline__ float warp_sum(float v) {
 #pragma unroll
diff --git a/speechbrain_b200/csrc/decoder.cu b/speechbrain_b200/csrc/decoder.cu
--- a/speechbrain_b200/csrc/decoder.cu
+++ b/speechbrain_b200/csrc/decoder.cu
@@ -14,25 +14,12 @@
         : "r"(a[0]), "r"(a[1]), "r"(a[2]), "r"(a[3]), "r"(b0), "r"(b1));
 }
 
-__device__ __forceinline__ void pdl_trigger() { asm volatile("griddepcontrol.launch_dependents;" ::: "memory"); }
-__device__ __forceinline__ void pdl_wait() { asm volatile("griddepcontrol.wait;" ::: "memory"); }
-
 static bool g_use_pdl = true;
 void set_pdl(bool on) { g_use_pdl = on; }
 
 template <typename... KArgs, typename... Args>
 static cudaError_t launch_k(void (*kern)(KArgs...), dim3 grid, dim3 block, size_t smem, cudaStream_t st, Args... args) {
-    cudaLaunchConfig_t cfg = {};
-    cfg.gridDim = grid;
-    cfg.blockDim = block;
-    cfg.dynamicSmemBytes = smem;
-    cfg.stream = st;
-    cudaLaunchAttribute attr[1];
-    attr[0].id = cudaLaunchAttributeProgrammaticStreamSerialization;
-    attr[0].val.programmaticStreamSerializationAllowed = 1;
-    cfg.attrs = attr;
-    cfg.numAttrs = g_use_pdl ? 1 : 0;
-    return cudaLaunchKernelEx(&cfg, kern, args...);
+    return launch_pdl(kern, grid, block, smem, st, g_use_pdl, args...);
 }
 
 constexpr int SK_WARPS = 8;
@@ -267,8 +254,9 @@
     const int warp = threadIdx.x >> 5, lane = threadIdx.x & 31;
     const int r = blockIdx.y, h = blockIdx.x;
     const int blk = r / a.rows_per_block;
+    const bool xatt = a.n_keys_ptr == nullptr && a.lineage == nullptr && a.tok_cache == nullptr;
     pdl_trigger();
-    pdl_wait();
+    if (!xatt) pdl_wait();
     int n_keys;
     if (a.n_keys_ptr) n_keys = *a.n_keys_ptr + 1;
     else n_keys = a.enc_len ? min(a.enc_len[blk], a.n_keys_fixed) : a.n_keys_fixed;
@@ -281,23 +269,9 @@
     const int* lin = nullptr;
     if (a.lineage) lin = a.lineage + static_cast<size_t>((n_keys - 1) & 1) * gridDim.y * a.lin_stride + static_cast<size_t>(r) * a.lin_stride;
     const int* tokc = a.tok_cache;
-    float qf[8];
-    {
-        const uint4 qv = *reinterpret_cast<const uint4*>(a.q + static_cast<size_t>(r) * a.ldq + h * 64 + dl);
-        const __half2* q2 = reinterpret_cast<const __half2*>(&qv);
-#pragma unroll
-        for (int u = 0; u < 4; ++u) {
-            const float2 f = __half22float2(q2[u]);
-            qf[2 * u] = f.x; qf[2 * u + 1] = f.y;
-        }
-    }
-    float m_run = -INFINITY, l_run = 0.0f;
-    float o[8];
-#pragma unroll
-    for (int e = 0; e < 8; ++e) o[e] = 0.0f;
-    for (int c0 = kb; c0 < ke; c0 += DA_CHUNK) {
-        uint4 kv[DA_KPG], vv[DA_KPG];
-        bool live[DA_KPG];
+    uint4 kv[DA_KPG], vv[DA_KPG];
+    bool live[DA_KPG];
+    auto load_chunk = [&](int c0) {
 #pragma unroll
         for (int i = 0; i < DA_KPG; ++i) {
             const int j = c0 + gq + 4 * i;
@@ -314,6 +288,27 @@
                 vv[i] = make_uint4(0u, 0u, 0u, 0u);
             }
         }
+    };
+    if (xatt) {
+        load_chunk(kb);
+        pdl_wait();
+    }
+    float qf[8];
+    {
+        const uint4 qv = *reinterpret_cast<const uint4*>(a.q + static_cast<size_t>(r) * a.ldq + h * 64 + dl);
+        const __half2* q2 = reinterpret_cast<const __half2*>(&qv);
+#pragma unroll
+        for (int u = 0; u < 4; ++u) {
+            const float2 f = __half22float2(q2[u]);
+            qf[2 * u] = f.x; qf[2 * u + 1] = f.y;
+        }
+    }
+    float m_run = -INFINITY, l_run = 0.0f;
+    float o[8];
+#pragma unroll
+    for (int e = 0; e < 8; ++e) o[e] = 0.0f;
+    for (int c0 = kb; c0 < ke; c0 += DA_CHUNK) {
+        if (!xatt || c0 != kb) load_chunk(c0);
         float sc[DA_KPG];
         float cm = -INFINITY;
 #pragma unroll
diff --git a/speechbrain_b200/csrc/encoder_ops.cu b/speechbrain_b200/csrc/encoder_ops.cu
--- a/speechbrain_b200/csrc/encoder_ops.cu
+++ b/speechbrain_b200/csrc/encoder_ops.cu
@@ -7,17 +7,30 @@
 
 constexpr int LN_MAX_PER_LANE = 32;
 
-template <bool OUT_HALF>
+template <bool OUT_HALF, bool PDL>
 __global__ void __launch_bounds__(256)
 layernorm_rows_kernel(const float* __restrict__ x, void* __restrict__ out, const float* __restrict__ gamma,
                       const float* __restrict__ beta, int M, int D, float eps, int act_silu) {
     const int row = blockIdx.x * (blockDim.x >> 5) + (threadIdx.x >> 5);
+    const int lane = threadIdx.x & 31;
+    const int nv = D >> 2;
+    float4 gp[PDL ? LN_MAX_PER_LANE / 4 : 1], bp[PDL ? LN_MAX_PER_LANE / 4 : 1];
+    if constexpr (PDL) {
+#pragma unroll
+        for (int i = 0; i < LN_MAX_PER_LANE / 4; ++i) {
+            const int vi = lane + i * 32;
+            if (vi < nv && row < M) {
+                gp[i] = __ldg(reinterpret_cast<const float4*>(gamma + vi * 4));
+                bp[i] = __ldg(reinterpret_cast<const float4*>(beta + vi * 4));
+            }
+        }
+        pdl_trigger();
+        pdl_wait();
+    }
     if (row >= M) return;
-    const int lane = threadIdx.x & 31;
     const float* xr = x + static_cast<size_t>(row) * D;
     float v[LN_MAX_PER_LANE];
     float s = 0.0f;
-    const int nv = D >> 2;
 #pragma unroll
     for (int i = 0; i < LN_MAX_PER_LANE / 4; ++i) {
         const int vi = lane + i * 32;
@@ -47,8 +60,8 @@
     for (int i = 0; i < LN_MAX_PER_LANE / 4; ++i) {
         const int vi = lane + i * 32;
         if (vi < nv) {
-            const float4 g = __ldg(reinterpret_cast<const float4*>(gamma + vi * 4));
-            const float4 b = __ldg(reinterpret_cast<const float4*>(beta + vi * 4));
+            const float4 g = PDL ? gp[PDL ? i : 0] : __ldg(reinterpret_cast<const float4*>(gamma + vi * 4));
+            const float4 b = PDL ? bp[PDL ? i : 0] : __ldg(reinterpret_cast<const float4*>(beta + vi * 4));
             float y0 = (v[4 * i] - mean) * rstd * g.x + b.x;
             float y1 = (v[4 * i + 1] - mean) * rstd * g.y + b.y;
             float y2 = (v[4 * i + 2] - mean) * rstd * g.z + b.z;
@@ -69,16 +82,20 @@
 }
 
 int layernorm_rows(const float* x, void* out, bool out_half, const float* gamma, const float* beta, int M, int D,
-                   float eps, bool act_silu, cudaStream_t stream) {
+                   float eps, bool act_silu, cudaStream_t stream, bool pdl) {
     SBK_REQUIRE(D % 4 == 0 && D <= 32 * LN_MAX_PER_LANE, "layernorm_rows: D=%d unsupported", D);
     if (M == 0) return SBK_OK;
     const int rows_per_cta = 8;
-    if (out_half)
-        layernorm_rows_kernel<true><<<ceil_div(M, rows_per_cta), rows_per_cta * 32, 0, stream>>>(x, out, gamma, beta, M, D,
-                                                                                              eps, act_silu);
-    else
-        layernorm_rows_kernel<false><<<ceil_div(M, rows_per_cta), rows_per_cta * 32, 0, stream>>>(x, out, gamma, beta, M,
-                                                                                               D, eps, act_silu);
+    const dim3 grid(ceil_div(M, rows_per_cta)), block(rows_per_cta * 32);
+    if (pdl) {
+        SBK_REQUIRE(out_half, "layernorm_rows: the PDL variant writes fp16");
+        SBK_CUDA_CHECK(launch_pdl(layernorm_rows_kernel<true, true>, grid, block, 0, stream, true, x, out, gamma, beta, M, D,
+                                  eps, static_cast<int>(act_silu)));
+    } else if (out_half) {
+        layernorm_rows_kernel<true, false><<<grid, block, 0, stream>>>(x, out, gamma, beta, M, D, eps, act_silu);
+    } else {
+        layernorm_rows_kernel<false, false><<<grid, block, 0, stream>>>(x, out, gamma, beta, M, D, eps, act_silu);
+    }
     SBK_LAUNCH_CHECK();
     return SBK_OK;
 }
diff --git a/speechbrain_b200/csrc/engine.cu b/speechbrain_b200/csrc/engine.cu
--- a/speechbrain_b200/csrc/engine.cu
+++ b/speechbrain_b200/csrc/engine.cu
@@ -713,7 +713,7 @@
         const DecLayerW& w = m->dec[l];
         __half* kc = b.kcache + (size_t)l * rows * S_max * d;
         __half* vc = b.vcache + (size_t)l * rows * S_max * d;
-        RC(layernorm_rows(b.dx, b.dh16, true, w.n1g, w.n1b, rows, d, 1e-6f, false, st));
+        RC(layernorm_rows(b.dx, b.dh16, true, w.n1g, w.n1b, rows, d, 1e-6f, false, st, true));
         GemmEpilogue e;
         e.mode = EPI_QKV_CACHE; e.bias = w.b_self_in; e.out = b.dq16; e.ldo = d; e.kcache = kc; e.vcache = vc;
         e.step_ptr = b.step; e.S_max = S_max; e.qkv_d = d;
@@ -725,7 +725,7 @@
         RC(dec_attention(t, rows, S_max, st));
         e = GemmEpilogue(); e.mode = EPI_RESID; e.bias = w.b_self_out; e.out = b.dx; e.resid = b.dx; e.ldo = d;
         RC(gemm_f16_small(b.datt16, d, w.w_self_out, d, e, rows, d, d, st));
-        RC(layernorm_rows(b.dx, b.dh16, true, w.n2g, w.n2b, rows, d, 1e-6f, false, st));
+        RC(layernorm_rows(b.dx, b.dh16, true, w.n2g, w.n2b, rows, d, 1e-6f, false, st, true));
         e = GemmEpilogue(); e.mode = EPI_F16; e.bias = w.b_cross_q; e.out = b.dq16; e.ldo = d;
         RC(gemm_f16_small(b.dh16, d, w.w_cross_q, d, e, rows, d, d, st));
         t = DecAttnArgs{};
@@ -734,7 +734,7 @@
         RC(dec_attention(t, rows, T, st));
         e = GemmEpilogue(); e.mode = EPI_RESID; e.bias = w.b_cross_out; e.out = b.dx; e.resid = b.dx; e.ldo = d;
         RC(gemm_f16_small(b.datt16, d, w.w_cross_out, d, e, rows, d, d, st));
-        RC(layernorm_rows(b.dx, b.dh16, true, w.n3g, w.n3b, rows, d, 1e-6f, false, st));
+        RC(layernorm_rows(b.dx, b.dh16, true, w.n3g, w.n3b, rows, d, 1e-6f, false, st, true));
         e = GemmEpilogue(); e.mode = EPI_F16; e.act = c.decoder_activation == SBK_ACT_GELU ? ACT_GELU : ACT_RELU;
         e.bias = w.b_ffn1; e.out = b.df16; e.ldo = F;
         RC(gemm_f16_small(b.dh16, d, w.w_ffn1, d, e, rows, F, d, st));
@@ -743,16 +743,21 @@
     }
     if (!with_head) return SBK_OK;
     SBK_REQUIRE(m->w_lin != nullptr, "decode step: this handle was created without the output head (seq_lin.w.*)");
-    RC(layernorm_rows(b.dx, b.dh16, true, m->dec_norm_g, m->dec_norm_b, rows, d, 1e-6f, false, st));
+    RC(layernorm_rows(b.dx, b.dh16, true, m->dec_norm_g, m->dec_norm_b, rows, d, 1e-6f, false, st, true));
     GemmEpilogue e;
     e.mode = EPI_F32; e.bias = m->b_lin; e.out = b.logits; e.ldo = c.vocab;
     RC(gemm_f16_small(b.dh16, d, m->w_lin, d, e, rows, c.vocab, d, st));
     return SBK_OK;
 }
 
+static bool decode_tc(const AsrModel* m, int rows) {
+    return rows >= m->dec_tc_rows && m->cfg.d_model % 32 == 0;
+}
+static void set_decode_pdl(const AsrModel* m, int rows) { set_pdl(decode_tc(m, rows) || getenv("SBK_PDL") != nullptr); }
+
 static int enqueue_decode_layers(AsrModel* m, int rows, int rows_per_utt, int T, int S_max, const int* lineage,
                                  cudaStream_t st, bool with_head = true) {
-    if (rows >= m->dec_tc_rows && m->cfg.d_model % 32 == 0)
+    if (decode_tc(m, rows))
         return enqueue_decode_layers_tc(m, rows, rows_per_utt, T, S_max, lineage, st, with_head);
     const sbk_asr_config& c = m->cfg;
     AsrModel::Buf& b = m->b;
@@ -909,7 +914,7 @@
     *steps_done = 0;
     if (p.max_steps <= 0) return SBK_OK;
     RC(project_cross_kv(m, M, T, st));
-    set_pdl(getenv("SBK_PDL") != nullptr);
+    set_decode_pdl(m, rows);
     const bool use_lm = p.lm_weight != 0.0f;
     SBK_REQUIRE(!use_lm || m->has_lm, "beam: lm_weight != 0 but this handle has no TransformerLM weights");
     const bool use_ctc = p.ctc_weight != 0.0f;
@@ -1064,7 +1069,7 @@
     if (max_steps <= 0) return SBK_OK;
     RC(project_cross_kv(m, M, T, st));
     RC(greedy_reset(b.tokens, S_max + 1, rows, bos, b.step, b.has_ended, b.ended_count, m->emb, m->dec_pe, d, b.dx, st));
-    set_pdl(getenv("SBK_PDL") != nullptr);
+    set_decode_pdl(m, rows);
     const bool use_graph = !in_capture && getenv("SBK_NO_GRAPH") == nullptr && log_probs == nullptr;
     if (in_capture) {
         for (int i = 0; i < max_steps; ++i) RC(enqueue_decode_step(m, rows, 1, T, S_max, eos, log_probs, max_steps, st));
diff --git a/speechbrain_b200/csrc/gemm_epilogue.cuh b/speechbrain_b200/csrc/gemm_epilogue.cuh
--- a/speechbrain_b200/csrc/gemm_epilogue.cuh
+++ b/speechbrain_b200/csrc/gemm_epilogue.cuh
@@ -9,13 +9,15 @@
     float4 res[8];
     bool on = false;
 };
-__device__ __forceinline__ void epilogue_prefetch(const GemmEpilogue& e, EpiPrefetch& p, int row, int col0, int M, int N) {
+__device__ __forceinline__ void epilogue_prefetch_bias(const GemmEpilogue& e, EpiPrefetch& p, int row, int col0, int M, int N) {
     p.on = row < M && col0 + 32 <= N;
     if (!p.on) return;
 #pragma unroll
     for (int j = 0; j < 8; ++j)
         p.bias[j] = e.bias != nullptr ? __ldg(reinterpret_cast<const float4*>(e.bias + col0) + j) : make_float4(0.f, 0.f, 0.f, 0.f);
-    if (e.mode == EPI_RESID) {
+}
+__device__ __forceinline__ void epilogue_prefetch_resid(const GemmEpilogue& e, EpiPrefetch& p, int row, int col0) {
+    if (p.on && e.mode == EPI_RESID) {
         const float4* r = reinterpret_cast<const float4*>(e.resid + static_cast<size_t>(row) * e.ldo + col0);
 #pragma unroll
         for (int j = 0; j < 8; ++j) p.res[j] = __ldcg(r + j);
diff --git a/speechbrain_b200/csrc/gemm_mainloop.cuh b/speechbrain_b200/csrc/gemm_mainloop.cuh
--- a/speechbrain_b200/csrc/gemm_mainloop.cuh
+++ b/speechbrain_b200/csrc/gemm_mainloop.cuh
@@ -3,10 +3,14 @@
 
 namespace sbk {
 
-constexpr int WG_BM = 128;
 constexpr int WG_BK = 64;
-constexpr int WG_CONSUMERS = 256;
-constexpr int WG_THREADS = WG_CONSUMERS + 32;
+
+template <int BM>
+struct WgRoles {
+    static_assert(BM == 64 || BM == 128, "one or two consumer warpgroups");
+    static constexpr int CONSUMERS = 2 * BM;
+    static constexpr int THREADS = CONSUMERS + 32;
+};
 
 template <int BN>
 struct WgAcc {
@@ -15,58 +19,69 @@
     float r[NI][WN / 2];
 };
 
-template <int BN, int STAGES>
+template <int BM, int BN, int STAGES>
 struct WgRing {
-    static constexpr int A_BYTES = WG_BM * WG_BK * 2;
+    static constexpr int A_BYTES = BM * WG_BK * 2;
     static constexpr int B_BYTES = BN * WG_BK * 2;
     static constexpr int STAGE_BYTES = A_BYTES + B_BYTES;
     static constexpr int BAR_OFFSET = STAGES * STAGE_BYTES;
     static constexpr int END = BAR_OFFSET + 2 * STAGES * 8;
     static constexpr int STG_PITCH = BN * 4 + 16;
     static_assert(STAGE_BYTES % 1024 == 0, "128B-swizzled stages must stay 1 KB aligned");
-    static_assert(WG_BM * STG_PITCH <= BAR_OFFSET, "the accumulator staging tile reuses the operand ring");
+    static_assert(BM * STG_PITCH <= BAR_OFFSET, "the accumulator staging tile reuses the operand ring");
 };
 
-__device__ __forceinline__ void wg_consumers_sync() { asm volatile("bar.sync 1, %0;" ::"n"(WG_CONSUMERS) : "memory"); }
+template <int BM>
+__device__ __forceinline__ void wg_consumers_sync() {
+    asm volatile("bar.sync 1, %0;" ::"n"(WgRoles<BM>::CONSUMERS) : "memory");
+}
 
-template <int BN, int STAGES>
+template <int BM, int BN, int STAGES>
 __device__ __forceinline__ void wg_init(uint8_t* smem, const CUtensorMap* ta, const CUtensorMap* tb) {
-    using R = WgRing<BN, STAGES>;
+    using R = WgRing<BM, BN, STAGES>;
     uint64_t* full_bar = reinterpret_cast<uint64_t*>(smem + R::BAR_OFFSET);
     uint64_t* empty_bar = full_bar + STAGES;
-    if (threadIdx.x == WG_CONSUMERS) {
+    if (threadIdx.x == WgRoles<BM>::CONSUMERS) {
         tma_prefetch_desc(ta);
         tma_prefetch_desc(tb);
         for (int s = 0; s < STAGES; ++s) {
             mbar_init(&full_bar[s], 1);
-            mbar_init(&empty_bar[s], 2);
+            mbar_init(&empty_bar[s], BM / 64);
         }
         mbar_fence_init();
     }
     __syncthreads();
 }
 
-template <int BN, int STAGES>
+template <int BM, int BN, int STAGES>
 __device__ __forceinline__ void wg_produce(uint8_t* smem, const CUtensorMap* ta, const CUtensorMap* tb, int m0, int n0,
                                            int kb0, int num_kb) {
-    using R = WgRing<BN, STAGES>;
-    if (threadIdx.x != WG_CONSUMERS) return;
+    using R = WgRing<BM, BN, STAGES>;
+    if (threadIdx.x != WgRoles<BM>::CONSUMERS) return;
     uint64_t* full_bar = reinterpret_cast<uint64_t*>(smem + R::BAR_OFFSET);
     uint64_t* empty_bar = full_bar + STAGES;
+    const int pre = num_kb < STAGES ? num_kb : STAGES;
+    for (int kb = 0; kb < pre; ++kb) {
+        mbar_arrive_expect_tx(&full_bar[kb], R::STAGE_BYTES);
+        tma_load_2d(smem + kb * R::STAGE_BYTES + R::A_BYTES, tb, &full_bar[kb], (kb0 + kb) * WG_BK, n0);
+    }
+    pdl_trigger();
+    pdl_wait();
     for (int kb = 0; kb < num_kb; ++kb) {
         const int s = kb % STAGES;
-        const uint32_t ph = (kb / STAGES) & 1;
-        mbar_wait(&empty_bar[s], ph ^ 1);
-        mbar_arrive_expect_tx(&full_bar[s], R::STAGE_BYTES);
         uint8_t* a_dst = smem + s * R::STAGE_BYTES;
+        if (kb >= pre) {
+            mbar_wait(&empty_bar[s], ((kb / STAGES) & 1) ^ 1);
+            mbar_arrive_expect_tx(&full_bar[s], R::STAGE_BYTES);
+            tma_load_2d(a_dst + R::A_BYTES, tb, &full_bar[s], (kb0 + kb) * WG_BK, n0);
+        }
         tma_load_2d(a_dst, ta, &full_bar[s], (kb0 + kb) * WG_BK, m0);
-        tma_load_2d(a_dst + R::A_BYTES, tb, &full_bar[s], (kb0 + kb) * WG_BK, n0);
     }
 }
 
-template <int BN, int STAGES>
+template <int BM, int BN, int STAGES>
 __device__ __forceinline__ void wg_consume_and_stage(uint8_t* smem, int num_kb) {
-    using R = WgRing<BN, STAGES>;
+    using R = WgRing<BM, BN, STAGES>;
     using Acc = WgAcc<BN>;
     uint64_t* full_bar = reinterpret_cast<uint64_t*>(smem + R::BAR_OFFSET);
     uint64_t* empty_bar = full_bar + STAGES;
@@ -94,7 +109,7 @@
         if (kb > 0 && (threadIdx.x & 127) == 0) mbar_arrive(&empty_bar[(kb - 1) % STAGES]);
     }
     wgmma_wait<0>();
-    wg_consumers_sync();
+    wg_consumers_sync<BM>();
     const int w = (threadIdx.x >> 5) & 3, l = threadIdx.x & 31;
     uint8_t* base = smem + (wg * 64 + w * 16 + (l >> 2)) * R::STG_PITCH + (l & 3) * 8;
 #pragma unroll
@@ -105,7 +120,7 @@
             *reinterpret_cast<float2*>(base + col * 4) = make_float2(acc.r[i][4 * j], acc.r[i][4 * j + 1]);
             *reinterpret_cast<float2*>(base + 8 * R::STG_PITCH + col * 4) = make_float2(acc.r[i][4 * j + 2], acc.r[i][4 * j + 3]);
         }
-    wg_consumers_sync();
+    wg_consumers_sync<BM>();
 }
 
 __device__ __forceinline__ void wg_load_row32(uint32_t addr, uint32_t (&a)[32]) {
diff --git a/speechbrain_b200/csrc/gemm_tc.cu b/speechbrain_b200/csrc/gemm_tc.cu
--- a/speechbrain_b200/csrc/gemm_tc.cu
+++ b/speechbrain_b200/csrc/gemm_tc.cu
@@ -7,9 +7,9 @@
 
 namespace sbk {
 
-template <int BN, int STAGES, int SPLIT = 1>
+template <int BM, int BN, int STAGES>
 struct GemmSmem {
-    static constexpr int TOTAL = WgRing<BN, STAGES>::END + 1024;
+    static constexpr int TOTAL = WgRing<BM, BN, STAGES>::END + 1024;
 };
 
 __device__ __forceinline__ uint32_t gemm_cluster_rank() {
@@ -30,32 +30,37 @@
     return v;
 }
 
-template <int BN, int STAGES, int SPLIT = 1>
-__global__ void __launch_bounds__(WG_THREADS, (BN <= 128 ? 2 : 1))
+template <int BM, int BN, int STAGES, int SPLIT = 1>
+__global__ void __launch_bounds__(WgRoles<BM>::THREADS, (BN <= 128 ? 2 : 1))
 gemm_tc_kernel(const __grid_constant__ CUtensorMap tmap_a, const __grid_constant__ CUtensorMap tmap_b,
                const GemmEpilogue epi, int M, int N, int K) {
-    using R = WgRing<BN, STAGES>;
+    using R = WgRing<BM, BN, STAGES>;
+    constexpr int CONSUMERS = WgRoles<BM>::CONSUMERS;
     extern __shared__ uint8_t smem_raw[];
     uint8_t* smem = reinterpret_cast<uint8_t*>((reinterpret_cast<uintptr_t>(smem_raw) + 1023) & ~uintptr_t(1023));
-    const int n0 = blockIdx.x * BN, m0 = blockIdx.y * WG_BM;
+    const int n0 = blockIdx.x * BN, m0 = blockIdx.y * BM;
     const uint32_t rank = SPLIT > 1 ? gemm_cluster_rank() : 0u;
     const int num_kb = (K + WG_BK - 1) / WG_BK / SPLIT;
     const int kb0 = static_cast<int>(rank) * num_kb;
 
-    wg_init<BN, STAGES>(smem, &tmap_a, &tmap_b);
+    wg_init<BM, BN, STAGES>(smem, &tmap_a, &tmap_b);
     EpiPrefetch pre;
-    if (threadIdx.x >= WG_CONSUMERS) {
-        wg_produce<BN, STAGES>(smem, &tmap_a, &tmap_b, m0, n0, kb0, num_kb);
+    if (threadIdx.x >= CONSUMERS) {
+        wg_produce<BM, BN, STAGES>(smem, &tmap_a, &tmap_b, m0, n0, kb0, num_kb);
     } else {
-        if constexpr (BN == 32 && SPLIT == 1)
-            if (threadIdx.x < WG_BM) epilogue_prefetch(epi, pre, m0 + threadIdx.x, n0, M, N);
-        wg_consume_and_stage<BN, STAGES>(smem, num_kb);
+        constexpr bool prefetch = BN == 32 && SPLIT == 1;
+        if constexpr (prefetch)
+            if (threadIdx.x < BM) epilogue_prefetch_bias(epi, pre, m0 + threadIdx.x, n0, M, N);
+        pdl_wait();
+        if constexpr (prefetch)
+            if (threadIdx.x < BM) epilogue_prefetch_resid(epi, pre, m0 + threadIdx.x, n0);
+        wg_consume_and_stage<BM, BN, STAGES>(smem, num_kb);
     }
     if constexpr (SPLIT > 1) gemm_cluster_sync();
-    if (threadIdx.x < WG_CONSUMERS && rank == 0) {
-        const int r = threadIdx.x & (WG_BM - 1);
+    if (threadIdx.x < CONSUMERS && rank == 0) {
+        const int r = threadIdx.x & (BM - 1);
 #pragma unroll 1
-        for (int c = threadIdx.x / WG_BM; c < BN / 32; c += WG_CONSUMERS / WG_BM) {
+        for (int c = threadIdx.x / BM; c < BN / 32; c += CONSUMERS / BM) {
             const uint32_t src = smem_u32(smem) + r * R::STG_PITCH + c * 128;
             uint32_t acc[32];
             wg_load_row32(src, acc);
@@ -76,18 +81,18 @@
     if constexpr (SPLIT > 1) gemm_cluster_sync();
 }
 
-template <int BN, int STAGES, int SPLIT = 1>
+template <int BM, int BN, int STAGES, int SPLIT = 1>
 static int launch_gemm(const void* A, int lda, const void* W, int ldw, const GemmEpilogue& epi, int M, int N, int K,
-                       cudaStream_t stream) {
-    using S = GemmSmem<BN, STAGES, SPLIT>;
+                       cudaStream_t stream, bool pdl) {
+    using S = GemmSmem<BM, BN, STAGES>;
     CUtensorMap ta, tb;
-    int rc = make_tmap_2d_f16(&ta, A, M, K, lda, WG_BM, WG_BK);
+    int rc = make_tmap_2d_f16(&ta, A, M, K, lda, BM, WG_BK);
     if (rc) return rc;
     rc = make_tmap_2d_f16(&tb, W, N, K, ldw, BN, WG_BK);
     if (rc) return rc;
-    auto kern = gemm_tc_kernel<BN, STAGES, SPLIT>;
+    auto kern = gemm_tc_kernel<BM, BN, STAGES, SPLIT>;
     SBK_CUDA_CHECK(cudaFuncSetAttribute(kern, cudaFuncAttributeMaxDynamicSharedMemorySize, S::TOTAL));
-    dim3 grid(ceil_div(N, BN), ceil_div(M, WG_BM), SPLIT);
+    dim3 grid(ceil_div(N, BN), ceil_div(M, BM), SPLIT);
     GemmProfile* prof = gemm_profile();
     cudaEvent_t e0 = nullptr, e1 = nullptr;
     if (prof->enabled) {
@@ -96,11 +101,11 @@
         cudaEventRecord(e0, stream);
     }
     if constexpr (SPLIT == 1) {
-        kern<<<grid, WG_THREADS, S::TOTAL, stream>>>(ta, tb, epi, M, N, K);
+        SBK_CUDA_CHECK(launch_pdl(kern, grid, dim3(WgRoles<BM>::THREADS), S::TOTAL, stream, pdl, ta, tb, epi, M, N, K));
     } else {
         cudaLaunchConfig_t cfg = {};
         cfg.gridDim = grid;
-        cfg.blockDim = dim3(WG_THREADS);
+        cfg.blockDim = dim3(WgRoles<BM>::THREADS);
         cfg.dynamicSmemBytes = S::TOTAL;
         cfg.stream = stream;
         cudaLaunchAttribute attr[1];
@@ -134,11 +139,11 @@
     if (epi.mode == EPI_QKV_CACHE)
         SBK_REQUIRE(epi.qkv_d % 32 == 0 && N == 3 * epi.qkv_d && epi.kcache && epi.vcache && epi.step_ptr,
                     "gemm_f16_small: bad EPI_QKV_CACHE arguments");
-    if (N > 2048) return launch_gemm<64, 6>(A, lda, W, ldw, epi, M, N, K, stream);
+    if (N > 2048) return launch_gemm<64, 64, 6>(A, lda, W, ldw, epi, M, N, K, stream, true);
     static const bool split = getenv("SBK_DEC_SPLITK") != nullptr;
     if (K >= 2048 && K % (4 * WG_BK) == 0 && split)
-        return launch_gemm<32, 8, 4>(A, lda, W, ldw, epi, M, N, K, stream);
-    return launch_gemm<32, 8>(A, lda, W, ldw, epi, M, N, K, stream);
+        return launch_gemm<128, 32, 8, 4>(A, lda, W, ldw, epi, M, N, K, stream, false);
+    return launch_gemm<64, 32, 8>(A, lda, W, ldw, epi, M, N, K, stream, true);
 }
 
 int gemm_f16(const void* A, int lda, const void* W, int ldw, const GemmEpilogue& epi, int M, int N, int K,
@@ -151,7 +156,7 @@
         SBK_REQUIRE(N % 32 == 0, "gemm_f16: GLU/RoPE epilogues need N %% 32 == 0");
     if (epi.mode == EPI_ROPE) SBK_REQUIRE(epi.head_dim % 32 == 0, "gemm_f16: RoPE epilogue needs head_dim %% 32 == 0");
     if (N % 256 == 0 && getenv("SBK_GEMM_V1") == nullptr) return gemm_f16_wide(A, lda, W, ldw, epi, M, N, K, stream);
-    return launch_gemm<128, 3>(A, lda, W, ldw, epi, M, N, K, stream);
+    return launch_gemm<128, 128, 3>(A, lda, W, ldw, epi, M, N, K, stream, false);
 }
 
 }
diff --git a/speechbrain_b200/csrc/sbk_internal.h b/speechbrain_b200/csrc/sbk_internal.h
--- a/speechbrain_b200/csrc/sbk_internal.h
+++ b/speechbrain_b200/csrc/sbk_internal.h
@@ -67,7 +67,7 @@
                          cudaStream_t stream);
 
 int layernorm_rows(const float* x, void* out, bool out_half, const float* gamma, const float* beta, int M, int D,
-                   float eps, bool act_silu, cudaStream_t stream);
+                   float eps, bool act_silu, cudaStream_t stream, bool pdl = false);
 int layernorm2_rows(const float* x, float* y_out, void* z_out, bool z_half, const float* ga, const float* ba, float eps_a,
                     const float* gb, const float* bb, float eps_b, int M, int D, cudaStream_t stream);
 int cast_f32_f16(const float* in, __half* out, size_t n, cudaStream_t stream);
```
